# filodb/FiloDB

Hardware: NVIDIA H100
Metric: samples/s scanned+aggregated (rate over 10M series); % HBM roofline (higher is better)
Workload: dtype f64

## Files before the change

### filodb_b200/csrc/capi.cu

```cuda
#include "../../include/filo_b200.h"
#include "kernels.h"
#include "host_util.h"
#include "scan_tile_layout.h"
#include "scan_wp_layout.h"
#include <cub/cub.cuh>
#include <algorithm>
#include <atomic>
#include <chrono>
#include <cmath>
#include <cstdio>
#include <cstdlib>
#include <cstring>
#include <mutex>
#include <string>
#include <thread>
#include <vector>

using namespace filo;

struct filo_ctx {
  int device = 0;
  filo_cfg cfg{};
  cudaStream_t stream = nullptr;
  int sm_count = 132;
// ... 538 lines not shown
                                    int32_t ts_col, int32_t val_col, const int32_t* group_ids, int32_t n_groups,
                                    int32_t schema_flags, filo_table** out) {
  try { return filo_load_series_impl(ctx, n_series, n_chunks, addrs, ts_col, val_col, group_ids, n_groups, schema_flags, out); }
  catch (const std::bad_alloc&) { return fail(ctx, FILO_ERR_OOM, "filo_load_series: host allocation failed"); }
  catch (const std::exception& e) { return fail(ctx, FILO_ERR_INVALID_ARG, std::string("filo_load_series: ") + e.what()); }
}

extern "C" int32_t filo_table_set_groups(filo_ctx* ctx, filo_table* t, const int32_t* group_ids, int32_t n_groups) {
  if (!ctx || !t) return fail(ctx, FILO_ERR_INVALID_ARG, "null");
  CUDA_TRY(ctx, cudaSetDevice(ctx->device));
  if (group_ids && ctx->cfg.group_by_cardinality_limit > 0 && n_groups > ctx->cfg.group_by_cardinality_limit)
    return fail(ctx, FILO_ERR_QUERY_LIMIT, "Query exceeded group-by cardinality limit");
  int32_t* d_gid = nullptr;
  if (group_ids && t->n_series > 0) {
    for (int64_t i = 0; i < t->n_series; ++i) if (group_ids[i] < 0 || group_ids[i] >= n_groups) return fail(ctx, FILO_ERR_INVALID_ARG, "group id out of range");
    CUDA_TRY(ctx, cudaMalloc(&d_gid, (size_t)t->n_series * 4));
    CUDA_TRY(ctx, cudaMemcpy(d_gid, group_ids, (size_t)t->n_series * 4, cudaMemcpyHostToDevice));
  }
  int32_t rc = build_groups(ctx, t, d_gid, group_ids ? n_groups : 1);
  cudaFree(d_gid);
  return rc;
}

extern "C" int64_t filo_table_read_record(filo_ctx* ctx, const filo_table* t, int64_t series, uint8_t* out, int64_t cap) {
  if (!ctx || !t || series < 0 || series >= t->n_series) return fail(ctx, FILO_ERR_INVALID_ARG, "bad series");
  cudaSetDevice(ctx->device);
  int64_t off[2];
  if (cudaMemcpy(off, t->d_rec_off + series, 16, cudaMemcpyDeviceToHost) != cudaSuccess) return fail(ctx, FILO_ERR_CUDA, "read rec_off");
  int64_t n = off[1] - off[0];
  if (n > cap) return -n;
  if (cudaMemcpy(out, t->d_arena + off[0], (size_t)n, cudaMemcpyDeviceToHost) != cudaSuccess) return fail(ctx, FILO_ERR_CUDA, "read record");
  return n;
}

namespace {
__device__ __forceinline__ uint32_t rec_used_vectors(const uint8_t* r) {
  const RecordHeader h = *reinterpret_cast<const RecordHeader*>(r);
  const uint32_t v0 = (uint32_t)sizeof(RecordHeader) + 32u * h.n_chunks;
  if (h.n_chunks == 0) return 0;
  const ChunkEntry& e = reinterpret_cast<const ChunkEntry*>(r + sizeof(RecordHeader))[h.n_chunks - 1];
  const uint32_t vt = *reinterpret_cast<const uint32_t*>(r + e.val_off) + 4u;
  return align_up(e.val_off + vt, 8) - v0;
}
__global__ void append_size_kernel(const uint8_t* __restrict__ ar_o, const int64_t* __restrict__ off_o, const uint8_t* __restrict__ ar_d, const int64_t* __restrict__ off_d,
                                   int64_t n, int64_t* __restrict__ sz) {
  const int64_t i = (int64_t)blockIdx.x * blockDim.x + threadIdx.x;
  if (i < n) {
    const uint8_t* ro = ar_o + off_o[i]; const uint8_t* rd = ar_d + off_d[i];
    const uint32_t nn = reinterpret_cast<const RecordHeader*>(ro)->n_chunks + reinterpret_cast<const RecordHeader*>(rd)->n_chunks;
    sz[i] = (int64_t)align_up((uint32_t)sizeof(RecordHeader) + 32u * nn + rec_used_vectors(ro) + rec_used_vectors(rd), 16);
  }
  if (i == n) sz[i] = 0;
}
__global__ void __launch_bounds__(256) append_merge_kernel(const uint8_t* __restrict__ ar_o, const int64_t* __restrict__ off_o, const uint8_t* __restrict__ ar_d,
                                                           const int64_t* __restrict__ off_d, const int64_t* __restrict__ off_n, int64_t n,
                                                           uint8_t* __restrict__ ar_n, unsigned int* __restrict__ stats) {
  const int lane = threadIdx.x & 31;
  const int64_t i = ((int64_t)blockIdx.x * blockDim.x + threadIdx.x) >> 5;
  if (i >= n) return;
  const uint8_t* ro = ar_o + off_o[i]; const uint8_t* rd = ar_d + off_d[i]; uint8_t* rn = ar_n + off_n[i];
  const RecordHeader ho = *reinterpret_cast<const RecordHeader*>(ro), hd = *reinterpret_cast<const RecordHeader*>(rd);
  const uint32_t no = ho.n_chunks, nd = hd.n_chunks, nn = no + nd;
  const uint32_t vo0 = (uint32_t)sizeof(RecordHeader) + 32u * no, vd0 = (uint32_t)sizeof(RecordHeader) + 32u * nd, vn0 = (uint32_t)sizeof(RecordHeader) + 32u * nn;
  const uint32_t Lo = rec_used_vectors(ro), Ld = rec_used_vectors(rd);
  const uint32_t rec_bytes = align_up(vn0 + Lo + Ld, 16);
  if (lane == 0) {
    RecordHeader hn; hn.rec_bytes = rec_bytes; hn.n_chunks = nn; hn.n_rows = ho.n_rows + hd.n_rows;
    hn.flags = ((ho.flags & hd.flags) & REC_ALL_TS_CONST) | ((ho.flags | hd.flags) & ~REC_ALL_TS_CONST);
    *reinterpret_cast<RecordHeader*>(rn) = hn;
    atomicMax(&stats[0], hn.rec_bytes); atomicMax(&stats[1], hn.n_rows); atomicMax(&stats[2], nn);
    if (no && nd) {
      const ChunkEntry& lo = reinterpret_cast<const ChunkEntry*>(ro + sizeof(RecordHeader))[no - 1];
      const ChunkEntry& fd = reinterpret_cast<const ChunkEntry*>(rd + sizeof(RecordHeader))[0];
      if (fd.start_time < lo.start_time || fd.end_time < lo.end_time) atomicAdd(&stats[3], 1u);
    }
    if ((vn0 + Lo + Ld) & 8u) *reinterpret_cast<uint64_t*>(rn + vn0 + Lo + Ld) = 0ull;
  }
  for (uint32_t c = lane; c < nn; c += 32) {
    ChunkEntry e;
    if (c < no) { e = reinterpret_cast<const ChunkEntry*>(ro + sizeof(RecordHeader))[c]; e.ts_off += 32u * nd; e.val_off += 32u * nd; }
    else { e = reinterpret_cast<const ChunkEntry*>(rd + sizeof(RecordHeader))[c - no]; e.ts_off += 32u * no + Lo; e.val_off += 32u * no + Lo; e.row_base += ho.n_rows; }
    reinterpret_cast<ChunkEntry*>(rn + sizeof(RecordHeader))[c] = e;
  }
  const uint64_t* so = reinterpret_cast<const uint64_t*>(ro + vo0); uint64_t* dn = reinterpret_cast<uint64_t*>(rn + vn0);
  for (uint32_t q = lane; q < Lo / 8; q += 32) dn[q] = so[q];
  const uint64_t* sd = reinterpret_cast<const uint64_t*>(rd + vd0); dn = reinterpret_cast<uint64_t*>(rn + vn0 + Lo);
  for (uint32_t q = lane; q < Ld / 8; q += 32) dn[q] = sd[q];
}
}

static int32_t filo_table_append_impl(filo_ctx* ctx, filo_table* t, const int32_t* n_chunks, const uint64_t* chunk_info_addrs, int32_t ts_col, int32_t val_col) {
  if (!ctx || !t || !n_chunks || !chunk_info_addrs) return fail(ctx, FILO_ERR_INVALID_ARG, "filo_table_append: null argument");
  if (t->hist) return fail(ctx, FILO_ERR_UNSUPPORTED, "filo_table_append: histogram tables are rebuilt with filo_load_series");
  const int64_t S = t->n_series;
  filo_table* d = nullptr;
  { const int32_t rc = filo_load_series(ctx, S, n_chunks, chunk_info_addrs, ts_col, val_col, nullptr, 0, t->schema_flags, &d); if (rc != FILO_OK) return rc; }
  struct FreeT { filo_ctx* c; filo_table* t; ~FreeT() { filo_table_free(c, t); } } guard{ctx, d};
  if (d->hist) return fail(ctx, FILO_ERR_UNSUPPORTED, "filo_table_append: histogram vectors");
  CUDA_TRY(ctx, cudaSetDevice(ctx->device));
  cudaStream_t s = ctx->stream;
  int64_t *d_sz = nullptr, *d_off = nullptr; unsigned int* d_stats = nullptr; void* tmp = nullptr; uint8_t* d_arena = nullptr;
  struct FreeD { std::vector<void*> p; ~FreeD() { for (void* x : p) cudaFree(x); } } tmps;
  CUDA_TRY(ctx, cudaMalloc(&d_sz, (size_t)(S + 1) * 8)); tmps.p.push_back(d_sz);
  CUDA_TRY(ctx, cudaMalloc(&d_off, (size_t)(S + 1) * 8));
  CUDA_TRY(ctx, cudaMalloc(&d_stats, 16)); tmps.p.push_back(d_stats);
  CUDA_TRY(ctx, cudaMemsetAsync(d_stats, 0, 16, s));
  append_size_kernel<<<(unsigned)((S + 1 + 255) / 256), 256, 0, s>>>(t->d_arena, t->d_rec_off, d->d_arena, d->d_rec_off, S, d_sz);
  size_t tmp_bytes = 0;
  cub::DeviceScan::ExclusiveSum(nullptr, tmp_bytes, d_sz, d_off, (int)(S + 1), s);
  if (cudaMalloc(&tmp, tmp_bytes + 16) != cudaSuccess) { cudaFree(d_off); return fail(ctx, FILO_ERR_OOM, "filo_table_append: scan storage"); }
  tmps.p.push_back(tmp);
  if (cub::DeviceScan::ExclusiveSum(tmp, tmp_bytes, d_sz, d_off, (int)(S + 1), s) != cudaSuccess) { cudaFree(d_off); return fail(ctx, FILO_ERR_CUDA, "filo_table_append: scan"); }
  int64_t arena_bytes = 0;
  if (cudaMemcpyAsync(&arena_bytes, d_off + S, 8, cudaMemcpyDeviceToHost, s) != cudaSuccess || cudaStreamSynchronize(s) != cudaSuccess) { cudaFree(d_off); return fail(ctx, FILO_ERR_CUDA, "filo_table_append: sizes"); }
  if (cudaMalloc(&d_arena, (size_t)arena_bytes + 64) != cudaSuccess) { cudaFree(d_off); return fail(ctx, FILO_ERR_OOM, "filo_table_append: the new arena does not fit beside the old one"); }
  cudaMemsetAsync(d_arena + arena_bytes, 0, 64, s);
  if (S > 0) append_merge_kernel<<<(unsigned)((S * 32 + 255) / 256), 256, 0, s>>>(t->d_arena, t->d_rec_off, d->d_arena, d->d_rec_off, d_off, S, d_arena, d_stats);
  unsigned int st[4] = {0, 0, 0, 0};
  cudaError_t e = cudaGetLastError();
  if (e == cudaSuccess) e = cudaMemcpyAsync(st, d_stats, 16, cudaMemcpyDeviceToHost, s);
  if (e == cudaSuccess) e = cudaStreamSynchronize(s);
  if (e != cudaSuccess) { cudaFree(d_off); cudaFree(d_arena); return fail(ctx, FILO_ERR_CUDA, std::string("filo_table_append: ") + cudaGetErrorString(e)); }
  if (st[3]) { cudaFree(d_off); cudaFree(d_arena); return fail(ctx, FILO_ERR_UNSUPPORTED, "filo_table_append: new chunks must follow the resident ones in time (unsupported on the device path)"); }
  cudaFree(t->d_arena); cudaFree(t->d_rec_off);
  t->d_arena = d_arena; t->d_rec_off = d_off;
  t->n_chunks += d->n_chunks; t->n_samples += d->n_samples; t->algorithmic_bytes += d->algorithmic_bytes;
  t->arena_bytes = arena_bytes + (S + 1) * 8;
  t->max_rec_bytes = st[0]; t->max_rows = (int32_t)st[1]; t->max_chunks = (int32_t)st[2];
  t->any_nonconst_ts = t->any_nonconst_ts || (d->n_chunks > 0 && d->any_nonconst_ts); t->any_drop = t->any_drop || d->any_drop;
  return FILO_OK;
}
extern "C" int32_t filo_table_append(filo_ctx* ctx, filo_table* t, const int32_t* n_chunks, const uint64_t* chunk_info_addrs, int32_t ts_col, int32_t val_col) {
  try { return filo_table_append_impl(ctx, t, n_chunks, chunk_info_addrs, ts_col, val_col); }
  catch (const std::bad_alloc&) { return fail(ctx, FILO_ERR_OOM, "filo_table_append: host allocation failed"); }
  catch (const std::exception& e) { return fail(ctx, FILO_ERR_INVALID_ARG, std::string("filo_table_append: ") + e.what()); }
}

extern "C" int64_t filo_table_read_arena(filo_ctx* ctx, const filo_table* t, int64_t first, int64_t n, uint8_t* out, int64_t cap,
                                         int64_t* rec_off_out) {
  if (!ctx || !t || first < 0 || n < 0 || first + n > t->n_series || !rec_off_out) return fail(ctx, FILO_ERR_INVALID_ARG, "bad range");
  cudaSetDevice(ctx->device);
  if (cudaMemcpy(rec_off_out, t->d_rec_off + first, (size_t)(n + 1) * 8, cudaMemcpyDeviceToHost) != cudaSuccess)
    return fail(ctx, FILO_ERR_CUDA, "read rec_off");
  const int64_t base = rec_off_out[0], bytes = rec_off_out[n] - base;
  for (int64_t i = 0; i <= n; ++i) rec_off_out[i] -= base;
  if (bytes > cap || !out) return -bytes;
  if (bytes > 0 && cudaMemcpy(out, t->d_arena + base, (size_t)bytes, cudaMemcpyDeviceToHost) != cudaSuccess)
    return fail(ctx, FILO_ERR_CUDA, "read arena");
  return bytes;
}

namespace {
struct Temp {
  cudaStream_t s; std::vector<void*> ptrs;
  explicit Temp(cudaStream_t st) : s(st) {}
  ~Temp() { for (void* p : ptrs) cudaFreeAsync(p, s); }
  cudaError_t alloc(void** p, size_t bytes) { cudaError_t e = cudaMallocAsync(p, bytes ? bytes : 16, s); if (e == cudaSuccess) ptrs.push_back(*p); return e; }
};
}

namespace {
struct AsyncSink { int herr[4]; unsigned long long hc[2]; int64_t launches; };
}
static int32_t query_device_impl(filo_ctx* ctx, const filo_table* t, int32_t fn, int64_t start, int64_t step, int64_t end, int64_t window,
                                 int32_t agg, int32_t k, int32_t flags, void* d_out_values, void* d_out_aux, void* cuda_stream,
                                 filo_stats* stats, AsyncSink* sink);
extern "C" int32_t filo_query_device(filo_ctx* ctx, const filo_table* t, int32_t fn, int64_t start, int64_t step, int64_t end, int64_t window,
                                     int32_t agg, int32_t k, int32_t flags, void* d_out_values, void* d_out_aux, void* cuda_stream,
                                     filo_stats* stats) {
  return query_device_impl(ctx, t, fn, start, step, end, window, agg, k, flags, d_out_values, d_out_aux, cuda_stream, stats, nullptr);
}
namespace {
struct EventPair {
  cudaEvent_t e0 = nullptr, e1 = nullptr;
  ~EventPair() { if (e0) cudaEventDestroy(e0); if (e1) cudaEventDestroy(e1); }
};
}
static int32_t report_device_error(filo_ctx* ctx, const int herr[4], int64_t series_base);
static int32_t poll_async_errors(filo_ctx* ctx, bool wait) {
  std::lock_guard<std::mutex> g(ctx->errslot_mu);
  int32_t rc = FILO_OK;
  for (auto& sl : ctx->errslots) {
    if (!sl.pending) continue;
    cudaError_t e = wait ? cudaEventSynchronize(sl.ev) : cudaEventQuery(sl.ev);
    if (e == cudaErrorNotReady) { cudaGetLastError(); continue; }
    sl.pending = false;
    if (e != cudaSuccess) { if (rc == FILO_OK) rc = fail(ctx, FILO_ERR_CUDA, std::string("asynchronous query: ") + cudaGetErrorString(e)); continue; }
    if (sl.h[0] && rc == FILO_OK) rc = report_device_error(ctx, sl.h, 0);
  }
  return rc;
}
static int32_t push_async_error(filo_ctx* ctx, const int* d_err, cudaStream_t s) {
  std::lock_guard<std::mutex> g(ctx->errslot_mu);
  filo_ctx::ErrSlot& sl = ctx->errslots[ctx->errslot_next];
  ctx->errslot_next = (ctx->errslot_next + 1) % 16;
  if (!sl.h) { CUDA_TRY(ctx, cudaMallocHost((void**)&sl.h, 16)); CUDA_TRY(ctx, cudaEventCreateWithFlags(&sl.ev, cudaEventDisableTiming)); }
  if (sl.pending) {
    CUDA_TRY(ctx, cudaEventSynchronize(sl.ev)); sl.pending = false;
    if (sl.h[0]) return report_device_error(ctx, sl.h, 0);
  }
  CUDA_TRY(ctx, cudaMemcpyAsync(sl.h, d_err, 16, cudaMemcpyDeviceToHost, s));
  CUDA_TRY(ctx, cudaEventRecord(sl.ev, s));
  sl.pending = true;
  return FILO_OK;
}
extern "C" int32_t filo_ctx_check(filo_ctx* ctx) {
  if (!ctx) return fail(nullptr, FILO_ERR_INVALID_ARG, "ctx is null");
  return poll_async_errors(ctx, true);
}
static int32_t report_device_error(filo_ctx* ctx, const int herr[4], int64_t series_base) {
  if (herr[0] == 5)
    return fail(ctx, FILO_ERR_UNSUPPORTED, "histogram series with more chunks / sections / rows in range than the device path holds, at series " +
                std::to_string(series_base + ((int64_t)herr[1] | ((int64_t)herr[2] << 31))));
  const char* what = herr[0] == 4 ? "series needs more decode scratch than the table statistics promised" : "CorruptVector on device";
  return fail(ctx, FILO_ERR_CORRUPT_VECTOR, std::string(what) + " (code " + std::to_string(herr[0]) + ") at series " +
              std::to_string(series_base + ((int64_t)herr[1] | ((int64_t)herr[2] << 31))));
}
static int32_t query_device_impl(filo_ctx* ctx, const filo_table* t, int32_t fn, int64_t start, int64_t step, int64_t end, int64_t window,
                                 int32_t agg, int32_t k, int32_t flags, void* d_out_values, void* d_out_aux, void* cuda_stream,
                                 filo_stats* stats, AsyncSink* sink) {
  if (!ctx || !t || !d_out_values) return fail(ctx, FILO_ERR_INVALID_ARG, "filo_query: null argument");
  if (fn < FILO_FN_LAST || fn > FILO_FN_PRESENT_OVER_TIME) return fail(ctx, FILO_ERR_INVALID_ARG, "unknown range function");
  if (t->hist) return fail(ctx, FILO_ERR_UNSUPPORTED, "histogram table: use filo_query_hist");
  const bool long_values = (t->schema_flags & FILO_SCHEMA_LONG_VALUES) != 0;
  if (long_values && !fn_long_column_ok(fn)) return fail(ctx, FILO_ERR_UNSUPPORTED, "no chunked range function for this function on a Long column");
  if (fn == FILO_FN_HOLT_WINTERS) {
    if (!(ctx->fn_args[0] >= 0 && ctx->fn_args[0] <= 1)) return fail(ctx, FILO_ERR_INVALID_ARG, "Sf should be in between 0 and 1");
    if (!(ctx->fn_args[1] >= 0 && ctx->fn_args[1] <= 1)) return fail(ctx, FILO_ERR_INVALID_ARG, "tf should be in between 0 and 1");
  }
  if (agg < FILO_AGG_NONE || agg > FILO_AGG_GROUP) return fail(ctx, FILO_ERR_INVALID_ARG, "unknown aggregation operator");
  if (start > end) return fail(ctx, FILO_ERR_INVALID_ARG, "start should be <= end");
  if (!(start == end || step > 0)) return fail(ctx, FILO_ERR_INVALID_ARG, "step should be > 0 for range query");
  if (start < end && step < ctx->cfg.min_step_ms) return fail(ctx, FILO_ERR_BAD_QUERY, "step should be at least min-step");
  const int64_t adjustedStep = step > 0 ? step : step + 1;
  const bool isLast = (fn == FILO_FN_LAST || fn == FILO_FN_TIMESTAMP);
  if (window <= 0) { if (isLast) window = 5 * 60 * 1000 + 1; else return fail(ctx, FILO_ERR_INVALID_ARG, "Need positive window lengths to apply range function"); }
  if ((agg == FILO_AGG_TOPK || agg == FILO_AGG_BOTTOMK) && (k <= 0 || k > FILO_MAX_TOPK)) return fail(ctx, FILO_ERR_INVALID_ARG, "topk/bottomk k must be in [1, 32]");
  if ((agg == FILO_AGG_TOPK || agg == FILO_AGG_BOTTOMK || agg == FILO_AGG_AVG) && !d_out_aux && !(agg == FILO_AGG_AVG && !(flags & FILO_Q_PARTIAL)))
    return fail(ctx, FILO_ERR_INVALID_ARG, "out_aux required");
  if ((flags & FILO_Q_PARTIAL) && agg != FILO_AGG_NONE && agg != FILO_AGG_TOPK && agg != FILO_AGG_BOTTOMK && !d_out_aux)
    return fail(ctx, FILO_ERR_INVALID_ARG, "partial aggregates need out_aux (counts)");
  CUDA_TRY(ctx, cudaSetDevice(ctx->device));
  { const int32_t prc = poll_async_errors(ctx, false); if (prc != FILO_OK) return prc; }
  cudaStream_t s = cuda_stream ? (cudaStream_t)cuda_stream : ctx->stream;
  QueryParams q{};
  q.start = start; q.step = adjustedStep; q.end = end; q.window = window; q.T = filo_num_windows(start, adjustedStep, end);
  q.fn = fn; q.cumulative = (t->schema_flags & FILO_SCHEMA_CUMULATIVE) ? 1 : 0; q.inclusive = ctx->cfg.inclusive_range ? 1 : 0;
  q.long_values = long_values ? 1 : 0; q.p0 = ctx->fn_args[0]; q.p1 = ctx->fn_args[1];
  const bool need_corr = (fn == FILO_FN_RATE || fn == FILO_FN_INCREASE) && q.cumulative;
  const bool fused = (agg != FILO_AGG_NONE && agg != FILO_AGG_TOPK && agg != FILO_AGG_BOTTOMK);
  const bool moments = agg_moments(agg);
  const int scan_op = moments ? AGG_SUM : agg == FILO_AGG_GROUP ? AGG_COUNT : agg;

  Temp tmp(s);
  int* d_err = nullptr; unsigned long long* d_counters = nullptr;
  CUDA_TRY(ctx, tmp.alloc((void**)&d_err, 16)); CUDA_TRY(ctx, tmp.alloc((void**)&d_counters, 16));
  CUDA_TRY(ctx, cudaMemsetAsync(d_err, 0, 16, s)); CUDA_TRY(ctx, cudaMemsetAsync(d_counters, 0, 16, s));
  EventPair evp;
  if (stats) { CUDA_TRY(ctx, cudaEventCreate(&evp.e0)); CUDA_TRY(ctx, cudaEventCreate(&evp.e1)); }
  cudaEvent_t& e0 = evp.e0; cudaEvent_t& e1 = evp.e1;

  const uint32_t acc_bytes = fused ? align_up((uint32_t)q.T * (moments ? 20u : 12u), 128) : 0;
  const bool need_corr2 = need_corr && t->any_drop;
  uint32_t scratch2 = align_up((uint32_t)t->max_chunks * (uint32_t)CHUNK_DESC_BYTES, 16) +
                      ((uint32_t)t->max_rows + (uint32_t)t->max_chunks * 8u) * 8u * (1u + (t->any_nonconst_ts ? 1u : 0u) + (need_corr2 ? 1u : 0u));
  scratch2 = align_up(scratch2 + 16, 128);
  const uint32_t rec_cap = align_up(t->max_rec_bytes + 16, 128);
  const size_t per_warp2 = v2_smem_per_warp(rec_cap, scratch2, acc_bytes);
  const char* force_env = std::getenv("FILO_KERNEL");
  const std::string force = force_env ? force_env : "";
  const size_t smem_cap = std::min<size_t>(ctx->max_smem_optin, 227 * 1024);
  const bool use_v2 = force != "v1" && t->max_rec_bytes > 0 && per_warp2 * FAST_WARPS + 1024 <= smem_cap;
  const int64_t work = fused ? t->n_items : t->n_series;
  int64_t launches = 0;
  uint8_t* gscratch = nullptr;
  ScanLaunch L{t->d_arena, t->d_rec_off, t->n_series, q, nullptr, 0, 0, d_counters, d_err, 1, s};
  uint32_t rec_cap_used = 0;
  if (use_v2) {
    const size_t cta_smem = per_warp2 * FAST_WARPS + 1024;
    const int ctas_per_sm = (int)std::max<size_t>(1, std::min<size_t>(64 / FAST_WARPS, (size_t)(228 * 1024) / cta_smem));
    L.grid = (int)std::max<int64_t>(1, std::min<int64_t>((work + FAST_WARPS - 1) / FAST_WARPS, (int64_t)ctx->sm_count * ctas_per_sm));
    L.scratch_bytes = scratch2; L.use_smem = 1; rec_cap_used = rec_cap;
  } else {
    uint32_t scratch = align_up((uint32_t)t->max_chunks * (uint32_t)CHUNK_DESC_BYTES, 16) + (uint32_t)t->max_rows * 8u * (need_corr ? 3u : 2u);
    scratch = align_up(scratch + 16, 16);
    const size_t cta_smem = (size_t)(scratch + acc_bytes) * SCAN_WARPS;
    const int use_smem = cta_smem <= std::min<size_t>(ctx->max_smem_optin, 200 * 1024);
    int ctas_per_sm = 16;
    if (use_smem) ctas_per_sm = (int)std::max<size_t>(1, std::min<size_t>(16, (size_t)(220 * 1024) / std::max<size_t>(cta_smem + 1024, 1)));
    L.grid = (int)std::max<int64_t>(1, std::min<int64_t>((work + SCAN_WARPS - 1) / SCAN_WARPS, (int64_t)ctx->sm_count * ctas_per_sm));
    if (!use_smem) CUDA_TRY(ctx, tmp.alloc((void**)&gscratch, (size_t)L.grid * SCAN_WARPS * (scratch + acc_bytes)));
    L.gscratch = gscratch; L.scratch_bytes = scratch; L.use_smem = use_smem;
  }
  const int fn_cls = fn_class_of(fn, q.cumulative, q.long_values);
  const uint64_t wrows = (uint64_t)(q.window / q.step) + 1;
  TileSmem TL{};
  bool use_tile = false;
  if (use_v2 && force != "v2" && fn_cls == CLASS_SUM && t->n_series > 0) {
    TL = tile_layout(t->max_rec_bytes, (uint32_t)t->max_rows, (uint32_t)q.T, (uint32_t)std::min<uint64_t>(2 * wrows, 1u << 20) + 16);
    if (((size_t)TL.total + 1024) * 2 > (size_t)228 * 1024) TL = tile_layout(t->max_rec_bytes, (uint32_t)t->max_rows, (uint32_t)q.T, 16);
    use_tile = (size_t)TL.total + 1024 <= smem_cap;
  }
  WpSmem WL{};
  bool use_wp = false;
  if (use_tile && force != "v3" && wrows <= 4096 && t->max_chunks > 0) {
    const bool alias = wp_max_items((uint32_t)t->max_chunks, (uint32_t)q.T, (uint32_t)wrows) <= 64;
    WL = wp_layout(t->max_rec_bytes, (uint32_t)t->max_rows, (uint32_t)t->max_chunks, (uint32_t)q.T, (uint32_t)wrows, alias);
    WL.warps = (uint32_t)std::min<size_t>(smem_cap / WL.per_warp, alias ? WP_MAX_WARPS_ALIAS : WP_MAX_WARPS);
    const WpSmem WL2 = wp_layout(t->max_rec_bytes, (uint32_t)t->max_rows, (uint32_t)t->max_chunks, (uint32_t)q.T, (uint32_t)wrows, alias, true);
    if (smem_cap / WL2.per_warp >= (size_t)WP_MAX_WARPS) { WL = WL2; WL.warps = WP_MAX_WARPS; }
    use_wp = WL.warps >= 4;
  }
  WpCtrSmem WC{};
  bool use_wp_ctr = false;
  if (use_v2 && force != "v2" && force != "v3" && fn_cls == CLASS_COUNTER && t->n_series > 0 && t->max_chunks > 0 &&
      (!fused || q.T <= TILE_AGG_ACC * TILE_THREADS) && wp_ctr_tile_footprint_ok(t->max_rec_bytes, (uint32_t)t->max_rows, (uint32_t)q.T, smem_cap)) {
    WC = wp_ctr_layout(t->max_rec_bytes, (uint32_t)t->max_rows, (uint32_t)t->max_chunks, (uint32_t)q.T, fused, t->any_nonconst_ts, moments);
    const size_t w = std::min<size_t>((smem_cap - sizeof(TileCtrTab) * (TILE_CTR_TABMAX + 1) - 64) / WC.per_warp, WC.tsr != 0 ? 16 : WP_CTR_MAX_WARPS);
    WC.warps = (uint32_t)w; WC.tab = (uint32_t)(WC.per_warp * w);
    use_wp_ctr = w >= 4;
  }
  auto run_per_series = [&](double* outp) -> int32_t {
    if (use_tile || use_wp_ctr) {
      int64_t* d_list = nullptr; unsigned long long* d_cnt = nullptr;
      CUDA_TRY(ctx, tmp.alloc((void**)&d_list, (size_t)t->n_series * 8));
      CUDA_TRY(ctx, tmp.alloc((void**)&d_cnt, 16));
      CUDA_TRY(ctx, cudaMemsetAsync(d_cnt, 0, 16, s));
      ScanLaunch LT = L;
      static const bool dbg = std::getenv("FILO_DEBUG_SYNC") != nullptr;
      if (use_wp) {
        LT.grid = (int)std::max<int64_t>(1, std::min<int64_t>((t->n_series + WL.warps - 1) / WL.warps, (int64_t)ctx->sm_count));
        CUDA_TRY(ctx, launch_scan_wp(LT, outp, WL, d_list, d_cnt));
      } else if (use_wp_ctr) {
        LT.grid = (int)std::max<int64_t>(1, std::min<int64_t>((t->n_series + WC.warps - 1) / WC.warps, (int64_t)ctx->sm_count));
        CUDA_TRY(ctx, launch_scan_wp_ctr(LT, outp, WC, d_list, d_cnt));
      } else {
        const int ctas_per_sm = ((size_t)TL.total + 1024) * 2 <= (size_t)228 * 1024 ? 2 : 1;
        const int64_t n_tiles = (t->n_series + TILE_NS - 1) / TILE_NS;
        LT.grid = (int)std::max<int64_t>(1, std::min<int64_t>(n_tiles, (int64_t)ctx->sm_count * ctas_per_sm));
        if (dbg) { fprintf(stderr, "[filo] tile kernel fn=%d T=%d grid=%d smem=%u pitch=%u\n", fn, q.T, LT.grid, TL.total, TL.vals_pitch); fflush(stderr); }
        CUDA_TRY(ctx, launch_scan_tile(LT, outp, TL, d_list, d_cnt));
      }
      if (dbg) { CUDA_TRY(ctx, cudaStreamSynchronize(s)); fprintf(stderr, "[filo] tile kernel done\n"); fflush(stderr); }
      ScanLaunch LF = L; LF.list = d_list; LF.list_count = d_cnt;
      CUDA_TRY(ctx, launch_scan_series_v2(LF, outp, rec_cap_used));
      if (dbg) { CUDA_TRY(ctx, cudaStreamSynchronize(s)); fprintf(stderr, "[filo] fallback kernel done\n"); fflush(stderr); }
      launches += 2;
    } else {
      CUDA_TRY(ctx, use_v2 ? launch_scan_series_v2(L, outp, rec_cap_used) : launch_scan_series(L, outp));
      launches += 1;
    }
    return FILO_OK;
  };
  if (stats) CUDA_TRY(ctx, cudaEventRecord(e0, s));
  if (agg == FILO_AGG_NONE) {
    { int32_t rc = run_per_series((double*)d_out_values); if (rc) return rc; }
  } else if (!fused) {
    double* per = nullptr;
    CUDA_TRY(ctx, tmp.alloc((void**)&per, (size_t)t->n_series * q.T * 8));
    { int32_t rc = run_per_series(per); if (rc) return rc; }
    CUDA_TRY(ctx, launch_topk(per, t->grouped ? t->d_order : nullptr, t->d_group_start, t->n_groups, q.T, k, agg == FILO_AGG_BOTTOMK,
                              (double*)d_out_values, (int64_t*)d_out_aux, s));
    launches += 1;
  } else {
    double* pval = nullptr; uint32_t* pcnt = nullptr;
    CUDA_TRY(ctx, tmp.alloc((void**)&pval, (size_t)t->n_items * q.T * 8 * (moments ? 2 : 1)));
    CUDA_TRY(ctx, tmp.alloc((void**)&pcnt, (size_t)t->n_items * q.T * 4));
    const int32_t* order = t->grouped ? t->d_order : nullptr;
    if ((use_tile && q.T <= TILE_AGG_ACC * TILE_THREADS) || use_wp_ctr) {
      int64_t* d_list = nullptr; unsigned long long* d_cnt = nullptr;
      CUDA_TRY(ctx, tmp.alloc((void**)&d_list, (size_t)t->n_items * 8));
      CUDA_TRY(ctx, tmp.alloc((void**)&d_cnt, 16));
      CUDA_TRY(ctx, cudaMemsetAsync(d_cnt, 0, 16, s));
      ScanLaunch LT = L;
      if (use_wp_ctr) {
        LT.grid = (int)std::max<int64_t>(1, std::min<int64_t>((t->n_items + WC.warps - 1) / WC.warps, (int64_t)ctx->sm_count));
        CUDA_TRY(ctx, launch_scan_wp_ctr_agg(LT, WC, order, t->d_item_begin, t->n_items, scan_op, pval, pcnt, d_list, d_cnt, moments));
      } else {
        const int ctas_per_sm = ((size_t)TL.total + 1024) * 2 <= (size_t)228 * 1024 ? 2 : 1;
        LT.grid = (int)std::max<int64_t>(1, std::min<int64_t>(t->n_items, (int64_t)ctx->sm_count * ctas_per_sm));
        CUDA_TRY(ctx, launch_scan_tile_agg(LT, TL, order, t->d_item_begin, t->n_items, scan_op, pval, pcnt, d_list, d_cnt, moments));
      }
      ScanLaunch LF = L; LF.list = d_list; LF.list_count = d_cnt;
      CUDA_TRY(ctx, launch_scan_agg_v2(LF, order, t->d_item_begin, t->n_items, scan_op, pval, pcnt, acc_bytes, rec_cap_used, moments));
      launches += 1;
    } else {
      CUDA_TRY(ctx, use_v2 ? launch_scan_agg_v2(L, order, t->d_item_begin, t->n_items, scan_op, pval, pcnt, acc_bytes, rec_cap_used, moments)
                           : launch_scan_agg(L, order, t->d_item_begin, t->n_items, moments ? agg : scan_op, pval, pcnt, acc_bytes));
    }
    CUDA_TRY(ctx, launch_merge_partials(pval, pcnt, t->d_gis, t->n_groups, q.T, agg, (flags & FILO_Q_PARTIAL) ? 1 : 0,
                                        (double*)d_out_values, (int64_t*)d_out_aux, s));
    launches += 2;
  }
  if (stats) {
    CUDA_TRY(ctx, cudaEventRecord(e1, s));
    int herr[4]; unsigned long long hc[2];
    CUDA_TRY(ctx, cudaMemcpyAsync(herr, d_err, 16, cudaMemcpyDeviceToHost, s));
    CUDA_TRY(ctx, cudaMemcpyAsync(hc, d_counters, 16, cudaMemcpyDeviceToHost, s));
    CUDA_TRY(ctx, cudaStreamSynchronize(s));
    float ms = 0; cudaEventElapsedTime(&ms, e0, e1);
    stats->kernel_ns = (int64_t)((double)ms * 1e6); stats->samples_scanned = (int64_t)hc[0]; stats->bytes_scanned = (int64_t)hc[1];
    stats->kernel_launches = launches; stats->h2d_bytes = 0; stats->d2h_bytes = 0;
    if (herr[0]) return report_device_error(ctx, herr, 0);
  }
  if (!stats && !sink) { const int32_t rc = push_async_error(ctx, d_err, s); if (rc != FILO_OK) return rc; }
  if (sink) {
    sink->launches = launches;
    CUDA_TRY(ctx, cudaMemcpyAsync(sink->herr, d_err, 16, cudaMemcpyDeviceToHost, s));
    CUDA_TRY(ctx, cudaMemcpyAsync(sink->hc, d_counters, 16, cudaMemcpyDeviceToHost, s));
  }
  return FILO_OK;
}

static int32_t filo_query_impl(filo_ctx* ctx, const filo_table* t, int32_t fn, int64_t start, int64_t step, int64_t end, int64_t window,
                              int32_t agg, int32_t k, int32_t flags, double* out_values, int64_t* out_aux, filo_stats* stats) {
  if (!ctx || !t || !out_values) return fail(ctx, FILO_ERR_INVALID_ARG, "filo_query: null argument");
  if (start > end) return fail(ctx, FILO_ERR_INVALID_ARG, "start should be <= end");
  CUDA_TRY(ctx, cudaSetDevice(ctx->device));
  const int64_t adjustedStep = step > 0 ? step : step + 1;
  const int T = filo_num_windows(start, adjustedStep, end);
  size_t nvals, naux = 0;
  if (agg == FILO_AGG_NONE) nvals = (size_t)t->n_series * T;
  else if (agg == FILO_AGG_TOPK || agg == FILO_AGG_BOTTOMK) { if (k <= 0 || k > FILO_MAX_TOPK) return fail(ctx, FILO_ERR_INVALID_ARG, "topk/bottomk k must be in [1, 32]"); nvals = naux = (size_t)t->n_groups * T * k; }
  else { naux = (size_t)t->n_groups * T; nvals = naux * ((flags & FILO_Q_PARTIAL) && agg_moments(agg) ? 2 : 1); }
  cudaStream_t s = ctx->stream;
  double* d_vals = nullptr; int64_t* d_aux = nullptr;
  CUDA_TRY(ctx, cudaMallocAsync((void**)&d_vals, std::max<size_t>(nvals, 1) * 8, s));
  if (naux) CUDA_TRY(ctx, cudaMallocAsync((void**)&d_aux, naux * 8, s));
  filo_stats st{};
  int32_t rc = filo_query_device(ctx, t, fn, start, step, end, window, agg, k, flags, d_vals, d_aux, s, &st);
  if (rc == FILO_OK) {
    cudaError_t e = cudaMemcpyAsync(out_values, d_vals, nvals * 8, cudaMemcpyDeviceToHost, s);
    if (e == cudaSuccess && naux && out_aux) e = cudaMemcpyAsync(out_aux, d_aux, naux * 8, cudaMemcpyDeviceToHost, s);
    if (e == cudaSuccess) e = cudaStreamSynchronize(s);
    if (e != cudaSuccess) rc = fail(ctx, FILO_ERR_CUDA, std::string("result copy: ") + cudaGetErrorString(e));
    st.d2h_bytes = (int64_t)(nvals * 8 + ((naux && out_aux) ? naux * 8 : 0));
  }
  cudaFreeAsync(d_vals, s); if (d_aux) cudaFreeAsync(d_aux, s);
  if (stats) *stats = st;
  return rc;
}
extern "C" int32_t filo_query(filo_ctx* ctx, const filo_table* t, int32_t fn, int64_t start, int64_t step, int64_t end, int64_t window,
                              int32_t agg, int32_t k, int32_t flags, double* out_values, int64_t* out_aux, filo_stats* stats) {
  try { return filo_query_impl(ctx, t, fn, start, step, end, window, agg, k, flags, out_values, out_aux, stats); }
  catch (const std::bad_alloc&) { return fail(ctx, FILO_ERR_OOM, "filo_query: host allocation failed"); }
  catch (const std::exception& e) { return fail(ctx, FILO_ERR_INVALID_ARG, std::string("filo_query: ") + e.what()); }
}



namespace {
__global__ void ratio_kernel(double* __restrict__ num, const double* __restrict__ den, int64_t n) {
  for (int64_t i = (int64_t)blockIdx.x * blockDim.x + threadIdx.x; i < n; i += (int64_t)gridDim.x * blockDim.x) num[i] = num[i] / den[i];
}
}
static int32_t filo_query_avg_sum_count_impl(filo_ctx* ctx, const filo_table* t_sum, const filo_table* t_count, int64_t start, int64_t step, int64_t end,
                                             int64_t window, double* out_values, filo_stats* stats) {
  if (!ctx || !t_sum || !t_count || !out_values) return fail(ctx, FILO_ERR_INVALID_ARG, "filo_query_avg_sum_count: null argument");
  if (start > end) return fail(ctx, FILO_ERR_INVALID_ARG, "start should be <= end");
  if (t_sum->hist || t_count->hist) return fail(ctx, FILO_ERR_INVALID_ARG, "filo_query_avg_sum_count: scalar columns only");
  if (t_sum->n_series != t_count->n_series) return fail(ctx, FILO_ERR_INVALID_ARG, "filo_query_avg_sum_count: the two tables hold different numbers of series");
  if (t_count->schema_flags & FILO_SCHEMA_LONG_VALUES) return fail(ctx, FILO_ERR_UNSUPPORTED, "filo_query_avg_sum_count: the count column is read as a DoubleVector (AggrOverTimeFunctions.scala:851,890)");
  CUDA_TRY(ctx, cudaSetDevice(ctx->device));
  const int64_t adjustedStep = step > 0 ? step : step + 1;
  const int T = filo_num_windows(start, adjustedStep, end);
  const size_t n = (size_t)t_sum->n_series * (size_t)T;
  cudaStream_t s = ctx->stream;
  Temp tmp(s);
  double *d_num = nullptr, *d_den = nullptr;
  CUDA_TRY(ctx, tmp.alloc((void**)&d_num, n * 8));
  CUDA_TRY(ctx, tmp.alloc((void**)&d_den, n * 8));
  const bool long_sum = (t_sum->schema_flags & FILO_SCHEMA_LONG_VALUES) != 0;
  filo_stats a{}, b{};
  int32_t rc = filo_query_device(ctx, t_sum, FILO_FN_SUM_OVER_TIME, start, step, end, window, FILO_AGG_NONE, 0, 0, d_num, nullptr, s, &a);
  if (rc == FILO_OK) rc = filo_query_device(ctx, t_count, long_sum ? FILO_FN_COUNT_OVER_TIME : FILO_FN_SUM_OVER_TIME, start, step, end, window, FILO_AGG_NONE, 0, 0, d_den, nullptr, s, &b);
  if (rc != FILO_OK) return rc;
  if (n) {
    ratio_kernel<<<(unsigned)std::min<size_t>((n + 255) / 256, (size_t)ctx->sm_count * 16), 256, 0, s>>>(d_num, d_den, (int64_t)n);
    CUDA_TRY(ctx, cudaGetLastError());
    CUDA_TRY(ctx, cudaMemcpyAsync(out_values, d_num, n * 8, cudaMemcpyDeviceToHost, s));
  }
  CUDA_TRY(ctx, cudaStreamSynchronize(s));
  if (stats) {
    *stats = a;
    stats->bytes_scanned += b.bytes_scanned; stats->samples_scanned += b.samples_scanned; stats->kernel_ns += b.kernel_ns;
    stats->kernel_launches += b.kernel_launches + 1; stats->d2h_bytes = (int64_t)(n * 8);
  }
  return FILO_OK;
}
extern "C" int32_t filo_query_avg_sum_count(filo_ctx* ctx, const filo_table* t_sum, const filo_table* t_count, int64_t start, int64_t step, int64_t end,
                                            int64_t window, double* out_values, filo_stats* stats) {
  try { return filo_query_avg_sum_count_impl(ctx, t_sum, t_count, start, step, end, window, out_values, stats); }
  catch (const std::bad_alloc&) { return fail(ctx, FILO_ERR_OOM, "filo_query_avg_sum_count: host allocation failed"); }
  catch (const std::exception& e) { return fail(ctx, FILO_ERR_INVALID_ARG, std::string("filo_query_avg_sum_count: ") + e.what()); }
}

namespace {

__device__ __forceinline__ void copy_bytes_warp(uint8_t* dst, const uint8_t* src, int n, int lane) {
  const uintptr_t a = reinterpret_cast<uintptr_t>(src);
  if ((a & 3) == 0) {
    const int nw = n >> 2;
    const uint32_t* s4 = reinterpret_cast<const uint32_t*>(src); uint32_t* d4 = reinterpret_cast<uint32_t*>(dst);
    for (int i = lane; i < nw; i += 32) d4[i] = s4[i];
    for (int i = (nw << 2) + lane; i < n; i += 32) dst[i] = src[i];
  } else {
    for (int i = lane; i < n; i += 32) dst[i] = src[i];
  }
}
__global__ void __launch_bounds__(256) gather_records_kernel(const GatherSeries* __restrict__ gs, const GatherChunk* __restrict__ gc,
                                                             const int64_t* __restrict__ rec_off, int64_t n, uint8_t* __restrict__ arena, int64_t rebase) {
  const int lane = threadIdx.x & 31;
  const int64_t w = ((int64_t)blockIdx.x * blockDim.x + threadIdx.x) >> 5, nw = ((int64_t)gridDim.x * blockDim.x) >> 5;
  for (int64_t i = w; i < n; i += nw) {
    const GatherSeries S = gs[i];
    uint8_t* rec = arena + rec_off[i];
    if (lane == 0) { RecordHeader h{S.rec_bytes, S.n_chunks, S.n_rows, S.flags}; *reinterpret_cast<RecordHeader*>(rec) = h; }
    uint32_t off = sizeof(RecordHeader) + S.n_chunks * (uint32_t)sizeof(ChunkEntry), row_base = 0;
    for (uint32_t c = 0; c < S.n_chunks; ++c) {
      const GatherChunk G = gc[S.first_chunk + c];
      const uint32_t ts_off = off, ts_pad = align_up((uint32_t)G.ts_bytes, 8), val_off = off + ts_pad, val_pad = align_up((uint32_t)G.val_bytes, 8);
      if (lane == 0) {
        ChunkEntry ce; ce.start_time = G.start_time; ce.end_time = G.end_time; ce.num_rows = G.num_rows; ce.ts_off = ts_off; ce.val_off = val_off; ce.row_base = row_base;
        reinterpret_cast<ChunkEntry*>(rec + sizeof(RecordHeader))[c] = ce;
      }
      copy_bytes_warp(rec + ts_off, reinterpret_cast<const uint8_t*>(G.ts_src + (uint64_t)rebase), G.ts_bytes, lane);
      copy_bytes_warp(rec + val_off, reinterpret_cast<const uint8_t*>(G.val_src + (uint64_t)rebase), G.val_bytes, lane);
      if (lane < (int)(ts_pad - G.ts_bytes)) rec[ts_off + G.ts_bytes + lane] = 0;
      if (lane < (int)(val_pad - G.val_bytes)) rec[val_off + G.val_bytes + lane] = 0;
      __syncwarp();
      if (lane == 0 && G.drop_patch) { if (G.drop_patch == 1) rec[val_off + 7] |= 0x80; else rec[val_off + 7] &= 0x7f; }
      off = val_off + val_pad; row_base += (uint32_t)G.val_len;
    }
    for (uint32_t k = off + lane; k < S.rec_bytes; k += 32) rec[k] = 0;
  }
}
}

extern "C" int32_t filo_host_register(filo_ctx* ctx, const void* base, int64_t bytes) {
  if (!ctx || !base || bytes <= 0) return fail(ctx, FILO_ERR_INVALID_ARG, "filo_host_register: bad arguments");
  CUDA_TRY(ctx, cudaSetDevice(ctx->device));
  CUDA_TRY(ctx, cudaHostRegister(const_cast<void*>(base), (size_t)bytes, cudaHostRegisterMapped | cudaHostRegisterPortable));
  std::lock_guard<std::mutex> g(ctx->scan_mu);
  ctx->ranges.push_back({(uintptr_t)base, (size_t)bytes});
  return FILO_OK;
}
extern "C" int32_t filo_host_unregister(filo_ctx* ctx, const void* base) {
  if (!ctx || !base) return fail(ctx, FILO_ERR_INVALID_ARG, "filo_host_unregister: bad arguments");
  std::lock_guard<std::mutex> g(ctx->scan_mu);
  for (size_t i = 0; i < ctx->ranges.size(); ++i) if (ctx->ranges[i].base == (uintptr_t)base) {
    for (auto& sl : ctx->scan) if (sl.stream) cudaStreamSynchronize(sl.stream);
    CUDA_TRY(ctx, cudaHostUnregister(const_cast<void*>(base)));
    ctx->ranges.erase(ctx->ranges.begin() + (long)i);
    return FILO_OK;
  }
  return fail(ctx, FILO_ERR_INVALID_ARG, "filo_host_unregister: range not registered");
}

namespace {
template <class T> int32_t grow_pinned(filo_ctx* ctx, T*& p, size_t& cap, size_t need) {
  if (need <= cap) return FILO_OK;
  cudaFreeHost(p); p = nullptr; cap = 0;
  CUDA_TRY(ctx, cudaHostAlloc((void**)&p, need, cudaHostAllocDefault));
  cap = need; return FILO_OK;
}
template <class T> int32_t grow_device(filo_ctx* ctx, T*& p, size_t& cap, size_t need) {
  if (need <= cap) return FILO_OK;
  cudaFree(p); p = nullptr; cap = 0;
  CUDA_TRY(ctx, cudaMalloc((void**)&p, need));
  cap = need; return FILO_OK;
}
}

static int32_t filo_scan_series_impl(filo_ctx* ctx, int64_t n_series, const int32_t* n_chunks, const uint64_t* addrs,
                                    int32_t ts_col, int32_t val_col, int32_t schema_flags,
                                    int32_t fn, int64_t start, int64_t step, int64_t end, int64_t window,
                                    double* out_values, filo_stats* stats) {
  if (!ctx || n_series < 0 || (n_series > 0 && (!n_chunks || !addrs || !out_values)) || ts_col < 0 || val_col < 0)
    return fail(ctx, FILO_ERR_INVALID_ARG, "filo_scan_series: bad arguments");
  if (start > end) return fail(ctx, FILO_ERR_INVALID_ARG, "start should be <= end");
  CUDA_TRY(ctx, cudaSetDevice(ctx->device));
  std::lock_guard<std::mutex> one(ctx->scan_mu);
  const int64_t adjustedStep = step > 0 ? step : step + 1;
  const int T = filo_num_windows(start, adjustedStep, end);
  static const bool timing = std::getenv("FILO_DEBUG_TIMING") != nullptr;
  auto now = [] { return std::chrono::steady_clock::now(); };
  auto ms_since = [](std::chrono::steady_clock::time_point a) { return std::chrono::duration<double, std::milli>(std::chrono::steady_clock::now() - a).count(); };
  const auto t_begin = now();
  double t_fill = 0, t_retire = 0, t_enq = 0;
  std::vector<SeriesPlan> plan;
  std::vector<int64_t> chunk_base;
  int64_t chunks_before = 0;
  LoadIn in{n_series, n_chunks, addrs, nullptr, ts_col, val_col};
  auto env_int = [](const char* name, long dflt, long lo, long hi) { const char* e = std::getenv(name); if (!e || !*e) return dflt; const long v = std::atol(e); return v < lo ? lo : v > hi ? hi : v; };
  const int64_t PLAN_CHUNK = env_int("FILO_SCAN_PLAN_CHUNK", 65536, 1024, 1 << 24);
  std::vector<GatherChunk> gc_walk;
  const size_t SLAB = (size_t)env_int("FILO_SCAN_SLAB_MB", 192, 1, 4096) << 20;
  const int64_t max_rows_out = std::max<int64_t>(1, (int64_t)(((size_t)env_int("FILO_SCAN_OUT_MB", 256, 1, 4096) << 20) / ((size_t)std::max(T, 1) * 8)));
  const char* trace_path = std::getenv("FILO_SCAN_TRACE");
  struct TraceRow { int64_t nb; size_t bytes; double host_ms; cudaEvent_t ev[4]; };
  std::vector<TraceRow> trace; cudaEvent_t trace_t0 = nullptr;
  struct Batch { int64_t s0, s1; size_t bytes; int64_t chunks; };
  std::vector<filo_ctx::HostRange> ranges = ctx->ranges;
  auto in_ranges = [&](const uint8_t* p, size_t n) { for (auto& r : ranges) if ((uintptr_t)p >= r.base && (uintptr_t)p + n <= r.base + r.bytes) return true; return false; };
  const int NSLOT = (int)env_int("FILO_SCAN_SLOTS", 6, 2, filo_ctx::MAX_SCAN_SLOTS);
  for (int i = 0; i < NSLOT; ++i) {
    filo_ctx::ScanSlot& sl = ctx->scan[i];
    if (!sl.stream) { CUDA_TRY(ctx, cudaStreamCreateWithFlags(&sl.stream, cudaStreamNonBlocking)); CUDA_TRY(ctx, cudaEventCreateWithFlags(&sl.done, cudaEventDisableTiming)); }
    if (!sl.h_sink) CUDA_TRY(ctx, cudaHostAlloc(&sl.h_sink, sizeof(AsyncSink), cudaHostAllocDefault));
  }
  double t_plan = 0;
  int64_t alg_total = 0; size_t n_batches = 0;
  filo_stats acc{};
  struct InFlight { int64_t s0 = -1; } fl[filo_ctx::MAX_SCAN_SLOTS];
  int32_t rc = FILO_OK;
  auto retire = [&](int i) -> int32_t {
    filo_ctx::ScanSlot& sl = ctx->scan[i];
    if (fl[i].s0 < 0) return FILO_OK;
    CUDA_TRY(ctx, cudaEventSynchronize(sl.done));
    const AsyncSink* k = reinterpret_cast<const AsyncSink*>(sl.h_sink);
    acc.samples_scanned += (int64_t)k->hc[0]; acc.bytes_scanned += (int64_t)k->hc[1]; acc.kernel_launches += k->launches;
    const int64_t base = fl[i].s0; fl[i].s0 = -1;
    if (k->herr[0]) return report_device_error(ctx, k->herr, base);
    return FILO_OK;
  };
  for (int64_t c0 = 0; c0 < n_series && rc == FILO_OK; c0 += PLAN_CHUNK) {
    const int64_t c1 = std::min<int64_t>(n_series, c0 + PLAN_CHUNK);
    const auto t_p0 = now();
    PlanTotals tot; int64_t err_series = -1;
    plan.resize((size_t)(c1 - c0)); chunk_base.resize((size_t)(c1 - c0) + 1);
    chunk_base[0] = chunks_before;
    for (int64_t i = c0; i < c1; ++i) {
      if (n_chunks[i] < 0) { rc = fail(ctx, FILO_ERR_INVALID_ARG, "negative n_chunks"); break; }
// ... 285 lines not shown
```

### filodb_b200/csrc/kernels.h

```cpp
#pragma once
#include <cuda_runtime.h>
#include <stdint.h>
#include "filo_record.h"

namespace filo {

constexpr int SCAN_WARPS = 4;
constexpr int FAST_WARPS = 4;
constexpr int FAST_MIN_CTAS = 4;
constexpr int CHUNK_DESC_BYTES = 144;
constexpr int FILO_MAX_TOPK = 32;
enum { AGG_NONE = 0, AGG_SUM = 1, AGG_AVG = 2, AGG_MIN = 3, AGG_MAX = 4, AGG_COUNT = 5, AGG_TOPK = 6, AGG_BOTTOMK = 7,
       AGG_STDDEV = 8, AGG_STDVAR = 9, AGG_GROUP = 10 };
__host__ __device__ inline bool agg_moments(int agg_op) { return agg_op == AGG_STDDEV || agg_op == AGG_STDVAR; }
template <bool ON, typename T> struct MomOnly { T v; };
template <typename T> struct MomOnly<false, T> {};

struct QueryParams;

}
#include "scan_params.h"
#include "scan_tile_layout.h"
namespace filo {

struct ScanLaunch {
  const uint8_t* arena; const int64_t* rec_off; int64_t n_series;
  QueryParams q;
  uint8_t* gscratch; uint32_t scratch_bytes; int use_smem;
  unsigned long long* d_counters; int* d_err;
  int grid; cudaStream_t stream;
  const int64_t* list = nullptr; const unsigned long long* list_count = nullptr;
};

cudaError_t launch_scan_series(const ScanLaunch& L, double* out);
cudaError_t launch_scan_agg(const ScanLaunch& L, const int32_t* order, const int64_t* item_begin, int64_t n_items, int agg_op,
                            double* pval, uint32_t* pcnt, uint32_t acc_bytes);
cudaError_t launch_scan_series_v2(const ScanLaunch& L, double* out, uint32_t rec_cap);
cudaError_t launch_scan_agg_v2(const ScanLaunch& L, const int32_t* order, const int64_t* item_begin, int64_t n_items, int agg_op,
                               double* pval, uint32_t* pcnt, uint32_t acc_bytes, uint32_t rec_cap, bool moments = false);
size_t v2_smem_per_warp(uint32_t rec_cap, uint32_t scratch_bytes, uint32_t acc_bytes);
cudaError_t launch_scan_tile(const ScanLaunch& L, double* out, const TileSmem& T, int64_t* fallback_list, unsigned long long* fallback_count);
cudaError_t launch_scan_tile_agg(const ScanLaunch& L, const TileSmem& T, const int32_t* order, const int64_t* item_begin, int64_t n_items, int agg_op,
                                 double* pval, uint32_t* pcnt, int64_t* fallback_list, unsigned long long* fallback_count, bool moments = false);
cudaError_t launch_merge_partials(const double* pval, const uint32_t* pcnt, const int64_t* gis, int n_groups, int T, int agg_op,
                                  int partial_out, double* out_val, int64_t* out_cnt, cudaStream_t s);
cudaError_t launch_present(int agg_op, int64_t n, const double* vals, const int64_t* cnts, double* out, cudaStream_t s);
cudaError_t launch_topk(const double* per_series, const int32_t* order, const int64_t* group_start, int n_groups, int T, int k, int bottom,
                        double* out_val, int64_t* out_id, cudaStream_t s);
struct WpSmem;
cudaError_t launch_scan_wp(const ScanLaunch& L, double* out, const WpSmem& W, int64_t* fallback_list, unsigned long long* fallback_count);
struct WpCtrSmem;
cudaError_t launch_scan_wp_ctr(const ScanLaunch& L, double* out, const WpCtrSmem& W, int64_t* fallback_list, unsigned long long* fallback_count);
cudaError_t launch_scan_wp_ctr_agg(const ScanLaunch& L, const WpCtrSmem& W, const int32_t* order, const int64_t* item_begin, int64_t n_items, int agg_op,
                                   double* pval, uint32_t* pcnt, int64_t* fallback_list, unsigned long long* fallback_count, bool moments = false);
size_t hist_smem_bytes(int max_rows, int nb, int T, bool agg, uint32_t max_rec);
cudaError_t launch_hist_scan(const ScanLaunch& L, int nb, int max_rows, uint32_t max_rec, const int32_t* order, const int64_t* item_begin, int64_t n_items, int agg,
                             double* out, double* pval, uint8_t* pany, const double* tops = nullptr, double qtl = 0.0, int exp_buckets = 0, double* out_q = nullptr);
cudaError_t launch_hist_merge(const double* pval, const uint8_t* pany, const int64_t* gis, int n_groups, int T, int nb, int exp_buckets, const double* tops, double q,
                              double* out_values, double* out_q, cudaStream_t s);
size_t hist2_smem_bytes(int max_rows, int nb, uint32_t max_rec);
cudaError_t launch_hist_scan2(const ScanLaunch& L, int nb, int max_rows, uint32_t max_rec, const int32_t* order, const int64_t* item_begin, int64_t n_items,
                              double* pval, uint8_t* pany);
int64_t hist2_series_items(int64_t n_series);
cudaError_t launch_hist_scan2_series(const ScanLaunch& L, int nb, int max_rows, uint32_t max_rec, double* out_values, double* out_q, double* scratch,
                                     const double* tops, double qtl, int exp_buckets);
cudaError_t launch_hist_merge2(const double* pval, const uint8_t* pany, const int64_t* gis, int n_groups, int T, int nb, int exp_buckets, const double* tops, double q,
                               double* out_values, double* out_q, cudaStream_t s);
cudaError_t launch_hist_merge_parts(const double* parts, int n_parts, int64_t n_cells, int nb, int exp_buckets, const double* tops, double q,
                                    double* out_values, double* out_q, cudaStream_t s);
cudaError_t launch_iota(int32_t* a, int64_t n, cudaStream_t s);
cudaError_t launch_group_bounds(const int32_t* sorted_keys, int64_t n, int n_groups, int64_t* group_start, cudaStream_t s);
cudaError_t launch_group_item_count(const int64_t* group_start, int n_groups, int seg, int64_t* cnt, cudaStream_t s);
cudaError_t launch_fill_items(const int64_t* group_start, const int64_t* gis, int n_groups, int seg, int64_t n_items, int64_t n_series,
                              int64_t* item_begin, cudaStream_t s);

}
```

### filodb_b200/csrc/scan_kernels.cu

```cuda
#include <cuda_runtime.h>
#include <stdint.h>
#define FILO_DEV_ERR_TS_WIRE 1
#define FILO_DEV_ERR_VAL_WIRE 2
#define FILO_DEV_ERR_EMPTY 3
#define FILO_DEV_ERR_SCRATCH 4
#include "scan_device.cuh"
#include "kernels.h"
#include "scan_fast.cuh"
#include "scan_tile.cuh"
#include "scan_wp.cuh"
#include "scan_wp_ctr.cuh"

namespace filo {

__device__ __forceinline__ void report_error(int* d_err, int code, int64_t series) {
  if (atomicCAS(&d_err[0], 0, code) == 0) { d_err[1] = (int)(series & 0x7fffffff); d_err[2] = (int)(series >> 31); }
}

__device__ __forceinline__ int resolve_series(const uint8_t* rec, const QueryParams& q, uint8_t* scratch, uint32_t scratch_bytes,
                                              bool need_corrected, int lane, int& err, int64_t& rows_scanned, int64_t& bytes_scanned) {
  const RecordHeader* h = reinterpret_cast<const RecordHeader*>(rec);
  const ChunkEntry* E = reinterpret_cast<const ChunkEntry*>(rec + sizeof(RecordHeader));
  const int nch = (int)h->n_chunks;
  const int64_t t1 = q.start - q.window, t2 = q.end;
// ... 63 lines not shown
  double* acc2 = acc + q.T;
  uint32_t* cnt = reinterpret_cast<uint32_t*>(base + (size_t)q.T * (mom ? 16 : 8));
  uint8_t* scratch = base + acc_bytes;
  const int fn = q.fn;
  const bool need_corrected = ((fn == FN_RATE || fn == FN_INCREASE) && q.cumulative);
  const double ident = agg_op == AGG_MIN ? __longlong_as_double(0x7ff0000000000000LL)
                     : agg_op == AGG_MAX ? __longlong_as_double(0xfff0000000000000LL) : 0.0;
  int64_t rows = 0, bytes = 0;
  for (int64_t it = gw; it < n_items; it += nw) {
    for (int k = lane; k < q.T; k += 32) { acc[k] = ident; cnt[k] = 0; if (mom) acc2[k] = 0.0; }
    const int64_t b = item_begin[it], e = item_begin[it + 1];
    for (int64_t pos = b; pos < e; ++pos) {
      const int64_t i = order ? order[pos] : pos;
      const uint8_t* rec = arena + rec_off[i];
      int err;
      const int n = resolve_series(rec, q, scratch, scratch_bytes, need_corrected, lane, err, rows, bytes);
      if (err) { if (lane == 0) report_error(d_err, err, i); continue; }
      const ChunkDesc* D = reinterpret_cast<const ChunkDesc*>(scratch);
      for (int k = lane; k < q.T; k += 32) {
        const double v = eval_window(D, 0, n, q, k);
        if (v == v) {
          double a = acc[k];
          if (agg_op == AGG_MIN) a = a < v ? a : v;
          else if (agg_op == AGG_MAX) a = a > v ? a : v;
          else if (agg_op == AGG_COUNT) a = a;
          else a += v;
          acc[k] = a; cnt[k] += 1;
          if (mom) acc2[k] += v * v;
        }
      }
      __syncwarp();
    }
    double* pv = pval + (size_t)it * q.T; uint32_t* pc = pcnt + (size_t)it * q.T;
    for (int k = lane; k < q.T; k += 32) { pv[k] = acc[k]; pc[k] = cnt[k]; }
    if (mom) { double* pv2 = pval + (size_t)(n_items + it) * q.T; for (int k = lane; k < q.T; k += 32) pv2[k] = acc2[k]; }
    __syncwarp();
  }
  if (lane == 0 && (rows | bytes)) { atomicAdd(&d_counters[0], (unsigned long long)rows); atomicAdd(&d_counters[1], (unsigned long long)bytes); }
}

__device__ __forceinline__ double present_cell(int agg_op, double s, double s2, int64_t c) {
  const double NaNv = __longlong_as_double(0x7ff8000000000000LL);
  if (c == 0) return NaNv;
  if (agg_op == AGG_AVG) return s / (double)c;
  if (agg_op == AGG_COUNT) return (double)c;
  if (agg_op == AGG_GROUP) return 1.0;
  if (agg_moments(agg_op)) {
    const double m = s / (double)c;
    const double var = s2 / (double)c - m * m;
    if (agg_op == AGG_STDVAR) return var;
    if (var < 0.0) return var == -__longlong_as_double(0x7ff0000000000000LL) ? __longlong_as_double(0x7ff0000000000000LL) : NaNv;
    return var == 0.0 ? 0.0 : sqrt(var);
  }
  return s;
}

enum { MERGE_PLAIN = 0, MERGE_MOMENTS = 1, MERGE_GROUP = 2 };
template <int EXT = MERGE_PLAIN>
__global__ void __launch_bounds__(256)
merge_partials_kernel(const double* __restrict__ pval, const uint32_t* __restrict__ pcnt, const int64_t* __restrict__ gis,
                      int n_groups, int T, int agg_op, int partial_out, double* __restrict__ out_val, int64_t* __restrict__ out_cnt) {
  __shared__ double sv[8][33]; __shared__ unsigned long long sc[8][33];
  const int kk = threadIdx.x & 31, j = threadIdx.x >> 5;
  const int ktiles = (T + 31) / 32;
  const int g = blockIdx.x / ktiles, k = (blockIdx.x % ktiles) * 32 + kk;
  if (g >= n_groups) return;
  const double ident = agg_op == AGG_MIN ? __longlong_as_double(0x7ff0000000000000LL)
                     : agg_op == AGG_MAX ? __longlong_as_double(0xfff0000000000000LL) : 0.0;
  double a = ident; unsigned long long c = 0;
  constexpr bool MOM = EXT == MERGE_MOMENTS;
  MomOnly<MOM, double> a2;
  if constexpr (MOM) a2.v = 0.0;
  if (k < T) {
    for (int64_t it = gis[g] + j; it < gis[g + 1]; it += 8) {
      const double v = pval[(size_t)it * T + k]; const uint32_t n = pcnt[(size_t)it * T + k];
      if (n) {
        if (agg_op == AGG_MIN) a = a < v ? a : v; else if (agg_op == AGG_MAX) a = a > v ? a : v; else a += v;
        if constexpr (MOM) a2.v += pval[(size_t)(gis[n_groups] + it) * T + k];
        c += n;
      }
    }
  }
  sv[j][kk] = a; sc[j][kk] = c;
  if constexpr (MOM) { __shared__ double sv2[8][33]; sv2[j][kk] = a2.v; __syncthreads(); if (j == 0 && k < T) for (int jj = 1; jj < 8; ++jj) if (sc[jj][kk]) a2.v += sv2[jj][kk]; }
  __syncthreads();
  if (j == 0 && k < T) {
    for (int jj = 1; jj < 8; ++jj) {
      const double v = sv[jj][kk]; const unsigned long long n = sc[jj][kk];
      if (n) { if (agg_op == AGG_MIN) a = a < v ? a : v; else if (agg_op == AGG_MAX) a = a > v ? a : v; else a += v; c += n; }
    }
    const size_t o = (size_t)g * T + k;
    if constexpr (EXT != MERGE_PLAIN) {
      double s2 = 0.0;
      if constexpr (MOM) s2 = a2.v;
      if (partial_out) { out_val[o] = a; if constexpr (MOM) out_val[(size_t)n_groups * T + o] = s2; if (out_cnt) out_cnt[o] = (int64_t)c; }
      else { out_val[o] = present_cell(agg_op, a, s2, (int64_t)c); if (out_cnt) out_cnt[o] = (int64_t)c; }
    } else if (partial_out) { out_val[o] = a; if (out_cnt) out_cnt[o] = (int64_t)c; }
    else {
      const double NaNv = __longlong_as_double(0x7ff8000000000000LL);
      double r;
      if (c == 0) r = NaNv;
      else if (agg_op == AGG_AVG) r = a / (double)c;
      else if (agg_op == AGG_COUNT) r = (double)c;
      else r = a;
      out_val[o] = r; if (out_cnt) out_cnt[o] = (int64_t)c;
    }
  }
}

__global__ void present_kernel(int agg_op, int64_t n, const double* __restrict__ vals, const int64_t* __restrict__ cnts, double* __restrict__ out) {
  const int64_t i = (int64_t)blockIdx.x * blockDim.x + threadIdx.x;
  if (i >= n) return;
  out[i] = present_cell(agg_op, vals[i], agg_moments(agg_op) ? vals[n + i] : 0.0, cnts[i]);
}

__global__ void topk_kernel(const double* __restrict__ per_series, const int32_t* __restrict__ order, const int64_t* __restrict__ group_start,
                            int n_groups, int T, int kk, int bottom, double* __restrict__ out_val, int64_t* __restrict__ out_id) {
  const int64_t tid = (int64_t)blockIdx.x * blockDim.x + threadIdx.x;
  if (tid >= (int64_t)n_groups * T) return;
  const int g = (int)(tid / T), t = (int)(tid % T);
  double bv[FILO_MAX_TOPK]; int64_t bi[FILO_MAX_TOPK]; int n = 0;
  for (int64_t pos = group_start[g]; pos < group_start[g + 1]; ++pos) {
    const int64_t s = order ? order[pos] : pos;
    const double v = per_series[(size_t)s * T + t];
    if (v != v) continue;
    int p = n;
    while (p > 0 && (bottom ? (v < bv[p - 1]) : (v > bv[p - 1]))) --p;
    if (p >= kk) continue;
    const int last = n < kk ? n : kk - 1;
    for (int m = last; m > p; --m) { bv[m] = bv[m - 1]; bi[m] = bi[m - 1]; }
    bv[p] = v; bi[p] = s; if (n < kk) ++n;
  }
  double* ov = out_val + (size_t)tid * kk; int64_t* oi = out_id + (size_t)tid * kk;
  for (int m = 0; m < kk; ++m) {
    if (m < n) { ov[m] = bv[n - 1 - m]; oi[m] = bi[n - 1 - m]; }
    else { ov[m] = bottom ? 1.7976931348623157e308 : -1.7976931348623157e308; oi[m] = -1; }
  }
}

__global__ void iota_kernel(int32_t* a, int64_t n) { int64_t i = (int64_t)blockIdx.x * blockDim.x + threadIdx.x; if (i < n) a[i] = (int32_t)i; }
__global__ void group_bounds_kernel(const int32_t* __restrict__ sorted_keys, int64_t n, int n_groups, int64_t* __restrict__ group_start) {
  const int g = blockIdx.x * blockDim.x + threadIdx.x;
  if (g > n_groups) return;
  int64_t lo = 0, hi = n;
  while (lo < hi) { int64_t m = (lo + hi) >> 1; if (sorted_keys[m] < g) lo = m + 1; else hi = m; }
  group_start[g] = lo;
}
__global__ void group_item_count_kernel(const int64_t* __restrict__ group_start, int n_groups, int seg, int64_t* __restrict__ cnt) {
  const int g = blockIdx.x * blockDim.x + threadIdx.x;
  if (g < n_groups) { int64_t n = group_start[g + 1] - group_start[g]; cnt[g] = (n + seg - 1) / seg; }
}
__global__ void fill_items_kernel(const int64_t* __restrict__ group_start, const int64_t* __restrict__ gis, int n_groups, int seg,
                                  int64_t n_items, int64_t n_series, int64_t* __restrict__ item_begin) {
  const int g = blockIdx.x * blockDim.x + threadIdx.x;
  if (g < n_groups) {
    const int64_t b = group_start[g], e = group_start[g + 1];
    int64_t it = gis[g];
    for (int64_t p = b; p < e; p += seg) item_begin[it++] = p;
  }
  if (g == 0) item_begin[n_items] = n_series;
}

struct WarpStage {
  uint64_t* bar; uint8_t* buf; uint32_t cap; uint32_t parity; bool staged;
  const uint8_t* arena; const int64_t* rec_off;
  __device__ __forceinline__ void issue(int64_t series, int lane) {
    const int64_t o = rec_off[series];
    const uint32_t bytes = (uint32_t)(rec_off[series + 1] - o);
    staged = cap != 0 && bytes <= cap;
    if (staged && lane == 0) { mbar_expect_tx(bar, bytes); tma_load_1d(buf, arena + o, bytes, bar); }
  }
  __device__ __forceinline__ const uint8_t* acquire(int64_t series) {
    if (!staged) return arena + rec_off[series];
    mbar_wait(bar, parity); parity ^= 1;
    return buf;
  }
};

template <int CLS>
__global__ void __launch_bounds__(FAST_WARPS * 32, FAST_MIN_CTAS)
scan_series_kernel_v2(const uint8_t* __restrict__ arena, const int64_t* __restrict__ rec_off, int64_t n_series,
                      QueryParams q, double* __restrict__ out, uint32_t rec_cap, uint32_t scratch_bytes,
                      unsigned long long* d_counters, int* d_err,
                      const int64_t* __restrict__ list, const unsigned long long* __restrict__ list_count) {
  if (list) n_series = (int64_t)*list_count;
  extern __shared__ __align__(128) uint8_t smem[];
  const int warp = threadIdx.x >> 5, lane = threadIdx.x & 31;
  const int64_t gw = (int64_t)blockIdx.x * FAST_WARPS + warp, nw = (int64_t)gridDim.x * FAST_WARPS;
  const uint32_t per_warp = WARP_HDR_BYTES + rec_cap + STAGE_BYTES + scratch_bytes;
  uint8_t* base = smem + (size_t)warp * per_warp;
  WarpStage st{reinterpret_cast<uint64_t*>(base), base + WARP_HDR_BYTES, rec_cap, 0, false, arena, rec_off};
  double* stage = reinterpret_cast<double*>(base + WARP_HDR_BYTES + rec_cap);
  uint8_t* scratch = base + WARP_HDR_BYTES + rec_cap + STAGE_BYTES;
  if (lane == 0) { mbar_init(st.bar, 1); mbar_fence_init(); }
  __syncwarp();
  int64_t rows = 0, bytes = 0;
  int64_t ii = gw;
  if (ii < n_series) st.issue(list ? list[ii] : ii, lane);
  for (; ii < n_series; ii += nw) {
    const int64_t i = list ? list[ii] : ii;
    const uint8_t* rec = st.acquire(i);
    double* o = out + (size_t)i * q.T;
    int err;
    const int64_t inext_i = ii + nw;
    const bool has_next = inext_i < n_series;
    const int64_t inext = has_next ? (list ? list[inext_i] : inext_i) : 0;
    process_series<CLS>(rec, q, scratch, scratch_bytes, stage, lane, err, rows, bytes,
                   [&](int k, double v, bool valid) { if (valid) o[k] = v; },
                   [&]() { if (has_next) st.issue(inext, lane); });
    if (err) {
      if (lane == 0) report_error(d_err, err, i);
      __syncwarp();
      if (has_next) st.issue(inext, lane);
    }
    __syncwarp();
  }
  if (lane == 0 && (rows | bytes)) { atomicAdd(&d_counters[0], (unsigned long long)rows); atomicAdd(&d_counters[1], (unsigned long long)bytes); }
}

template <int CLS, bool MOM = false>
__global__ void __launch_bounds__(FAST_WARPS * 32, FAST_MIN_CTAS)
scan_agg_kernel_v2(const uint8_t* __restrict__ arena, const int64_t* __restrict__ rec_off, const int32_t* __restrict__ order,
                   const int64_t* __restrict__ item_begin, int64_t n_items,
                   QueryParams q, int agg_op, double* __restrict__ pval, uint32_t* __restrict__ pcnt,
                   uint32_t rec_cap, uint32_t scratch_bytes, uint32_t acc_bytes,
                   unsigned long long* d_counters, int* d_err,
                   const int64_t* __restrict__ list, const unsigned long long* __restrict__ list_count) {
  MomOnly<MOM, double*> pval2;
  if constexpr (MOM) pval2.v = pval + (size_t)n_items * q.T;
  if (list) n_items = (int64_t)*list_count;
  extern __shared__ __align__(128) uint8_t smem[];
  const int warp = threadIdx.x >> 5, lane = threadIdx.x & 31;
  const int64_t gw = (int64_t)blockIdx.x * FAST_WARPS + warp, nw = (int64_t)gridDim.x * FAST_WARPS;
  const uint32_t per_warp = WARP_HDR_BYTES + rec_cap + STAGE_BYTES + acc_bytes + scratch_bytes;
  uint8_t* base = smem + (size_t)warp * per_warp;
  WarpStage st{reinterpret_cast<uint64_t*>(base), base + WARP_HDR_BYTES, rec_cap, 0, false, arena, rec_off};
  double* stage = reinterpret_cast<double*>(base + WARP_HDR_BYTES + rec_cap);
  double* acc = reinterpret_cast<double*>(base + WARP_HDR_BYTES + rec_cap + STAGE_BYTES);
  MomOnly<MOM, double*> acc2;
  if constexpr (MOM) acc2.v = acc + q.T;
  uint32_t* cnt = reinterpret_cast<uint32_t*>(base + WARP_HDR_BYTES + rec_cap + STAGE_BYTES + (size_t)q.T * (MOM ? 16 : 8));
  uint8_t* scratch = base + WARP_HDR_BYTES + rec_cap + STAGE_BYTES + acc_bytes;
  if (lane == 0) { mbar_init(st.bar, 1); mbar_fence_init(); }
  __syncwarp();
  const double ident = agg_op == AGG_MIN ? __longlong_as_double(0x7ff0000000000000LL)
                     : agg_op == AGG_MAX ? __longlong_as_double(0xfff0000000000000LL) : 0.0;
  int64_t rows = 0, bytes = 0;
  int64_t it = gw;
  int64_t pos = 0, pend = 0;
  auto real_item = [&](int64_t x) -> int64_t { return list ? list[x] : x; };
  auto advance_item = [&]() { while (it < n_items) { const int64_t ri = real_item(it); pos = item_begin[ri]; pend = item_begin[ri + 1]; if (pos < pend) return true; it += nw; } return false; };
  bool have = advance_item();
  if (have) st.issue(order ? order[pos] : pos, lane);
  while (have) {
    for (int k = lane; k < q.T; k += 32) { acc[k] = ident; cnt[k] = 0; if constexpr (MOM) acc2.v[k] = 0.0; }
    __syncwarp();
    const int64_t my_item = real_item(it);
    while (true) {
      const int64_t i = order ? order[pos] : pos;
      int64_t npos = pos + 1, nit = it, npend = pend; bool nhave = true;
      if (npos >= pend) { nit = it + nw; nhave = false; while (nit < n_items) { const int64_t ri = real_item(nit); npos = item_begin[ri]; npend = item_begin[ri + 1]; if (npos < npend) { nhave = true; break; } nit += nw; } }
      const int64_t inext = nhave ? (order ? order[npos] : npos) : -1;
      const uint8_t* rec = st.acquire(i);
      int err;
      process_series<CLS>(rec, q, scratch, scratch_bytes, stage, lane, err, rows, bytes,
                     [&](int k, double v, bool valid) {
                       if (valid && v == v) {
                         double a = acc[k];
                         if (agg_op == AGG_MIN) a = a < v ? a : v;
                         else if (agg_op == AGG_MAX) a = a > v ? a : v;
                         else if (agg_op != AGG_COUNT) a += v;
                         acc[k] = a; cnt[k] += 1;
                         if constexpr (MOM) acc2.v[k] += v * v;
                       }
                     },
                     [&]() { if (inext >= 0) st.issue(inext, lane); });
      if (err) {
        if (lane == 0) report_error(d_err, err, i);
        __syncwarp();
        if (inext >= 0) st.issue(inext, lane);
      }
      __syncwarp();
      const bool same_item = nhave && nit == it;
      pos = npos; pend = npend; it = nit; have = nhave;
      if (!same_item) break;
    }
    double* pv = pval + (size_t)my_item * q.T; uint32_t* pc = pcnt + (size_t)my_item * q.T;
    for (int k = lane; k < q.T; k += 32) { pv[k] = acc[k]; pc[k] = cnt[k]; }
    if constexpr (MOM) { double* pv2 = pval2.v + (size_t)my_item * q.T; for (int k = lane; k < q.T; k += 32) pv2[k] = acc2.v[k]; }
    __syncwarp();
  }
  if (lane == 0 && (rows | bytes)) { atomicAdd(&d_counters[0], (unsigned long long)rows); atomicAdd(&d_counters[1], (unsigned long long)bytes); }
}

#ifndef FILO_CUSIM
#ifdef FILO_TILE_PROF
extern "C" int filo_debug_tile_prof(unsigned long long* out16, int reset) {
  cudaError_t e = cudaMemcpyFromSymbol(out16, g_tile_prof, sizeof(unsigned long long) * 16);
  if (e == cudaSuccess && reset) { unsigned long long z[16] = {}; e = cudaMemcpyToSymbol(g_tile_prof, z, sizeof z); }
  return (int)e;
}
#endif
#ifdef FILO_WP_PROF
extern "C" int filo_debug_wp_prof(unsigned long long* out16, int reset) {
  cudaError_t e = cudaMemcpyFromSymbol(out16, g_wp_prof, sizeof(unsigned long long) * 16);
  if (e == cudaSuccess && reset) { unsigned long long z[16] = {}; e = cudaMemcpyToSymbol(g_wp_prof, z, sizeof z); }
  return (int)e;
}
#endif
template <int CLS>
static cudaError_t launch_series_v2_cls(const ScanLaunch& L, double* out, uint32_t rec_cap, size_t smem) {
  cudaError_t e = cudaFuncSetAttribute(scan_series_kernel_v2<CLS>, cudaFuncAttributeMaxDynamicSharedMemorySize, (int)smem);
  if (e != cudaSuccess) return e;
  scan_series_kernel_v2<CLS><<<L.grid, FAST_WARPS * 32, smem, L.stream>>>(L.arena, L.rec_off, L.n_series, L.q, out, rec_cap, L.scratch_bytes,
                                                                           L.d_counters, L.d_err, L.list, L.list_count);
  return cudaGetLastError();
}
cudaError_t launch_scan_series_v2(const ScanLaunch& L, double* out, uint32_t rec_cap) {
  const size_t smem = (size_t)(WARP_HDR_BYTES + rec_cap + STAGE_BYTES + L.scratch_bytes) * FAST_WARPS;
  switch (fn_class_of(L.q.fn, L.q.cumulative, L.q.long_values)) {
    case CLASS_SUM: return launch_series_v2_cls<CLASS_SUM>(L, out, rec_cap, smem);
    case CLASS_MINMAX: return launch_series_v2_cls<CLASS_MINMAX>(L, out, rec_cap, smem);
    case CLASS_COUNTER: return launch_series_v2_cls<CLASS_COUNTER>(L, out, rec_cap, smem);
    default: return launch_series_v2_cls<CLASS_POINT>(L, out, rec_cap, smem);
  }
}
template <int CLS, bool MOM>
static cudaError_t launch_agg_v2_cls(const ScanLaunch& L, const int32_t* order, const int64_t* item_begin, int64_t n_items, int agg_op,
                                     double* pval, uint32_t* pcnt, uint32_t acc_bytes, uint32_t rec_cap, size_t smem) {
  cudaError_t e = cudaFuncSetAttribute(scan_agg_kernel_v2<CLS, MOM>, cudaFuncAttributeMaxDynamicSharedMemorySize, (int)smem);
  if (e != cudaSuccess) return e;
  scan_agg_kernel_v2<CLS, MOM><<<L.grid, FAST_WARPS * 32, smem, L.stream>>>(L.arena, L.rec_off, order, item_begin, n_items, L.q, agg_op, pval, pcnt,
                                                                             rec_cap, L.scratch_bytes, acc_bytes, L.d_counters, L.d_err, L.list, L.list_count);
  return cudaGetLastError();
}
template <bool MOM>
static cudaError_t launch_agg_v2_any(const ScanLaunch& L, const int32_t* order, const int64_t* item_begin, int64_t n_items, int agg_op,
                                     double* pval, uint32_t* pcnt, uint32_t acc_bytes, uint32_t rec_cap, size_t smem) {
  switch (fn_class_of(L.q.fn, L.q.cumulative, L.q.long_values)) {
    case CLASS_SUM: return launch_agg_v2_cls<CLASS_SUM, MOM>(L, order, item_begin, n_items, agg_op, pval, pcnt, acc_bytes, rec_cap, smem);
    case CLASS_MINMAX: return launch_agg_v2_cls<CLASS_MINMAX, MOM>(L, order, item_begin, n_items, agg_op, pval, pcnt, acc_bytes, rec_cap, smem);
    case CLASS_COUNTER: return launch_agg_v2_cls<CLASS_COUNTER, MOM>(L, order, item_begin, n_items, agg_op, pval, pcnt, acc_bytes, rec_cap, smem);
    default: return launch_agg_v2_cls<CLASS_POINT, MOM>(L, order, item_begin, n_items, agg_op, pval, pcnt, acc_bytes, rec_cap, smem);
  }
}
cudaError_t launch_scan_agg_v2(const ScanLaunch& L, const int32_t* order, const int64_t* item_begin, int64_t n_items, int agg_op,
                               double* pval, uint32_t* pcnt, uint32_t acc_bytes, uint32_t rec_cap, bool moments) {
  const size_t smem = (size_t)(WARP_HDR_BYTES + rec_cap + STAGE_BYTES + acc_bytes + L.scratch_bytes) * FAST_WARPS;
  return moments ? launch_agg_v2_any<true>(L, order, item_begin, n_items, agg_op, pval, pcnt, acc_bytes, rec_cap, smem)
                 : launch_agg_v2_any<false>(L, order, item_begin, n_items, agg_op, pval, pcnt, acc_bytes, rec_cap, smem);
}
struct TileAggArgs { const int32_t* order; const int64_t* item_begin; int64_t n_items; int agg_op; double* pval; uint32_t* pcnt; };
template <int FN, bool AGG, bool MOM>
static cudaError_t launch_tile_fn(const ScanLaunch& L, double* out, const TileSmem& T, int64_t* fallback_list, unsigned long long* fallback_count,
                                  const TileAggArgs& A) {
  cudaError_t e = cudaFuncSetAttribute(scan_tile_kernel<FN, AGG, MOM>, cudaFuncAttributeMaxDynamicSharedMemorySize, (int)T.total);
  if (e != cudaSuccess) return e;
  scan_tile_kernel<FN, AGG, MOM><<<L.grid, TILE_LAUNCH_THREADS, T.total, L.stream>>>(L.arena, L.rec_off, L.n_series, L.q, out, T, fallback_list, fallback_count,
      L.d_counters, L.d_err, A.order, A.item_begin, A.n_items, A.agg_op, A.pval, A.pcnt);
  return cudaGetLastError();
}
template <bool AGG, bool MOM = false>
static cudaError_t launch_tile_any(const ScanLaunch& L, double* out, const TileSmem& T, int64_t* fallback_list, unsigned long long* fallback_count,
                                   const TileAggArgs& A) {
  switch (L.q.fn) {
    case FN_RATE: return launch_tile_fn<FN_RATE, AGG, MOM>(L, out, T, fallback_list, fallback_count, A);
    case FN_AVG: return launch_tile_fn<FN_AVG, AGG, MOM>(L, out, T, fallback_list, fallback_count, A);
    case FN_COUNT: return launch_tile_fn<FN_COUNT, AGG, MOM>(L, out, T, fallback_list, fallback_count, A);
    default: return launch_tile_fn<FN_SUM, AGG, MOM>(L, out, T, fallback_list, fallback_count, A);
  }
}
cudaError_t launch_scan_tile(const ScanLaunch& L, double* out, const TileSmem& T, int64_t* fallback_list, unsigned long long* fallback_count) {
  return launch_tile_any<false>(L, out, T, fallback_list, fallback_count, TileAggArgs{nullptr, nullptr, 0, 0, nullptr, nullptr});
}
cudaError_t launch_scan_tile_agg(const ScanLaunch& L, const TileSmem& T, const int32_t* order, const int64_t* item_begin, int64_t n_items, int agg_op,
                                 double* pval, uint32_t* pcnt, int64_t* fallback_list, unsigned long long* fallback_count, bool moments) {
  const TileAggArgs A{order, item_begin, n_items, agg_op, pval, pcnt};
  return moments ? launch_tile_any<true, true>(L, nullptr, T, fallback_list, fallback_count, A)
                 : launch_tile_any<true>(L, nullptr, T, fallback_list, fallback_count, A);
}
template <int FN, int NW>
static cudaError_t launch_wp_nw(const ScanLaunch& L, double* out, const WpSmem& W, int64_t* fallback_list, unsigned long long* fallback_count) {
  const size_t smem = (size_t)W.per_warp * W.warps;
  cudaError_t e = cudaFuncSetAttribute(scan_wp_sum_kernel<FN, NW>, cudaFuncAttributeMaxDynamicSharedMemorySize, (int)smem);
  if (e != cudaSuccess) return e;
  scan_wp_sum_kernel<FN, NW><<<L.grid, W.warps * 32, smem, L.stream>>>(L.arena, L.rec_off, L.n_series, L.q, out, W, fallback_list, fallback_count, L.d_counters, L.d_err);
  return cudaGetLastError();
}
template <int FN>
static cudaError_t launch_wp_fn(const ScanLaunch& L, double* out, const WpSmem& W, int64_t* fallback_list, unsigned long long* fallback_count) {
  if (W.warps <= (uint32_t)WP_MAX_WARPS) return launch_wp_nw<FN, WP_MAX_WARPS>(L, out, W, fallback_list, fallback_count);
  return launch_wp_nw<FN, WP_MAX_WARPS_ALIAS>(L, out, W, fallback_list, fallback_count);
}
cudaError_t launch_scan_wp(const ScanLaunch& L, double* out, const WpSmem& W, int64_t* fallback_list, unsigned long long* fallback_count) {
  switch (L.q.fn) {
    case FN_RATE: return launch_wp_fn<FN_RATE>(L, out, W, fallback_list, fallback_count);
    case FN_AVG: return launch_wp_fn<FN_AVG>(L, out, W, fallback_list, fallback_count);
    case FN_COUNT: return launch_wp_fn<FN_COUNT>(L, out, W, fallback_list, fallback_count);
    default: return launch_wp_fn<FN_SUM>(L, out, W, fallback_list, fallback_count);
  }
}
template <int FN, bool AGG, int NW, bool IRR, bool MOM>
static cudaError_t launch_wp_ctr_nw(const ScanLaunch& L, double* out, const WpCtrSmem& W, int64_t* fallback_list, unsigned long long* fallback_count,
                                    const TileAggArgs& A) {
  const size_t smem = (size_t)W.per_warp * W.warps + sizeof(TileCtrTab) * (TILE_CTR_TABMAX + 1);
  cudaError_t e = cudaFuncSetAttribute(scan_wp_ctr_kernel<FN, AGG, NW, IRR, MOM>, cudaFuncAttributeMaxDynamicSharedMemorySize, (int)smem);
  if (e != cudaSuccess) return e;
  scan_wp_ctr_kernel<FN, AGG, NW, IRR, MOM><<<L.grid, W.warps * 32, smem, L.stream>>>(L.arena, L.rec_off, L.n_series, L.q, out, W, fallback_list, fallback_count,
      L.d_counters, L.d_err, A.order, A.item_begin, A.n_items, A.agg_op, A.pval, A.pcnt);
  return cudaGetLastError();
}
template <int FN, bool AGG, bool MOM>
static cudaError_t launch_wp_ctr_fn(const ScanLaunch& L, double* out, const WpCtrSmem& W, int64_t* fallback_list, unsigned long long* fallback_count, const TileAggArgs& A) {
  if (W.tsr != 0) return launch_wp_ctr_nw<FN, AGG, 16, true, MOM>(L, out, W, fallback_list, fallback_count, A);
  if (W.warps <= 16) return launch_wp_ctr_nw<FN, AGG, 16, false, MOM>(L, out, W, fallback_list, fallback_count, A);
  return launch_wp_ctr_nw<FN, AGG, WP_CTR_MAX_WARPS, false, MOM>(L, out, W, fallback_list, fallback_count, A);
}
template <bool AGG, bool MOM = false>
static cudaError_t launch_wp_ctr_any(const ScanLaunch& L, double* out, const WpCtrSmem& W, int64_t* fallback_list, unsigned long long* fallback_count, const TileAggArgs& A) {
  switch (L.q.fn) {
    case FN_RATE: return launch_wp_ctr_fn<FN_RATE, AGG, MOM>(L, out, W, fallback_list, fallback_count, A);
    case FN_INCREASE: return launch_wp_ctr_fn<FN_INCREASE, AGG, MOM>(L, out, W, fallback_list, fallback_count, A);
    default: return launch_wp_ctr_fn<FN_DELTA, AGG, MOM>(L, out, W, fallback_list, fallback_count, A);
  }
}
cudaError_t launch_scan_wp_ctr(const ScanLaunch& L, double* out, const WpCtrSmem& W, int64_t* fallback_list, unsigned long long* fallback_count) {
  return launch_wp_ctr_any<false>(L, out, W, fallback_list, fallback_count, TileAggArgs{nullptr, nullptr, 0, 0, nullptr, nullptr});
}
cudaError_t launch_scan_wp_ctr_agg(const ScanLaunch& L, const WpCtrSmem& W, const int32_t* order, const int64_t* item_begin, int64_t n_items, int agg_op,
                                   double* pval, uint32_t* pcnt, int64_t* fallback_list, unsigned long long* fallback_count, bool moments) {
  const TileAggArgs A{order, item_begin, n_items, agg_op, pval, pcnt};
  return moments ? launch_wp_ctr_any<true, true>(L, nullptr, W, fallback_list, fallback_count, A)
                 : launch_wp_ctr_any<true>(L, nullptr, W, fallback_list, fallback_count, A);
}
size_t v2_smem_per_warp(uint32_t rec_cap, uint32_t scratch_bytes, uint32_t acc_bytes) { return WARP_HDR_BYTES + (size_t)rec_cap + STAGE_BYTES + acc_bytes + scratch_bytes; }
cudaError_t launch_scan_series(const ScanLaunch& L, double* out) {
  size_t smem = L.use_smem ? (size_t)L.scratch_bytes * SCAN_WARPS : 0;
  if (smem > 48 * 1024) {
    cudaError_t e = cudaFuncSetAttribute(scan_series_kernel, cudaFuncAttributeMaxDynamicSharedMemorySize, (int)smem);
    if (e != cudaSuccess) return e;
  }
  scan_series_kernel<<<L.grid, SCAN_WARPS * 32, smem, L.stream>>>(L.arena, L.rec_off, L.n_series, L.q, out,
      L.gscratch, L.scratch_bytes, L.use_smem, L.d_counters, L.d_err);
  return cudaGetLastError();
}
cudaError_t launch_scan_agg(const ScanLaunch& L, const int32_t* order, const int64_t* item_begin, int64_t n_items, int agg_op,
                            double* pval, uint32_t* pcnt, uint32_t acc_bytes) {
  size_t smem = L.use_smem ? (size_t)(L.scratch_bytes + acc_bytes) * SCAN_WARPS : 0;
  if (smem > 48 * 1024) {
    cudaError_t e = cudaFuncSetAttribute(scan_agg_kernel, cudaFuncAttributeMaxDynamicSharedMemorySize, (int)smem);
    if (e != cudaSuccess) return e;
  }
  scan_agg_kernel<<<L.grid, SCAN_WARPS * 32, smem, L.stream>>>(L.arena, L.rec_off, order, item_begin, n_items, L.q, agg_op,
      pval, pcnt, L.gscratch, L.scratch_bytes, acc_bytes, L.use_smem, L.d_counters, L.d_err);
  return cudaGetLastError();
}
cudaError_t launch_merge_partials(const double* pval, const uint32_t* pcnt, const int64_t* gis, int n_groups, int T, int agg_op,
                                  int partial_out, double* out_val, int64_t* out_cnt, cudaStream_t s) {
  const int ktiles = (T + 31) / 32;
  if (agg_moments(agg_op)) merge_partials_kernel<MERGE_MOMENTS><<<n_groups * ktiles, 256, 0, s>>>(pval, pcnt, gis, n_groups, T, agg_op, partial_out, out_val, out_cnt);
  else if (agg_op == AGG_GROUP) merge_partials_kernel<MERGE_GROUP><<<n_groups * ktiles, 256, 0, s>>>(pval, pcnt, gis, n_groups, T, agg_op, partial_out, out_val, out_cnt);
  else merge_partials_kernel<<<n_groups * ktiles, 256, 0, s>>>(pval, pcnt, gis, n_groups, T, agg_op, partial_out, out_val, out_cnt);
  return cudaGetLastError();
}
cudaError_t launch_present(int agg_op, int64_t n, const double* vals, const int64_t* cnts, double* out, cudaStream_t s) {
  present_kernel<<<(unsigned)((n + 255) / 256), 256, 0, s>>>(agg_op, n, vals, cnts, out);
  return cudaGetLastError();
}
cudaError_t launch_topk(const double* per_series, const int32_t* order, const int64_t* group_start, int n_groups, int T, int k, int bottom,
                        double* out_val, int64_t* out_id, cudaStream_t s) {
  const int64_t n = (int64_t)n_groups * T;
  topk_kernel<<<(unsigned)((n + 127) / 128), 128, 0, s>>>(per_series, order, group_start, n_groups, T, k, bottom, out_val, out_id);
  return cudaGetLastError();
}
cudaError_t launch_iota(int32_t* a, int64_t n, cudaStream_t s) {
  iota_kernel<<<(unsigned)((n + 255) / 256), 256, 0, s>>>(a, n); return cudaGetLastError();
}
cudaError_t launch_group_bounds(const int32_t* sorted_keys, int64_t n, int n_groups, int64_t* group_start, cudaStream_t s) {
  group_bounds_kernel<<<(n_groups + 1 + 127) / 128, 128, 0, s>>>(sorted_keys, n, n_groups, group_start); return cudaGetLastError();
}
cudaError_t launch_group_item_count(const int64_t* group_start, int n_groups, int seg, int64_t* cnt, cudaStream_t s) {
  group_item_count_kernel<<<(n_groups + 127) / 128, 128, 0, s>>>(group_start, n_groups, seg, cnt); return cudaGetLastError();
}
cudaError_t launch_fill_items(const int64_t* group_start, const int64_t* gis, int n_groups, int seg, int64_t n_items, int64_t n_series,
                              int64_t* item_begin, cudaStream_t s) {
  fill_items_kernel<<<(n_groups + 127) / 128, 128, 0, s>>>(group_start, gis, n_groups, seg, n_items, n_series, item_begin);
  return cudaGetLastError();
}

#endif

}
```

### filodb_b200/csrc/scan_wp.cuh

```cuda
#pragma once
#include "scan_tile.cuh"
#include "scan_wp_layout.h"

namespace filo {

#ifdef FILO_CUSIM
__device__ __forceinline__ uint32_t wp_soff(const void* p) { return (uint32_t)(reinterpret_cast<const uint8_t*>(p) - smem); }
__device__ __forceinline__ uint32_t wp_lds32(uint32_t off) { uint32_t v; std::memcpy(&v, smem + off, 4); return v; }
#else
__device__ __forceinline__ uint32_t wp_soff(const void* p) { return smem_u32(p); }
__device__ __forceinline__ uint32_t wp_lds32(uint32_t off) { uint32_t v; asm volatile("ld.shared.u32 %0, [%1];" : "=r"(v) : "r"(off)); return v; }
#endif

#if defined(FILO_WP_PROF) && !defined(FILO_CUSIM)
__device__ unsigned long long g_wp_prof[16];
#define WPROF_DECL uint32_t wpp_t0 = (uint32_t)clock(), wpp_acc[14] = {0, 0, 0, 0, 0, 0, 0, 0, 0, 0, 0, 0, 0, 0};
#define WPROF(i) { const uint32_t wpp_t1 = (uint32_t)clock(); wpp_acc[i] += wpp_t1 - wpp_t0; wpp_t0 = wpp_t1; }
#define WPROF_COUNT(i) { ++wpp_acc[i]; }
#define WPROF_FLUSH if (lane == 0) { for (int wpp_i = 0; wpp_i < 14; ++wpp_i) atomicAdd(&g_wp_prof[wpp_i], (unsigned long long)wpp_acc[wpp_i]); atomicAdd(&g_wp_prof[15], 1ull); }
#else
#define WPROF_DECL
#define WPROF(i)
#define WPROF_COUNT(i)
#define WPROF_FLUSH
#endif

__device__ __forceinline__ int wp_vidx(int p) { return p + (p >> 3); }
__device__ __forceinline__ double nan0(double x) { return x != x ? 0.0 : x; }
#ifdef FILO_CUSIM
__device__ __forceinline__ void wp_store_result(double* g, double v) { *g = v; }
#else
__device__ __forceinline__ void wp_store_result(double* g, double v) { __stcs(g, v); }
#endif

template <int FN>
__device__ __forceinline__ double wp_finish(double cs, int nn, double div, double rcp, double scale, int nfull, double rcpn, bool raw) {
  if (FN == FN_RATE) { const double q0 = __dmul_rn(cs, rcp); const double r = __fma_rn(-q0, div, cs); return __dmul_rn(__fma_rn(r, rcp, q0), scale); }
  if (FN == FN_COUNT) return (double)nn;
  if (FN == FN_AVG) {
    if (raw) return cs;
    if (nn == nfull) { const double q0 = __dmul_rn(cs, rcpn); const double r = __fma_rn(-q0, (double)nfull, cs); return __fma_rn(r, rcpn, q0); }
    return cs / (double)nn;
  }
  return cs;
}

template <int U>
__device__ __forceinline__ void wp_block_tail(const double* __restrict__ pa, const double* __restrict__ pb, double a[WP_R], double b[WP_R]) {
#pragma unroll
  for (int t = 0; t < 8; ++t) {
    const double va = pa[t], vb = pb[t];
#pragma unroll
    for (int w = 0; w < 8; ++w) if (w >= t - U) { a[w] += va; b[w] += vb; }
  }
#pragma unroll
  for (int t = 0; t < U; ++t) {
    const double va = pa[9 + t], vb = pb[9 + t];
#pragma unroll
    for (int w = 0; w < 8; ++w) if (w >= 8 + t - U) { a[w] += va; b[w] += vb; }
  }
}

__device__ __forceinline__ void wp_block_pair(const double* __restrict__ pa, const double* __restrict__ pb, int Wr, double a[WP_R], double b[WP_R]) {
#pragma unroll
  for (int t = 0; t < 8; ++t) {
    const double va = pa[t], vb = pb[t];
#pragma unroll
    for (int w = 0; w < t; ++w) { a[w] += va; b[w] += vb; }
    a[t] = va; b[t] = vb;
  }
  const int q = Wr >> 3;
  pa += 9; pb += 9;
  for (int m = 1; m < q; ++m, pa += 9, pb += 9) {
#pragma unroll
    for (int t = 0; t < 8; ++t) {
      const double va = pa[t], vb = pb[t];
#pragma unroll
      for (int w = 0; w < 8; ++w) { a[w] += va; b[w] += vb; }
    }
  }
  switch (Wr & 7) {
    case 0: wp_block_tail<0>(pa, pb, a, b); break;
    case 1: wp_block_tail<1>(pa, pb, a, b); break;
    case 2: wp_block_tail<2>(pa, pb, a, b); break;
    case 3: wp_block_tail<3>(pa, pb, a, b); break;
    case 4: wp_block_tail<4>(pa, pb, a, b); break;
    case 5: wp_block_tail<5>(pa, pb, a, b); break;
    case 6: wp_block_tail<6>(pa, pb, a, b); break;
    default: wp_block_tail<7>(pa, pb, a, b); break;
  }
}

struct WpParsed {
  bool regular, have, any_raw; bool irr;
  int tslope; uint32_t toff;
  int n, cLo;
  int64_t init, end_time; int nrows, num_rows, vbytes, ng, vwire, dropped, tlen, grp_base, ngroups; uint32_t voff, w12;
};
template <bool STRICT, bool IRR = false>
__device__ __forceinline__ WpParsed wp_parse(const uint8_t* R, const QueryParams& q, bool staged, int lane) {
  const unsigned FULL = 0xffffffffu;
  WpParsed P;
  bool regular = staged;
  int n = 0, cLo = 0;
  if (staged) {
    const RecordHeader* h = reinterpret_cast<const RecordHeader*>(R);
    const ChunkEntry* Eall = reinterpret_cast<const ChunkEntry*>(R + sizeof(RecordHeader));
    const int nch = (int)h->n_chunks;
    regular = nch <= 32 && (IRR || (h->flags & REC_ALL_TS_CONST) != 0);
    const int64_t t1 = q.start - q.window, t2 = q.end;
    bool below = false, within = false;
    if (regular && lane < nch) { below = Eall[lane].end_time < t1; within = !below && Eall[lane].start_time <= t2; }
    const unsigned mb = __ballot_sync(FULL, below), mw = __ballot_sync(FULL, within);
    cLo = __ffs((int)~mb) - 1; if (cLo < 0) cLo = 32;
    const unsigned rest = cLo < 32 ? (mw >> cLo) : 0u;
    n = __ffs((int)~rest) - 1; if (n < 0) n = 32;
    if (n > WP_MAXC) regular = false;
  }
  const int c = lane;
  bool have = regular && c < n;
  int64_t init = 0, end_time = 0; int nrows = 0, num_rows = 0, vbytes = 0, ng = 0, vwire = 0, dropped = 0, tlen = 0; uint32_t voff = 0, w12 = 0;
  bool okc = true, irrc = false; int slope = 0; uint32_t toff = 0;
  if (have) {
    const ChunkEntry& e = reinterpret_cast<const ChunkEntry*>(R + sizeof(RecordHeader))[cLo + c];
    const uint8_t* tv = R + e.ts_off; const uint8_t* vv = R + e.val_off;
    const uint32_t vw4 = ld32(vv + 4);
    vwire = (int)(vw4 & 0xffff); dropped = (int)((vw4 >> 31) & 1);
    toff = e.ts_off;
    const int twire = (int)(ld32(tv + 4) & 0xffff);
    if (!IRR || twire == WIRE_DDV_CONST) { tlen = (int)ld32(tv + 8); init = (int64_t)ld64_a4(tv + 12); slope = (int)ld32(tv + 20); if (IRR && twire != WIRE_DDV_CONST) okc = false; }
    else if (twire == WIRE_DDV) {
      init = (int64_t)ld64(tv + 8); slope = (int)ld32(tv + 16); tlen = int_length(tv + 20); irrc = true;
      const int nb = (int)((ld32(tv + 24) >> 16) & 0x7f);
      if (!(nb == 2 || nb == 4 || nb == 8 || nb == 16 || nb == 32)) okc = false;
    } else okc = false;
    if (IRR && (int64_t)slope != q.step) irrc = true;
    end_time = e.end_time; num_rows = e.num_rows; voff = e.val_off;
    vbytes = (int)ld32(tv) + 4 + (int)ld32(vv) + 4;
    int vlen = 0;
    if (vwire == WIRE_XOR) { vlen = (int)ld32(vv + XOR_OFF_N); w12 = ld32(vv + XOR_OFF_NGROUPS); ng = (int)(w12 & 0xffff); if (ng != (vlen + 6) / 8) okc = false; }
    else if (vwire == WIRE_RAW64) vlen = ((int)ld32(vv) - 4) / 8;
    else okc = false;
    if ((!IRR && (int64_t)slope != q.step) || slope <= 0 || tlen <= 0 || vlen <= 0 || num_rows <= 0) okc = false;
    nrows = num_rows < tlen ? num_rows : tlen;
    if (vlen != nrows) okc = false;
    if (STRICT && end_time < init + (int64_t)(nrows - 1) * q.step) okc = false;
  }
  {
    const int64_t endp = __shfl_up_sync(FULL, end_time, 1);
    if (STRICT && have && c > 0 && !(endp < init)) okc = false;
    if (!__all_sync(FULL, okc)) regular = false;
  }
  have = have && regular;
  if (!have) { ng = 0; nrows = 0; }
  int grp_base = ng;
  { const int a0 = __shfl_sync(FULL, ng, 0), a1 = __shfl_sync(FULL, ng, 1), a2 = __shfl_sync(FULL, ng, 2), a3 = __shfl_sync(FULL, ng, 3);
    grp_base = (c > 0 ? a0 : 0) + (c > 1 ? a1 : 0) + (c > 2 ? a2 : 0);
    if (a0 + a1 + a2 + a3 > WP_MAXG) regular = false; }
  P.ngroups = __shfl_sync(FULL, grp_base + ng, WP_MAXC - 1);
  P.any_raw = __any_sync(FULL, have && vwire == WIRE_RAW64);
  P.irr = IRR && __any_sync(FULL, have && irrc); P.tslope = slope; P.toff = toff;
  P.regular = regular; P.have = have && regular; P.n = n; P.cLo = cLo; P.init = init; P.end_time = end_time; P.nrows = nrows; P.num_rows = num_rows;
  P.vbytes = vbytes; P.ng = ng; P.vwire = vwire; P.dropped = dropped; P.tlen = tlen; P.grp_base = grp_base; P.voff = voff; P.w12 = w12;
  return P;
}

struct WpNoop { __device__ __forceinline__ void operator()() const {} };
template <bool DROPS, typename RDone = WpNoop>
__device__ __forceinline__ uint32_t wp_decode(const uint8_t* R, double* V, const WpChunk* CD, uint64_t* xtab, const int dd_dst[2], const int dd_inf[2],
                                              int n, bool any_raw, int lane, TileDrops* DR, RDone r_done = RDone()) {
  uint32_t okbits = 0xffffffffu;
  uint64_t d[2][8];
#pragma unroll
  for (int jj = 0; jj < 2; ++jj) {
    const bool active = dd_inf[jj] & 1;
    const WpChunk& ch = CD[(dd_inf[jj] >> 1) & 3];
    const uint8_t* gp = R;
    if (active) gp = R + ch.grp_off + reinterpret_cast<const uint16_t*>(R + ch.tab_off)[dd_inf[jj] >> 8];
    const uint32_t mask = active ? gp[0] : 0u;
    const uint32_t hdr = gp[1];
    const uint32_t numBits = ((hdr >> 4) + 1) * 4;
    const uint32_t tz = (hdr & 0x0f) * 4;
    const uint64_t fm = (~0ull >> (64 - numBits)) << tz;
    uint32_t xb = (wp_soff(gp + 2) << 3) - tz;
    uint64_t x = 0;
#pragma unroll
    for (int i = 0; i < 8; ++i) {
      const bool on = (mask >> i) & 1u;
      const uint32_t wa = (xb >> 3) & ~3u;
      const uint32_t w0 = wp_lds32(wa), w1 = wp_lds32(wa + 4), w2 = wp_lds32(wa + 8);
      const uint32_t lo = __funnelshift_r(w0, w1, xb), hi = __funnelshift_r(w1, w2, xb);
      const uint64_t f = on ? fm : 0ull;
      x ^= (((uint64_t)hi << 32) | lo) & f;
      xb += on ? numBits : 0u;
      d[jj][i] = x;
    }
  }
  if (!any_raw) r_done();
  uint64_t i0x = d[0][7], i1x = d[1][7];
#pragma unroll
  for (int o = 1; o < 32; o <<= 1) {
    const uint64_t y0 = shfl_up_u64(i0x, o), y1 = shfl_up_u64(i1x, o);
    if (lane >= o) { i0x ^= y0; i1x ^= y1; }
  }
  const uint64_t tot0 = shfl_u64(i0x, 31);
  const uint64_t ex0 = i0x ^ d[0][7], ex1 = i1x ^ d[1][7] ^ tot0;
  xtab[lane] = ex0; xtab[32 + lane] = ex1;
  __syncwarp();
#pragma unroll
  for (int jj = 0; jj < 2; ++jj) {
    const bool active = dd_inf[jj] & 1;
    const int ci = (dd_inf[jj] >> 1) & 3;
    const WpChunk& ch = CD[ci];
    const uint64_t pre = ch.first ^ (jj ? ex1 : ex0) ^ xtab[active ? ch.grp_base : 0];
    uint64_t* dst = reinterpret_cast<uint64_t*>(V) + dd_dst[jj];
    const int t = (dd_inf[jj] >> 3) & 7;
    if (active) {
#pragma unroll
      for (int i = 0; i < 8; ++i) {
        const uint64_t b = d[jj][i] ^ pre;
        dst[i + ((t + i) >> 3)] = b;
        const uint32_t h = (uint32_t)(b >> 32);
        okbits &= h ^ (h << 1);
      }
      if ((dd_inf[jj] >> 8) == 0) { dst[t == 0 ? -2 : -1] = ch.first; const uint32_t h = (uint32_t)(ch.first >> 32); okbits &= h ^ (h << 1); }
      if (DROPS && ch.dropped) {
        const int g = dd_inf[jj] >> 8;
        const int nleft = ch.nrows - 1 - g * 8;
        double prevv = nan0(__longlong_as_double((long long)pre));
        TileDrops& D = DR[ci];
#pragma unroll
        for (int i = 0; i < 8; ++i) {
          const double cur = nan0(__longlong_as_double((long long)(d[jj][i] ^ pre)));
          if (i < nleft && cur < prevv) {
            const int at = atomicAdd(&D.n, 1);
            if (at < TILE_MAXDROP) { D.pos[at] = 1 + g * 8 + i; D.amt[at] = prevv; }
          }
          prevv = cur;
        }
      }
    }
  }
  for (int ci = 0; any_raw && ci < n; ++ci) {
    const WpChunk& ch = CD[ci];
    if (ch.wire != WIRE_RAW64) continue;
    const uint64_t* src = reinterpret_cast<const uint64_t*>(R + ch.val_off + 8);
    const bool drp = DROPS && ch.dropped;
    for (int r = lane; r < ch.nrows; r += 32) {
      const uint64_t b = src[r];
      reinterpret_cast<uint64_t*>(V)[wp_vidx(ch.rowpos + r)] = b;
      const uint32_t h = (uint32_t)(b >> 32);
      okbits &= h ^ (h << 1);
      if (drp && r > 0) {
        const double cur = nan0(__longlong_as_double((long long)b)), prevv = nan0(__longlong_as_double((long long)src[r - 1]));
        if (cur < prevv) { TileDrops& D = DR[ci]; const int at = atomicAdd(&D.n, 1); if (at < TILE_MAXDROP) { D.pos[at] = r; D.amt[at] = prevv; } }
      }
    }
  }
  if (any_raw) r_done();
  return okbits;
}

constexpr uint32_t WP_FINAL = 0, WP_RAWFIN = 1, WP_JUNC = 2, WP_GAP = 3;
__device__ __forceinline__ int wp_chunk_of(const WpChunk* CD, int n, int k) {
  int ci = -1;
  for (int c = 0; c < n; ++c) if (CD[c].nblk > 0 && k >= CD[c].kT0) ci = c;
  return ci;
}
__device__ __forceinline__ uint32_t wp_class(const WpChunk* CD, int n, int k, uint32_t& jslot) {
  const int ci = wp_chunk_of(CD, n, k);
  jslot = 0;
  if (ci < 0 || k > CD[ci].kT1) return WP_GAP;
  const WpChunk& ch = CD[ci];
  const int i = k - ch.kT0;
  if (i < ch.jzb * WP_R) { jslot = (uint32_t)(ch.joff + i) | (i < ch.hs ? 128u : 0u); return WP_JUNC; }
  return i >= ch.tb * WP_R ? WP_RAWFIN : WP_FINAL;
}
__device__ __forceinline__ int wp_rows_in(const WpChunk& x, int k, int Wr) {
  int lo = x.s0 + k; if (lo < 0) lo = 0; int hi = x.s0 + k + Wr; if (hi > x.nrows - 1) hi = x.nrows - 1;
  return hi - lo + 1;
}

__device__ __forceinline__ void wp_item(const WpChunk* CD, const WpSmem& L, int it, int items, int psi, int& pp, int& op, int& inf) {
  const bool active = it < items;
  int ci = 0;
  if (CD[1].nblk > 0 && it >= CD[1].blk0) ci = 1;
  if (CD[2].nblk > 0 && it >= CD[2].blk0) ci = 2;
  if (CD[3].nblk > 0 && it >= CD[3].blk0) ci = 3;
  const WpChunk& ch = CD[ci];
  const int b = active ? it - ch.blk0 : 0;
  const int k0 = ch.kT0 + WP_R * b;
  pp = ch.vidx0 + 9 * b;
  const bool tojz = b < ch.jzb;
  const bool raw = tojz || b >= ch.tb;
  op = tojz ? (int)WP_OFF_J + 8 * (ch.joff + WP_R * b) : (int)L.out + 8 * (k0 + ((k0 + psi) >> 3));
  int jEnd = !active ? -1 : tojz ? WP_R - 1 : ch.kT1 - k0;
  if (jEnd > WP_R - 1) jEnd = WP_R - 1;
  const int ot = tojz ? 0 : (k0 + psi) & 7;
  inf = (jEnd + 1) | ((raw ? 1 : 0) << 4) | (ot << 5) | (ci << 8) | (k0 << 10);
}

template <int FN, int NW>
__global__ void __launch_bounds__(NW * 32, 1)
scan_wp_sum_kernel(const uint8_t* __restrict__ arena, const int64_t* __restrict__ rec_off, int64_t n_series, QueryParams q,
                   double* __restrict__ out, WpSmem L, int64_t* __restrict__ fallback_list, unsigned long long* __restrict__ fallback_count,
                   unsigned long long* d_counters, int* d_err) {
  extern __shared__ __align__(128) uint8_t smem[];
  const unsigned FULL = 0xffffffffu;
  const int lane = threadIdx.x & 31, warp = threadIdx.x >> 5;
  uint8_t* wb = smem + (size_t)warp * L.per_warp;
  uint64_t* bar = reinterpret_cast<uint64_t*>(wb);
  WpChunk* CD = reinterpret_cast<WpChunk*>(wb + WP_OFF_DESC);
  uint64_t* xtab = reinterpret_cast<uint64_t*>(wb + WP_OFF_J);
  double* J = reinterpret_cast<double*>(wb + WP_OFF_J);
  const bool two = L.rec2 != 0;
  uint8_t* R = wb + WP_OFF_REC;
  double* V = reinterpret_cast<double*>(wb + L.vals);
  double* O = reinterpret_cast<double*>(wb + L.out);
  const int64_t nwarps = (int64_t)gridDim.x * (blockDim.x >> 5);
  int64_t s = (int64_t)blockIdx.x * (blockDim.x >> 5) + warp;
  if (lane == 0) { mbar_init(bar, 1); if (two) mbar_init(bar + 1, 1); mbar_fence_init(); }
  __syncwarp();

  int64_t winDur = q.inclusive ? q.window : q.window - 1; if (winDur < 0) winDur = 0;
  const double fdiv = (double)(q.inclusive ? winDur : winDur + 1), frcp = 1.0 / fdiv;
  const int64_t S0 = q.start - winDur, E0 = q.start;
  const int64_t lastEnd = q.start + (int64_t)(q.T - 1) * q.step;
  StepDiv sd; sd.init(q.step);
  const double NaNv = __longlong_as_double(0x7ff8000000000000LL);

  int64_t m_init = 0, m_end = 0; int m_nrows = -1, m_n = -1, m_wire = -1; bool m_ok = false;
  int dd_dst[2] = {0, 0}, dd_inf[2] = {0, 0}, wi_pp[2] = {0, 0}, wi_op[2] = {0, 0}, wi_inf[2] = {0, 0};
  int gz[3] = {-1, -1, -1}; bool gz_all = true;
  int p_Wr = 0, p_items = 0, p_nfull = 0, p_psi = 0; double p_rcpn = 0.0; bool p_oal = false;
  uint32_t p_cls = 0; uint64_t p_jx = 0;
  int64_t rows_scanned = 0, bytes_scanned = 0;
  uint32_t parity = 0;

  auto issue = [&](int64_t off, uint32_t sz) {
    uint64_t* b = bar + (R == wb + WP_OFF_REC ? 0 : 1);
    mbar_expect_tx(b, sz);
    tma_load_1d(R, arena + off, sz, b);
  };
  uint32_t cur_sz = 0, nb_sz = 0;
  int64_t cur_off = 0;
  if (s < n_series) { cur_off = rec_off[s]; cur_sz = (uint32_t)(rec_off[s + 1] - cur_off); }
  if (s < n_series && cur_sz <= L.rec_cap && lane == 0) issue(cur_off, cur_sz);
  if (two && s + nwarps < n_series) {
    const int64_t o1 = rec_off[s + nwarps]; nb_sz = (uint32_t)(rec_off[s + nwarps + 1] - o1);
    R = wb + L.rec2;
    if (nb_sz <= L.rec_cap && lane == 0) issue(o1, nb_sz);
    R = wb + WP_OFF_REC;
  }
  uint32_t stage = 0;
  WPROF_DECL

  for (; s < n_series; s += nwarps) {
    const int64_t sn = s + (two ? 2 : 1) * nwarps;
    int64_t nxt_off = 0; uint32_t nxt_end = 0;
    if (sn < n_series) { nxt_off = rec_off[sn]; nxt_end = (uint32_t)rec_off[sn + 1]; }
    const bool staged = cur_sz <= L.rec_cap;
    WPROF_COUNT(10)
    WPROF(9)
    if (staged) { mbar_wait(bar + stage, (parity >> stage) & 1u); parity ^= 1u << stage; }
    WPROF(0)
    const WpParsed P = wp_parse<true>(R, q, staged, lane);
    const uint32_t nxt_sz = nxt_end - (uint32_t)nxt_off;
    WPROF(1)
    bool regular = P.regular;
    const bool have = P.have; const int n = P.n, c = lane;
    const int64_t init = P.init, end_time = P.end_time;
    const int nrows = P.nrows, num_rows = P.num_rows, vbytes = P.vbytes, ng = P.ng, vwire = P.vwire, grp_base = P.grp_base, ngroups = P.ngroups;
    const uint32_t voff = P.voff, w12 = P.w12; const bool any_raw = P.any_raw;
    const bool samec = !(c < n) || (init == m_init && nrows == m_nrows && end_time == m_end && vwire == m_wire);
    const bool same_all = __all_sync(FULL, samec);
    const bool same = m_ok && n == m_n && same_all;
    if (regular && !same) {
      WPROF_COUNT(11)
      m_init = init; m_end = end_time; m_nrows = nrows; m_n = n; m_wire = vwire; m_ok = false;
      int64_t s0 = 0, e0 = 0;
      if (have) { s0 = sd.ceil_div(S0 - init); e0 = sd.floor_div(E0 - init); }
      const int Wr = (int)(e0 - s0);
      int64_t kT0 = -e0; if (kT0 < 0) kT0 = 0;
      int64_t kT1 = (int64_t)(nrows - 1) - s0; if (kT1 > q.T - 1) kT1 = q.T - 1;
      const bool touch = have && kT0 <= kT1;
      if (!touch) { kT0 = 0x3fffffff; kT1 = -1; }
      const int Wr0 = __shfl_sync(FULL, Wr, 0);
      bool okp = !have || Wr == Wr0;
      if (Wr0 < 8 || (uint32_t)Wr0 + 1 > L.jcap) okp = false;
      const unsigned tm = __ballot_sync(FULL, touch) & 0xfu;
      if (tm != 0) { const unsigned lowbit = tm & (0u - tm); const unsigned filled = tm + lowbit; if ((filled & (filled - 1)) != 0) okp = false; }
      const int64_t kT1p = __shfl_up_sync(FULL, kT1, 1), kT1pp = __shfl_up_sync(FULL, kT1, 2), kT0n = __shfl_down_sync(FULL, kT0, 1);
      const bool prev_t = c > 0 && ((tm >> (c - 1)) & 1u), next_t = c + 1 < WP_MAXC && ((tm >> (c + 1)) & 1u);
      if (touch && c >= 2 && ((tm >> (c - 2)) & 1u) && !(kT1pp < kT0)) okp = false;
      int64_t ownLo = kT0, ownHi = kT1;
      if (touch && prev_t && kT1p + 1 > ownLo) ownLo = kT1p + 1;
      if (touch && next_t && kT0n - 1 < ownHi) ownHi = kT0n - 1;
      const int hs = touch ? (int)(ownLo - kT0) : 0;
      const int nblk = touch ? (int)((kT1 - kT0 + WP_R) / WP_R) : 0;
      const int jzb = (hs + WP_R - 1) / WP_R;
      const int tb = (touch && ownHi < kT1) ? (int)((ownHi + 1 - kT0) / WP_R) : nblk;
      if (touch && jzb > tb) okp = false;
      int blk0, items, joff, jtot;
      { const int a0 = __shfl_sync(FULL, nblk, 0), a1 = __shfl_sync(FULL, nblk, 1), a2 = __shfl_sync(FULL, nblk, 2), a3 = __shfl_sync(FULL, nblk, 3);
        blk0 = (c > 0 ? a0 : 0) + (c > 1 ? a1 : 0) + (c > 2 ? a2 : 0); items = a0 + a1 + a2 + a3; }
      { const int z = jzb * WP_R;
        const int a0 = __shfl_sync(FULL, z, 0), a1 = __shfl_sync(FULL, z, 1), a2 = __shfl_sync(FULL, z, 2), a3 = __shfl_sync(FULL, z, 3);
        joff = (c > 0 ? a0 : 0) + (c > 1 ? a1 : 0) + (c > 2 ? a2 : 0); jtot = a0 + a1 + a2 + a3; }
      if ((uint32_t)jtot > L.jcap) okp = false;
      if (L.alias && items > 64) okp = false;
      const int fr = touch ? (int)(s0 + kT0) : 0;
      int rowpos = 0;
      {
        int base = 0;
#pragma unroll
        for (int cc = 0; cc < WP_MAXC; ++cc) {
          int x;
          if (cc == 0) { x = fr < 0 ? -fr : ((8 - (fr & 7)) & 7); }
          else { x = base + ((-(base + fr)) & 7); }
          if (c == cc) rowpos = x;
          const int nb = __shfl_sync(FULL, x + nrows + Wr0, cc);
          base = nb;
        }
      }
      const int pend = __shfl_sync(FULL, rowpos + nrows, n > 0 ? n - 1 : 0) + Wr0 + 8;
      if ((uint32_t)(pend + (pend >> 3) + 2) > L.vcap) okp = false;
      if (!__all_sync(FULL, okp)) regular = false;
      if (regular) {
        if (c < WP_MAXC) {
          WpChunk& d = CD[c];
          d.kT0 = (int)kT0; d.kT1 = (int)kT1; d.ownLo = (int)ownLo; d.ownHi = (int)ownHi; d.blk0 = blk0; d.nblk = nblk;
          d.vidx0 = wp_vidx(rowpos + fr); d.rowpos = rowpos; d.nrows = nrows; d.s0 = (int)s0; d.e0 = (int)e0; d.joff = joff; d.hs = hs; d.jzb = jzb; d.tb = tb;
        }
        { const int first_t = tm ? __ffs((int)tm) - 1 : 0;
          p_psi = (-(int)__shfl_sync(FULL, (int)(touch ? kT0 : 0), first_t)) & 7;
          p_oal = __all_sync(FULL, !touch || (((int)kT0 + p_psi) & 7) == 0); }
        p_Wr = Wr0; p_items = items; p_nfull = Wr0 + 1; p_rcpn = 1.0 / (double)(Wr0 + 1);
        __syncwarp();
        {
          int tot = 0;
          gz[0] = gz[1] = gz[2] = -1;
          for (int g = 0; g <= n; ++g) {
            const int g0 = g == 0 ? 0 : CD[g - 1].rowpos + CD[g - 1].nrows;
            const int g1 = g == n ? pend : CD[g].rowpos;
#pragma unroll
            for (int u = 0; u < 3; ++u) { const int i = u * 32 + lane - tot; if (i >= 0 && i < g1 - g0) gz[u] = wp_vidx(g0 + i); }
            tot += g1 - g0;
          }
          gz_all = tot <= 96;
        }
        {
          uint32_t cls = 0; uint64_t jx = 0; int nj = 0;
#pragma unroll 1
          for (int m = 0; m < 16 && lane + 32 * m < q.T; ++m) {
            uint32_t js;
            const uint32_t code = wp_class(CD, n, lane + 32 * m, js);
            cls |= code << (2 * m);
            if (code == WP_JUNC) { jx |= (uint64_t)js << (8 * nj); ++nj; }
          }
          p_cls = cls; p_jx = jx;
        }
        {
          const int gb1 = __shfl_sync(FULL, have ? grp_base : 0x7fffffff, 1), gb2 = __shfl_sync(FULL, have ? grp_base : 0x7fffffff, 2),
                    gb3 = __shfl_sync(FULL, have ? grp_base : 0x7fffffff, 3);
#pragma unroll
          for (int jj = 0; jj < 2; ++jj) {
            const int slot = jj * 32 + lane;
            const bool active = slot < ngroups;
            const int ci = active ? (slot >= gb1 ? 1 : 0) + (slot >= gb2 ? 1 : 0) + (slot >= gb3 ? 1 : 0) : 0;
            const int gbc = ci == 0 ? 0 : ci == 1 ? gb1 : ci == 2 ? gb2 : gb3;
            const int g = active ? slot - gbc : 0;
            const int pq = CD[ci].rowpos + 1 + g * 8;
            dd_dst[jj] = wp_vidx(pq);
            dd_inf[jj] = (active ? 1 : 0) | (ci << 1) | ((pq & 7) << 3) | (g << 8);
          }
#pragma unroll
          for (int X = 0; X < 2; ++X) wp_item(CD, L, X * 32 + lane, items, p_psi, wi_pp[X], wi_op[X], wi_inf[X]);
        }
        m_ok = true;
      }
    }
    WPROF(2)
    if (!regular) {
      WPROF_COUNT(12)
      if (lane == 0) { const unsigned long long slot = atomicAdd(fallback_count, 1ull); fallback_list[slot] = s; }
      __syncwarp();
      if (sn < n_series && nxt_sz <= L.rec_cap && lane == 0) issue(nxt_off, nxt_sz);
      if (two) { cur_sz = nb_sz; nb_sz = nxt_sz; stage ^= 1u; R = wb + (stage ? L.rec2 : WP_OFF_REC); } else cur_sz = nxt_sz;
      continue;
    }
    if (c < WP_MAXC) {
      WpChunk& d = CD[c];
      d.grp_base = have ? grp_base : 0x7fffffff; d.ng = ng; d.wire = vwire; d.val_off = voff; d.dropped = P.dropped;
      if (have && vwire == WIRE_XOR) { const uint32_t po = w12 >> 16; d.first = ld64(R + voff + po); d.grp_off = voff + po + 8; d.tab_off = voff + XOR_OFF_GROUPTAB; }
      else { d.first = have ? ld64(R + voff + 8) : 0ull; d.grp_off = 0; d.tab_off = 0; }
    }
    int cnt_rows = 0, cnt_bytes = 0;
    { const int64_t endp = __shfl_up_sync(FULL, end_time, 1);
      if (have && !(c > 0 && !(endp < lastEnd))) { cnt_rows = num_rows; cnt_bytes = vbytes; } }
#pragma unroll
    for (int o = 1; o < WP_MAXC; o <<= 1) { cnt_rows += __shfl_xor_sync(FULL, cnt_rows, o); cnt_bytes += __shfl_xor_sync(FULL, cnt_bytes, o); }
    __syncwarp();
    WPROF(3)
    auto rec_done = [&]() {
      __syncwarp();
      if (sn < n_series && nxt_sz <= L.rec_cap && lane == 0) issue(nxt_off, nxt_sz);
    };
    const uint32_t okbits = wp_decode<false>(R, V, CD, xtab, dd_dst, dd_inf, n, any_raw, lane, nullptr, rec_done);
    const bool vals_ok = __all_sync(FULL, (okbits >> 30) & 1u);
    __syncwarp();
    if (two) { cur_sz = nb_sz; nb_sz = nxt_sz; stage ^= 1u; R = wb + (stage ? L.rec2 : WP_OFF_REC); } else cur_sz = nxt_sz;
    WPROF(4)
    if (gz_all) {
#pragma unroll
      for (int u = 0; u < 3; ++u) if (gz[u] >= 0) V[gz[u]] = 0.0;
    } else {
      const int pend = CD[n - 1].rowpos + CD[n - 1].nrows + p_Wr + 8;
      for (int g = 0; g <= n; ++g) {
        const int g0 = g == 0 ? 0 : CD[g - 1].rowpos + CD[g - 1].nrows;
        const int g1 = g == n ? pend : CD[g].rowpos;
        for (int pz = g0 + lane; pz < g1; pz += 32) V[wp_vidx(pz)] = 0.0;
      }
    }
    WPROF(5)
    if (!vals_ok) {
      WPROF_COUNT(13)
      if (lane == 0) { const unsigned long long slot = atomicAdd(fallback_count, 1ull); fallback_list[slot] = s; }
      __syncwarp();
      continue;
    }
    if (lane == 0) { rows_scanned += cnt_rows; bytes_scanned += cnt_bytes; }
    __syncwarp();
    const int psi = p_psi;
    auto oidx = [&](int k) -> int { return k + ((k + psi) >> 3); };
    {
      const int Wr = p_Wr;
      for (int it0 = 0; it0 < p_items; it0 += 64) {
        int ipp[2], iop[2], iinf[2];
#pragma unroll
        for (int X = 0; X < 2; ++X) {
          if (it0 == 0) { ipp[X] = wi_pp[X]; iop[X] = wi_op[X]; iinf[X] = wi_inf[X]; }
          else wp_item(CD, L, it0 + X * 32 + lane, p_items, psi, ipp[X], iop[X], iinf[X]);
        }
        const double* pp[2]; double* op[2]; int jEnd[2], ot[2]; bool rawm[2];
#pragma unroll
        for (int X = 0; X < 2; ++X) {
          pp[X] = V + ipp[X]; op[X] = reinterpret_cast<double*>(wb + iop[X]);
          jEnd[X] = (iinf[X] & 15) - 1; rawm[X] = (iinf[X] >> 4) & 1; ot[X] = (iinf[X] >> 5) & 7;
        }
        double a[WP_R], bb[WP_R];
        wp_block_pair(pp[0], pp[1], Wr, a, bb);
        __syncwarp();
#pragma unroll
        for (int X = 0; X < 2; ++X) {
          const double dv = rawm[X] ? 1.0 : fdiv, rc = rawm[X] ? 1.0 : frcp, sc = rawm[X] ? 1.0 : 1000.0;
#pragma unroll
          for (int j = 0; j < WP_R; ++j) {
            const double raw = X ? bb[j] : a[j];
            int nn = 1;
            if (FN == FN_AVG || FN == FN_COUNT) {
              const WpChunk& ch = CD[(iinf[X] >> 8) & 3];
              int lo = ch.s0 + (iinf[X] >> 10) + j; const int hi0 = lo + Wr; if (lo < 0) lo = 0;
              const int hi = hi0 > ch.nrows - 1 ? ch.nrows - 1 : hi0;
              nn = hi - lo + 1;
            }
            const double fin = wp_finish<FN>(raw, nn, dv, rc, sc, p_nfull, p_rcpn, rawm[X]);
            if (X) bb[j] = fin; else a[j] = fin;
          }
        }
        if (p_oal) {
#pragma unroll
          for (int j = 0; j < WP_R; ++j) { if (j <= jEnd[0]) op[0][j] = a[j]; if (j <= jEnd[1]) op[1][j] = bb[j]; }
        } else {
#pragma unroll
          for (int j = 0; j < WP_R; ++j) {
            if (j <= jEnd[0]) op[0][j + ((ot[0] + j) >> 3)] = a[j];
            if (j <= jEnd[1]) op[1][j + ((ot[1] + j) >> 3)] = bb[j];
          }
        }
      }
      __syncwarp();
      WPROF(6)
      double* gp = out + (size_t)s * q.T + lane;
      const double* sp = O + oidx(lane);
      auto fin = [&](double o, uint32_t code, uint32_t js, int k) -> double {
        double v = o;
        if (code == WP_JUNC) { const double jv = J[js & 127u]; v = (js & 128u) ? o + jv : jv; }
        double r;
        if (FN == FN_COUNT) r = v;
        else {
          int nn = 1;
          if (FN == FN_AVG && (code == WP_RAWFIN || code == WP_JUNC)) {
            const int ci = wp_chunk_of(CD, n, k);
            nn = wp_rows_in(CD[ci], k, Wr);
            if (code == WP_JUNC && (js & 128u)) nn += wp_rows_in(CD[ci - 1], k, Wr);
          }
          r = wp_finish<FN>(v, nn, fdiv, frcp, 1000.0, p_nfull, p_rcpn, false);
        }
        return code == WP_FINAL ? o : code == WP_GAP ? NaNv : r;
      };
      uint32_t cls = p_cls; uint64_t jx = p_jx;
      auto fin_m = [&](double o, int k) -> double {
        const uint32_t code = cls & 3u, js = (uint32_t)jx & 0xffu;
        cls >>= 2;
        if (code == WP_JUNC) jx >>= 8;
        return fin(o, code, js, k);
      };
      int k = lane, iters = (q.T - lane + 31) >> 5;
      int rest = iters > 16 ? iters - 16 : 0;
      if (rest) iters = 16;
      for (; iters >= 4; iters -= 4, gp += 128, sp += 144, k += 128) {
        const double v0 = sp[0], v1 = sp[36], v2 = sp[72], v3 = sp[108];
        const double r0 = fin_m(v0, k), r1 = fin_m(v1, k + 32), r2 = fin_m(v2, k + 64), r3 = fin_m(v3, k + 96);
        wp_store_result(gp, r0); wp_store_result(gp + 32, r1); wp_store_result(gp + 64, r2); wp_store_result(gp + 96, r3);
      }
      for (; iters > 0; --iters, gp += 32, sp += 36, k += 32) wp_store_result(gp, fin_m(*sp, k));
      for (; rest > 0; --rest, gp += 32, sp += 36, k += 32) {
        uint32_t js;
        const uint32_t code = wp_class(CD, n, k, js);
        wp_store_result(gp, fin(*sp, code, js, k));
      }
    }
    __syncwarp();
    WPROF(7)
  }
  WPROF(9)
  WPROF_FLUSH
  if (lane == 0) {
    if (rows_scanned | bytes_scanned) { atomicAdd(&d_counters[0], (unsigned long long)rows_scanned); atomicAdd(&d_counters[1], (unsigned long long)bytes_scanned); }
  }
}

}
```

### filodb_b200/csrc/scan_wp_layout.h

```cpp
#pragma once
#include <stdint.h>
#include "filo_record.h"
#include "scan_params.h"
#include "scan_tile_layout.h"
namespace filo {
constexpr int WP_MAXC = 4;
constexpr int WP_MAXG = 64;
constexpr int WP_R = 8;
constexpr int WP_MAX_WARPS = 16;
constexpr int WP_MAX_WARPS_ALIAS = 20;

struct WpChunk {
  uint64_t first;
  int32_t kT0, kT1;
  int32_t ownLo, ownHi;
  int32_t blk0, nblk;
  int32_t vidx0;
  int32_t rowpos;
  int32_t nrows, s0, e0;
  int32_t grp_base, ng, wire;
  uint32_t grp_off, tab_off, val_off;
  int32_t joff, hs;
  int32_t jzb, tb;
  int32_t dropped;
};
static_assert(sizeof(WpChunk) == 96, "WpChunk");

constexpr uint32_t WP_OFF_DESC = 16, WP_OFF_J = WP_OFF_DESC + WP_MAXC * 96, WP_J_DOUBLES = 128, WP_OFF_REC = WP_OFF_J + WP_J_DOUBLES * 8;
struct WpSmem {
  uint32_t desc, jbuf, rec, vals, out, per_warp;
  uint32_t rec_cap, vcap , jcap , ocap ;
  uint32_t warps;
  uint32_t alias;
  uint32_t rec2;
};
FILO_HD inline WpSmem wp_layout(uint32_t max_rec_bytes, uint32_t max_rows, uint32_t max_chunks, uint32_t T, uint32_t wrows, bool alias, bool two_rec = false) {
  WpSmem L;
  if (max_chunks > (uint32_t)WP_MAXC) max_chunks = WP_MAXC;
  L.rec_cap = align_up(max_rec_bytes + 16, 16);
  const uint32_t P = max_rows + (max_chunks + 1) * (wrows + 7) + 16;
  L.vcap = align_up(P + P / 8 + 2, 2);
  L.jcap = WP_J_DOUBLES;
  (void)wrows;
  L.ocap = align_up(T + T / 8 + 4, 2);
  if (alias && L.vcap < L.ocap) L.vcap = L.ocap;
  static_assert(sizeof(WpChunk) == 96, "WP_OFF_J");
  uint32_t o = WP_OFF_REC;
  L.desc = WP_OFF_DESC; L.jbuf = WP_OFF_J;
  L.rec = o; o += L.rec_cap;
  L.rec2 = 0;
  if (two_rec) { L.rec2 = o; o += L.rec_cap; }
  L.vals = o; o += L.vcap * 8;
  if (alias) L.out = L.vals; else { L.out = o; o += L.ocap * 8; }
  L.per_warp = align_up(o, 16);
  L.warps = 0;
  L.alias = alias ? 1u : 0u;
  return L;
}
FILO_HD inline uint32_t wp_max_items(uint32_t max_chunks, uint32_t T, uint32_t wrows) {
  if (max_chunks > (uint32_t)WP_MAXC) max_chunks = WP_MAXC;
  if (max_chunks == 0) max_chunks = 1;
  return (T + (max_chunks - 1) * (wrows - 1) + 7 * max_chunks) / 8;
}

constexpr int WP_CTR_MAX_WARPS = 20;
struct TileCtr {
  double dTS, thr, half, endpart, sI, ratio0, skipC;
  int32_t dropped, pad;
};
constexpr int TILE_MAXDROP = 8;
constexpr int TILE_CTR_TABMAX = 64;
struct TileCtrTab { double sI, thr, half, rcpSI; };
struct TileDrops {
  int32_t n, pos[TILE_MAXDROP], pad[3];
  double amt[TILE_MAXDROP];
};
struct WpCtrChunk {
  int64_t init, end_time;
  int32_t nrows, s0, e0, rowpos;
  int32_t kA, kB;
  int32_t kA2, kB2;
  TileCtr kc;
};
static_assert(sizeof(WpCtrChunk) == 112, "WpCtrChunk");

struct WpCtrSmem {
  uint32_t vals, kc, acc, nbad, per_warp, tab ;
  uint32_t rec_cap, vcap , warps, agg;
  uint32_t tsr;
};
constexpr uint32_t WP_OFF_DROPS = WP_OFF_J + 64 * 8;
static_assert(WP_OFF_DROPS + WP_MAXC * sizeof(TileDrops) <= WP_OFF_REC, "drops fit in front of the record");
FILO_HD inline WpCtrSmem wp_ctr_layout(uint32_t max_rec_bytes, uint32_t max_rows, uint32_t max_chunks, uint32_t T, bool agg, bool irr = false,
                                       bool moments = false) {
  WpCtrSmem L;
  if (max_chunks > (uint32_t)WP_MAXC) max_chunks = WP_MAXC;
  L.rec_cap = align_up(max_rec_bytes + 16, 16);
  const uint32_t P = max_rows + 8 * max_chunks + 8;
  L.vcap = align_up(P + P / 8 + 2, 2);
  uint32_t o = WP_OFF_REC + L.rec_cap;
  L.vals = o; o += L.vcap * 8;
  L.kc = o; o += (uint32_t)(WP_MAXC * sizeof(WpCtrChunk));
  L.tsr = 0;
  if (irr) { L.tsr = o; o += align_up(P * 4, 16); }
  L.acc = o; L.nbad = o;
  if (agg) { o += T * 8; L.nbad = o; o += align_up(T * 2, 16); }
  if (agg && moments) o += T * 8;
  L.per_warp = align_up(o, 16);
  L.tab = 0; L.warps = 0; L.agg = agg ? 1u : 0u;
  return L;
}
FILO_HD inline bool wp_ctr_tile_footprint_ok(uint32_t max_rec_bytes, uint32_t max_rows, uint32_t T, uint64_t cap) {
  const uint32_t ctr = 2 * align_up(TILE_NS * TILE_MAXC * (uint32_t)sizeof(TileCtr), 128) + align_up(TILE_NS * TILE_MAXC * (uint32_t)sizeof(TileDrops), 128) +
                       align_up((TILE_CTR_TABMAX + 1) * (uint32_t)sizeof(TileCtrTab), 128);
  return (uint64_t)(tile_layout(max_rec_bytes, max_rows, T, 0).total + ctr) + 1024 <= cap;
}

}
```

### scratch/wp_prof.py

```python
import ctypes as C
import os
import sys

import numpy as np

HERE = os.path.dirname(os.path.abspath(__file__))
sys.path.insert(0, os.path.dirname(HERE))
import filodb_b200.capi as capi
capi.LIB_PATH = os.environ.get("FILO_LIB_PATH") or os.path.join(HERE, "libfilo_b200_wp_prof.so")
import bench

workload = sys.argv[1] if len(sys.argv) > 1 else "c2"
series = sys.argv[2] if len(sys.argv) > 2 else "5000000"
L = capi.lib()
L.filo_debug_wp_prof.argtypes = [C.c_void_p, C.c_int]
out = np.zeros(16, np.uint64)
sys.argv = ["bench.py", "--workload", workload, "--series", series, "--steps", "4", "--warmup", "2", "--no-e2e", "--no-cpu", "--no-extra", "--no-c5"]
L.filo_debug_wp_prof(out.ctypes.data, 1)
bench.main()
L.filo_debug_wp_prof(out.ctypes.data, 0)
names = ["wait: record (mbarrier)", "parse", "memo check (+ window plan on a miss)", "per-series descriptors, scan counters", "decode",
         "zero rows", "window blocks", "finish and store (earlier: fix-up, gaps)", None, "loop head, declined series"]
ns = float(out[10])
tot = float(out[:10].sum())
print("scan_wp_sum_kernel: %d warps, %d series taken up, %d memo misses, %d declined by the plan, %d declined by the values"
      % (int(out[15]), int(ns), int(out[11]), int(out[12]), int(out[13])))
print("  %-40s %10s %7s" % ("phase", "cyc/series", "share"))
for i, n in enumerate(names):
    if n is None:
        if out[i] == 0:
            continue
        n = "result row (earlier builds)"
    print("  %-40s %10.1f %6.1f %%" % (n, float(out[i]) / ns, 100.0 * float(out[i]) / tot))
print("  %-40s %10.1f" % ("total", tot / ns))
```

Baseline: 151.8 billion.

## Add producer/consumer batched warp-per-series scan kernel with staged record buffers

Adds a new scan kernel in which one producer warp per CTA copies batches of series records into double-buffered shared memory and pre-parses chunk headers into entry tables. Fifteen consumer warps wait on mbarriers, then plan, decode and window-aggregate from those entries. The host now prefers this path when the shared-memory layout fits. The goal is to overlap record loading and parsing with decode and aggregation and to move per-series header parsing off the consumer warps. In exchange it spends a whole warp on production, adds barrier synchronisation, and uses more shared memory per CTA.

Result: faster. 160.2 billion (median of 6 runs) (+5.5%).

```diff
diff --git a/filodb_b200/csrc/capi.cu b/filodb_b200/csrc/capi.cu
--- a/filodb_b200/csrc/capi.cu
+++ b/filodb_b200/csrc/capi.cu
@@ -864,13 +864,18 @@
     use_tile = (size_t)TL.total + 1024 <= smem_cap;
   }
   WpSmem WL{};
-  bool use_wp = false;
+  WpBatchSmem WB{};
+  bool use_wp = false, use_wp_batch = false;
   if (use_tile && force != "v3" && wrows <= 4096 && t->max_chunks > 0) {
     const bool alias = wp_max_items((uint32_t)t->max_chunks, (uint32_t)q.T, (uint32_t)wrows) <= 64;
     WL = wp_layout(t->max_rec_bytes, (uint32_t)t->max_rows, (uint32_t)t->max_chunks, (uint32_t)q.T, (uint32_t)wrows, alias);
     WL.warps = (uint32_t)std::min<size_t>(smem_cap / WL.per_warp, alias ? WP_MAX_WARPS_ALIAS : WP_MAX_WARPS);
     const WpSmem WL2 = wp_layout(t->max_rec_bytes, (uint32_t)t->max_rows, (uint32_t)t->max_chunks, (uint32_t)q.T, (uint32_t)wrows, alias, true);
-    if (smem_cap / WL2.per_warp >= (size_t)WP_MAX_WARPS) { WL = WL2; WL.warps = WP_MAX_WARPS; }
+    if (smem_cap / WL2.per_warp >= (size_t)WP_MAX_WARPS) {
+      WL = WL2; WL.warps = WP_MAX_WARPS;
+      WB = wp_batch_layout(t->max_rec_bytes, (uint32_t)t->max_rows, (uint32_t)t->max_chunks, (uint32_t)q.T, (uint32_t)wrows, alias);
+      use_wp_batch = WB.total <= smem_cap;
+    }
     use_wp = WL.warps >= 4;
   }
   WpCtrSmem WC{};
@@ -890,7 +895,10 @@
       CUDA_TRY(ctx, cudaMemsetAsync(d_cnt, 0, 16, s));
       ScanLaunch LT = L;
       static const bool dbg = std::getenv("FILO_DEBUG_SYNC") != nullptr;
-      if (use_wp) {
+      if (use_wp_batch) {
+        LT.grid = (int)std::max<int64_t>(1, std::min<int64_t>((t->n_series + WB.B - 1) / WB.B, (int64_t)ctx->sm_count));
+        CUDA_TRY(ctx, launch_scan_wp_batch(LT, outp, WB, d_list, d_cnt));
+      } else if (use_wp) {
         LT.grid = (int)std::max<int64_t>(1, std::min<int64_t>((t->n_series + WL.warps - 1) / WL.warps, (int64_t)ctx->sm_count));
         CUDA_TRY(ctx, launch_scan_wp(LT, outp, WL, d_list, d_cnt));
       } else if (use_wp_ctr) {
diff --git a/filodb_b200/csrc/kernels.h b/filodb_b200/csrc/kernels.h
--- a/filodb_b200/csrc/kernels.h
+++ b/filodb_b200/csrc/kernels.h
@@ -49,6 +49,8 @@
                         double* out_val, int64_t* out_id, cudaStream_t s);
 struct WpSmem;
 cudaError_t launch_scan_wp(const ScanLaunch& L, double* out, const WpSmem& W, int64_t* fallback_list, unsigned long long* fallback_count);
+struct WpBatchSmem;
+cudaError_t launch_scan_wp_batch(const ScanLaunch& L, double* out, const WpBatchSmem& W, int64_t* fallback_list, unsigned long long* fallback_count);
 struct WpCtrSmem;
 cudaError_t launch_scan_wp_ctr(const ScanLaunch& L, double* out, const WpCtrSmem& W, int64_t* fallback_list, unsigned long long* fallback_count);
 cudaError_t launch_scan_wp_ctr_agg(const ScanLaunch& L, const WpCtrSmem& W, const int32_t* order, const int64_t* item_begin, int64_t n_items, int agg_op,
diff --git a/filodb_b200/csrc/scan_kernels.cu b/filodb_b200/csrc/scan_kernels.cu
--- a/filodb_b200/csrc/scan_kernels.cu
+++ b/filodb_b200/csrc/scan_kernels.cu
@@ -389,9 +389,9 @@
 }
 #endif
 #ifdef FILO_WP_PROF
-extern "C" int filo_debug_wp_prof(unsigned long long* out16, int reset) {
-  cudaError_t e = cudaMemcpyFromSymbol(out16, g_wp_prof, sizeof(unsigned long long) * 16);
-  if (e == cudaSuccess && reset) { unsigned long long z[16] = {}; e = cudaMemcpyToSymbol(g_wp_prof, z, sizeof z); }
+extern "C" int filo_debug_wp_prof(unsigned long long* out32, int reset) {
+  cudaError_t e = cudaMemcpyFromSymbol(out32, g_wp_prof, sizeof(unsigned long long) * 32);
+  if (e == cudaSuccess && reset) { unsigned long long z[32] = {}; e = cudaMemcpyToSymbol(g_wp_prof, z, sizeof z); }
   return (int)e;
 }
 #endif
@@ -487,6 +487,22 @@
     default: return launch_wp_fn<FN_SUM>(L, out, W, fallback_list, fallback_count);
   }
 }
+template <int FN>
+static cudaError_t launch_wp_batch_fn(const ScanLaunch& L, double* out, const WpBatchSmem& W, int64_t* fallback_list, unsigned long long* fallback_count) {
+  cudaError_t e = cudaFuncSetAttribute(scan_wp_batch_kernel<FN, WP_BATCH_WARPS>, cudaFuncAttributeMaxDynamicSharedMemorySize, (int)W.total);
+  if (e != cudaSuccess) return e;
+  scan_wp_batch_kernel<FN, WP_BATCH_WARPS><<<L.grid, WP_BATCH_WARPS * 32, W.total, L.stream>>>(L.arena, L.rec_off, L.n_series, L.q, out, W, fallback_list,
+      fallback_count, L.d_counters, L.d_err);
+  return cudaGetLastError();
+}
+cudaError_t launch_scan_wp_batch(const ScanLaunch& L, double* out, const WpBatchSmem& W, int64_t* fallback_list, unsigned long long* fallback_count) {
+  switch (L.q.fn) {
+    case FN_RATE: return launch_wp_batch_fn<FN_RATE>(L, out, W, fallback_list, fallback_count);
+    case FN_AVG: return launch_wp_batch_fn<FN_AVG>(L, out, W, fallback_list, fallback_count);
+    case FN_COUNT: return launch_wp_batch_fn<FN_COUNT>(L, out, W, fallback_list, fallback_count);
+    default: return launch_wp_batch_fn<FN_SUM>(L, out, W, fallback_list, fallback_count);
+  }
+}
 template <int FN, bool AGG, int NW, bool IRR, bool MOM>
 static cudaError_t launch_wp_ctr_nw(const ScanLaunch& L, double* out, const WpCtrSmem& W, int64_t* fallback_list, unsigned long long* fallback_count,
                                     const TileAggArgs& A) {
diff --git a/filodb_b200/csrc/scan_wp.cuh b/filodb_b200/csrc/scan_wp.cuh
--- a/filodb_b200/csrc/scan_wp.cuh
+++ b/filodb_b200/csrc/scan_wp.cuh
@@ -13,7 +13,7 @@
 #endif
 
 #if defined(FILO_WP_PROF) && !defined(FILO_CUSIM)
-__device__ unsigned long long g_wp_prof[16];
+__device__ unsigned long long g_wp_prof[32];
 #define WPROF_DECL uint32_t wpp_t0 = (uint32_t)clock(), wpp_acc[14] = {0, 0, 0, 0, 0, 0, 0, 0, 0, 0, 0, 0, 0, 0};
 #define WPROF(i) { const uint32_t wpp_t1 = (uint32_t)clock(); wpp_acc[i] += wpp_t1 - wpp_t0; wpp_t0 = wpp_t1; }
 #define WPROF_COUNT(i) { ++wpp_acc[i]; }
@@ -97,6 +97,34 @@
   int n, cLo;
   int64_t init, end_time; int nrows, num_rows, vbytes, ng, vwire, dropped, tlen, grp_base, ngroups; uint32_t voff, w12;
 };
+template <bool STRICT, bool IRR>
+__device__ __forceinline__ void wp_chunk_fields(const uint8_t* R, const ChunkEntry& e, const QueryParams& q, int64_t& init, int64_t& end_time, int& nrows,
+                                                int& num_rows, int& vbytes, int& ng, int& vwire, int& dropped, int& tlen, uint32_t& voff, uint32_t& w12,
+                                                bool& okc, bool& irrc, int& slope, uint32_t& toff) {
+  const uint8_t* tv = R + e.ts_off; const uint8_t* vv = R + e.val_off;
+  const uint32_t vw4 = ld32(vv + 4);
+  vwire = (int)(vw4 & 0xffff); dropped = (int)((vw4 >> 31) & 1);
+  toff = e.ts_off;
+  const int twire = (int)(ld32(tv + 4) & 0xffff);
+  if (!IRR || twire == WIRE_DDV_CONST) { tlen = (int)ld32(tv + 8); init = (int64_t)ld64_a4(tv + 12); slope = (int)ld32(tv + 20); if (IRR && twire != WIRE_DDV_CONST) okc = false; }
+  else if (twire == WIRE_DDV) {
+    init = (int64_t)ld64(tv + 8); slope = (int)ld32(tv + 16); tlen = int_length(tv + 20); irrc = true;
+    const int nb = (int)((ld32(tv + 24) >> 16) & 0x7f);
+    if (!(nb == 2 || nb == 4 || nb == 8 || nb == 16 || nb == 32)) okc = false;
+  } else okc = false;
+  if (IRR && (int64_t)slope != q.step) irrc = true;
+  end_time = e.end_time; num_rows = e.num_rows; voff = e.val_off;
+  vbytes = (int)ld32(tv) + 4 + (int)ld32(vv) + 4;
+  int vlen = 0;
+  if (vwire == WIRE_XOR) { vlen = (int)ld32(vv + XOR_OFF_N); w12 = ld32(vv + XOR_OFF_NGROUPS); ng = (int)(w12 & 0xffff); if (ng != (vlen + 6) / 8) okc = false; }
+  else if (vwire == WIRE_RAW64) vlen = ((int)ld32(vv) - 4) / 8;
+  else okc = false;
+  if ((!IRR && (int64_t)slope != q.step) || slope <= 0 || tlen <= 0 || vlen <= 0 || num_rows <= 0) okc = false;
+  nrows = num_rows < tlen ? num_rows : tlen;
+  if (vlen != nrows) okc = false;
+  if (STRICT && end_time < init + (int64_t)(nrows - 1) * q.step) okc = false;
+}
+
 template <bool STRICT, bool IRR = false>
 __device__ __forceinline__ WpParsed wp_parse(const uint8_t* R, const QueryParams& q, bool staged, int lane) {
   const unsigned FULL = 0xffffffffu;
@@ -121,31 +149,9 @@
   bool have = regular && c < n;
   int64_t init = 0, end_time = 0; int nrows = 0, num_rows = 0, vbytes = 0, ng = 0, vwire = 0, dropped = 0, tlen = 0; uint32_t voff = 0, w12 = 0;
   bool okc = true, irrc = false; int slope = 0; uint32_t toff = 0;
-  if (have) {
-    const ChunkEntry& e = reinterpret_cast<const ChunkEntry*>(R + sizeof(RecordHeader))[cLo + c];
-    const uint8_t* tv = R + e.ts_off; const uint8_t* vv = R + e.val_off;
-    const uint32_t vw4 = ld32(vv + 4);
-    vwire = (int)(vw4 & 0xffff); dropped = (int)((vw4 >> 31) & 1);
-    toff = e.ts_off;
-    const int twire = (int)(ld32(tv + 4) & 0xffff);
-    if (!IRR || twire == WIRE_DDV_CONST) { tlen = (int)ld32(tv + 8); init = (int64_t)ld64_a4(tv + 12); slope = (int)ld32(tv + 20); if (IRR && twire != WIRE_DDV_CONST) okc = false; }
-    else if (twire == WIRE_DDV) {
-      init = (int64_t)ld64(tv + 8); slope = (int)ld32(tv + 16); tlen = int_length(tv + 20); irrc = true;
-      const int nb = (int)((ld32(tv + 24) >> 16) & 0x7f);
-      if (!(nb == 2 || nb == 4 || nb == 8 || nb == 16 || nb == 32)) okc = false;
-    } else okc = false;
-    if (IRR && (int64_t)slope != q.step) irrc = true;
-    end_time = e.end_time; num_rows = e.num_rows; voff = e.val_off;
-    vbytes = (int)ld32(tv) + 4 + (int)ld32(vv) + 4;
-    int vlen = 0;
-    if (vwire == WIRE_XOR) { vlen = (int)ld32(vv + XOR_OFF_N); w12 = ld32(vv + XOR_OFF_NGROUPS); ng = (int)(w12 & 0xffff); if (ng != (vlen + 6) / 8) okc = false; }
-    else if (vwire == WIRE_RAW64) vlen = ((int)ld32(vv) - 4) / 8;
-    else okc = false;
-    if ((!IRR && (int64_t)slope != q.step) || slope <= 0 || tlen <= 0 || vlen <= 0 || num_rows <= 0) okc = false;
-    nrows = num_rows < tlen ? num_rows : tlen;
-    if (vlen != nrows) okc = false;
-    if (STRICT && end_time < init + (int64_t)(nrows - 1) * q.step) okc = false;
-  }
+  if (have)
+    wp_chunk_fields<STRICT, IRR>(R, reinterpret_cast<const ChunkEntry*>(R + sizeof(RecordHeader))[cLo + c], q, init, end_time, nrows, num_rows, vbytes, ng,
+                                 vwire, dropped, tlen, voff, w12, okc, irrc, slope, toff);
   {
     const int64_t endp = __shfl_up_sync(FULL, end_time, 1);
     if (STRICT && have && c > 0 && !(endp < init)) okc = false;
@@ -298,6 +304,263 @@
   if (jEnd > WP_R - 1) jEnd = WP_R - 1;
   const int ot = tojz ? 0 : (k0 + psi) & 7;
   inf = (jEnd + 1) | ((raw ? 1 : 0) << 4) | (ot << 5) | (ci << 8) | (k0 << 10);
+}
+
+struct WpQuery {
+  double fdiv, frcp;
+  int64_t S0, E0, lastEnd;
+  StepDiv sd;
+  __device__ __forceinline__ void init(const QueryParams& q) {
+    int64_t winDur = q.inclusive ? q.window : q.window - 1; if (winDur < 0) winDur = 0;
+    fdiv = (double)(q.inclusive ? winDur : winDur + 1); frcp = 1.0 / fdiv;
+    S0 = q.start - winDur; E0 = q.start;
+    lastEnd = q.start + (int64_t)(q.T - 1) * q.step;
+    sd.init(q.step);
+  }
+};
+struct WpPlan {
+  int64_t m_init = 0, m_end = 0; int m_nrows = -1, m_n = -1, m_wire = -1; bool m_ok = false;
+  int dd_dst[2] = {0, 0}, dd_inf[2] = {0, 0}, wi_pp[2] = {0, 0}, wi_op[2] = {0, 0}, wi_inf[2] = {0, 0};
+  int gz[3] = {-1, -1, -1}; bool gz_all = true;
+  int p_Wr = 0, p_items = 0, p_nfull = 0, p_psi = 0; double p_rcpn = 0.0; bool p_oal = false;
+  uint32_t p_cls = 0; uint64_t p_jx = 0;
+};
+
+__device__ __forceinline__ bool wp_plan_series(WpPlan& M, bool& regular, bool have, int n, int64_t init, int64_t end_time, int nrows, int vwire,
+                                               int grp_base, int ngroups, const QueryParams& q, const WpSmem& L, const WpQuery& Q, WpChunk* CD, int lane) {
+  const unsigned FULL = 0xffffffffu;
+  const int c = lane;
+  const bool samec = !(c < n) || (init == M.m_init && nrows == M.m_nrows && end_time == M.m_end && vwire == M.m_wire);
+  const bool same_all = __all_sync(FULL, samec);
+  const bool same = M.m_ok && n == M.m_n && same_all;
+  const bool miss = regular && !same;
+  if (miss) {
+    M.m_init = init; M.m_end = end_time; M.m_nrows = nrows; M.m_n = n; M.m_wire = vwire; M.m_ok = false;
+    int64_t s0 = 0, e0 = 0;
+    if (have) { s0 = Q.sd.ceil_div(Q.S0 - init); e0 = Q.sd.floor_div(Q.E0 - init); }
+    const int Wr = (int)(e0 - s0);
+    int64_t kT0 = -e0; if (kT0 < 0) kT0 = 0;
+    int64_t kT1 = (int64_t)(nrows - 1) - s0; if (kT1 > q.T - 1) kT1 = q.T - 1;
+    const bool touch = have && kT0 <= kT1;
+    if (!touch) { kT0 = 0x3fffffff; kT1 = -1; }
+    const int Wr0 = __shfl_sync(FULL, Wr, 0);
+    bool okp = !have || Wr == Wr0;
+    if (Wr0 < 8 || (uint32_t)Wr0 + 1 > L.jcap) okp = false;
+    const unsigned tm = __ballot_sync(FULL, touch) & 0xfu;
+    if (tm != 0) { const unsigned lowbit = tm & (0u - tm); const unsigned filled = tm + lowbit; if ((filled & (filled - 1)) != 0) okp = false; }
+    const int64_t kT1p = __shfl_up_sync(FULL, kT1, 1), kT1pp = __shfl_up_sync(FULL, kT1, 2), kT0n = __shfl_down_sync(FULL, kT0, 1);
+    const bool prev_t = c > 0 && ((tm >> (c - 1)) & 1u), next_t = c + 1 < WP_MAXC && ((tm >> (c + 1)) & 1u);
+    if (touch && c >= 2 && ((tm >> (c - 2)) & 1u) && !(kT1pp < kT0)) okp = false;
+    int64_t ownLo = kT0, ownHi = kT1;
+    if (touch && prev_t && kT1p + 1 > ownLo) ownLo = kT1p + 1;
+    if (touch && next_t && kT0n - 1 < ownHi) ownHi = kT0n - 1;
+    const int hs = touch ? (int)(ownLo - kT0) : 0;
+    const int nblk = touch ? (int)((kT1 - kT0 + WP_R) / WP_R) : 0;
+    const int jzb = (hs + WP_R - 1) / WP_R;
+    const int tb = (touch && ownHi < kT1) ? (int)((ownHi + 1 - kT0) / WP_R) : nblk;
+    if (touch && jzb > tb) okp = false;
+    int blk0, items, joff, jtot;
+    { const int a0 = __shfl_sync(FULL, nblk, 0), a1 = __shfl_sync(FULL, nblk, 1), a2 = __shfl_sync(FULL, nblk, 2), a3 = __shfl_sync(FULL, nblk, 3);
+      blk0 = (c > 0 ? a0 : 0) + (c > 1 ? a1 : 0) + (c > 2 ? a2 : 0); items = a0 + a1 + a2 + a3; }
+    { const int z = jzb * WP_R;
+      const int a0 = __shfl_sync(FULL, z, 0), a1 = __shfl_sync(FULL, z, 1), a2 = __shfl_sync(FULL, z, 2), a3 = __shfl_sync(FULL, z, 3);
+      joff = (c > 0 ? a0 : 0) + (c > 1 ? a1 : 0) + (c > 2 ? a2 : 0); jtot = a0 + a1 + a2 + a3; }
+    if ((uint32_t)jtot > L.jcap) okp = false;
+    if (L.alias && items > 64) okp = false;
+    const int fr = touch ? (int)(s0 + kT0) : 0;
+    int rowpos = 0;
+    {
+      int base = 0;
+#pragma unroll
+      for (int cc = 0; cc < WP_MAXC; ++cc) {
+        int x;
+        if (cc == 0) { x = fr < 0 ? -fr : ((8 - (fr & 7)) & 7); }
+        else { x = base + ((-(base + fr)) & 7); }
+        if (c == cc) rowpos = x;
+        const int nb = __shfl_sync(FULL, x + nrows + Wr0, cc);
+        base = nb;
+      }
+    }
+    const int pend = __shfl_sync(FULL, rowpos + nrows, n > 0 ? n - 1 : 0) + Wr0 + 8;
+    if ((uint32_t)(pend + (pend >> 3) + 2) > L.vcap) okp = false;
+    if (!__all_sync(FULL, okp)) regular = false;
+    if (regular) {
+      if (c < WP_MAXC) {
+        WpChunk& d = CD[c];
+        d.kT0 = (int)kT0; d.kT1 = (int)kT1; d.ownLo = (int)ownLo; d.ownHi = (int)ownHi; d.blk0 = blk0; d.nblk = nblk;
+        d.vidx0 = wp_vidx(rowpos + fr); d.rowpos = rowpos; d.nrows = nrows; d.s0 = (int)s0; d.e0 = (int)e0; d.joff = joff; d.hs = hs; d.jzb = jzb; d.tb = tb;
+      }
+      { const int first_t = tm ? __ffs((int)tm) - 1 : 0;
+        M.p_psi = (-(int)__shfl_sync(FULL, (int)(touch ? kT0 : 0), first_t)) & 7;
+        M.p_oal = __all_sync(FULL, !touch || (((int)kT0 + M.p_psi) & 7) == 0); }
+      M.p_Wr = Wr0; M.p_items = items; M.p_nfull = Wr0 + 1; M.p_rcpn = 1.0 / (double)(Wr0 + 1);
+      __syncwarp();
+      {
+        int tot = 0;
+        M.gz[0] = M.gz[1] = M.gz[2] = -1;
+        for (int g = 0; g <= n; ++g) {
+          const int g0 = g == 0 ? 0 : CD[g - 1].rowpos + CD[g - 1].nrows;
+          const int g1 = g == n ? pend : CD[g].rowpos;
+#pragma unroll
+          for (int u = 0; u < 3; ++u) { const int i = u * 32 + lane - tot; if (i >= 0 && i < g1 - g0) M.gz[u] = wp_vidx(g0 + i); }
+          tot += g1 - g0;
+        }
+        M.gz_all = tot <= 96;
+      }
+      {
+        uint32_t cls = 0; uint64_t jx = 0; int nj = 0;
+#pragma unroll 1
+        for (int m = 0; m < 16 && lane + 32 * m < q.T; ++m) {
+          uint32_t js;
+          const uint32_t code = wp_class(CD, n, lane + 32 * m, js);
+          cls |= code << (2 * m);
+          if (code == WP_JUNC) { jx |= (uint64_t)js << (8 * nj); ++nj; }
+        }
+        M.p_cls = cls; M.p_jx = jx;
+      }
+      {
+        const int gb1 = __shfl_sync(FULL, have ? grp_base : 0x7fffffff, 1), gb2 = __shfl_sync(FULL, have ? grp_base : 0x7fffffff, 2),
+                  gb3 = __shfl_sync(FULL, have ? grp_base : 0x7fffffff, 3);
+#pragma unroll
+        for (int jj = 0; jj < 2; ++jj) {
+          const int slot = jj * 32 + lane;
+          const bool active = slot < ngroups;
+          const int ci = active ? (slot >= gb1 ? 1 : 0) + (slot >= gb2 ? 1 : 0) + (slot >= gb3 ? 1 : 0) : 0;
+          const int gbc = ci == 0 ? 0 : ci == 1 ? gb1 : ci == 2 ? gb2 : gb3;
+          const int g = active ? slot - gbc : 0;
+          const int pq = CD[ci].rowpos + 1 + g * 8;
+          M.dd_dst[jj] = wp_vidx(pq);
+          M.dd_inf[jj] = (active ? 1 : 0) | (ci << 1) | ((pq & 7) << 3) | (g << 8);
+        }
+#pragma unroll
+        for (int X = 0; X < 2; ++X) wp_item(CD, L, X * 32 + lane, items, M.p_psi, M.wi_pp[X], M.wi_op[X], M.wi_inf[X]);
+      }
+      M.m_ok = true;
+    }
+  }
+  return miss;
+}
+
+__device__ __forceinline__ void wp_zero_rows(double* V, const WpChunk* CD, int n, const WpPlan& M, int lane) {
+  if (M.gz_all) {
+#pragma unroll
+    for (int u = 0; u < 3; ++u) if (M.gz[u] >= 0) V[M.gz[u]] = 0.0;
+  } else {
+    const int pend = CD[n - 1].rowpos + CD[n - 1].nrows + M.p_Wr + 8;
+    for (int g = 0; g <= n; ++g) {
+      const int g0 = g == 0 ? 0 : CD[g - 1].rowpos + CD[g - 1].nrows;
+      const int g1 = g == n ? pend : CD[g].rowpos;
+      for (int pz = g0 + lane; pz < g1; pz += 32) V[wp_vidx(pz)] = 0.0;
+    }
+  }
+}
+
+template <int FN>
+__device__ __forceinline__ void wp_window_blocks(const double* V, uint8_t* wb, const WpChunk* CD, const WpSmem& L, const WpPlan& M, const WpQuery& Q,
+                                                 int lane) {
+  const int psi = M.p_psi;
+  const int Wr = M.p_Wr;
+  for (int it0 = 0; it0 < M.p_items; it0 += 64) {
+    int ipp[2], iop[2], iinf[2];
+#pragma unroll
+    for (int X = 0; X < 2; ++X) {
+      if (it0 == 0) { ipp[X] = M.wi_pp[X]; iop[X] = M.wi_op[X]; iinf[X] = M.wi_inf[X]; }
+      else wp_item(CD, L, it0 + X * 32 + lane, M.p_items, psi, ipp[X], iop[X], iinf[X]);
+    }
+    const double* pp[2]; double* op[2]; int jEnd[2], ot[2]; bool rawm[2];
+#pragma unroll
+    for (int X = 0; X < 2; ++X) {
+      pp[X] = V + ipp[X]; op[X] = reinterpret_cast<double*>(wb + iop[X]);
+      jEnd[X] = (iinf[X] & 15) - 1; rawm[X] = (iinf[X] >> 4) & 1; ot[X] = (iinf[X] >> 5) & 7;
+    }
+    double a[WP_R], bb[WP_R];
+    wp_block_pair(pp[0], pp[1], Wr, a, bb);
+    __syncwarp();
+#pragma unroll
+    for (int X = 0; X < 2; ++X) {
+      const double dv = rawm[X] ? 1.0 : Q.fdiv, rc = rawm[X] ? 1.0 : Q.frcp, sc = rawm[X] ? 1.0 : 1000.0;
+#pragma unroll
+      for (int j = 0; j < WP_R; ++j) {
+        const double raw = X ? bb[j] : a[j];
+        int nn = 1;
+        if (FN == FN_AVG || FN == FN_COUNT) {
+          const WpChunk& ch = CD[(iinf[X] >> 8) & 3];
+          int lo = ch.s0 + (iinf[X] >> 10) + j; const int hi0 = lo + Wr; if (lo < 0) lo = 0;
+          const int hi = hi0 > ch.nrows - 1 ? ch.nrows - 1 : hi0;
+          nn = hi - lo + 1;
+        }
+        const double fin = wp_finish<FN>(raw, nn, dv, rc, sc, M.p_nfull, M.p_rcpn, rawm[X]);
+        if (X) bb[j] = fin; else a[j] = fin;
+      }
+    }
+    if (M.p_oal) {
+#pragma unroll
+      for (int j = 0; j < WP_R; ++j) { if (j <= jEnd[0]) op[0][j] = a[j]; if (j <= jEnd[1]) op[1][j] = bb[j]; }
+    } else {
+#pragma unroll
+      for (int j = 0; j < WP_R; ++j) {
+        if (j <= jEnd[0]) op[0][j + ((ot[0] + j) >> 3)] = a[j];
+        if (j <= jEnd[1]) op[1][j + ((ot[1] + j) >> 3)] = bb[j];
+      }
+    }
+  }
+  __syncwarp();
+}
+
+template <int FN>
+__device__ __forceinline__ void wp_finish_store(double* __restrict__ out, int64_t s, const QueryParams& q, const double* O, const double* J,
+                                                const WpChunk* CD, int n, const WpPlan& M, const WpQuery& Q, int lane) {
+  const double NaNv = __longlong_as_double(0x7ff8000000000000LL);
+  const int psi = M.p_psi, Wr = M.p_Wr;
+  auto oidx = [&](int k) -> int { return k + ((k + psi) >> 3); };
+  double* gp = out + (size_t)s * q.T + lane;
+  const double* sp = O + oidx(lane);
+  auto fin = [&](double o, uint32_t code, uint32_t js, int k) -> double {
+    double v = o;
+    if (code == WP_JUNC) { const double jv = J[js & 127u]; v = (js & 128u) ? o + jv : jv; }
+    double r;
+    if (FN == FN_COUNT) r = v;
+    else {
+      int nn = 1;
+      if (FN == FN_AVG && (code == WP_RAWFIN || code == WP_JUNC)) {
+        const int ci = wp_chunk_of(CD, n, k);
+        nn = wp_rows_in(CD[ci], k, Wr);
+        if (code == WP_JUNC && (js & 128u)) nn += wp_rows_in(CD[ci - 1], k, Wr);
+      }
+      r = wp_finish<FN>(v, nn, Q.fdiv, Q.frcp, 1000.0, M.p_nfull, M.p_rcpn, false);
+    }
+    return code == WP_FINAL ? o : code == WP_GAP ? NaNv : r;
+  };
+  uint32_t cls = M.p_cls; uint64_t jx = M.p_jx;
+  auto fin_m = [&](double o, int k) -> double {
+    const uint32_t code = cls & 3u, js = (uint32_t)jx & 0xffu;
+    cls >>= 2;
+    if (code == WP_JUNC) jx >>= 8;
+    return fin(o, code, js, k);
+  };
+  int k = lane, iters = (q.T - lane + 31) >> 5;
+  int rest = iters > 16 ? iters - 16 : 0;
+  if (rest) iters = 16;
+  for (; iters >= 4; iters -= 4, gp += 128, sp += 144, k += 128) {
+    const double v0 = sp[0], v1 = sp[36], v2 = sp[72], v3 = sp[108];
+    const double r0 = fin_m(v0, k), r1 = fin_m(v1, k + 32), r2 = fin_m(v2, k + 64), r3 = fin_m(v3, k + 96);
+    wp_store_result(gp, r0); wp_store_result(gp + 32, r1); wp_store_result(gp + 64, r2); wp_store_result(gp + 96, r3);
+  }
+  for (; iters > 0; --iters, gp += 32, sp += 36, k += 32) wp_store_result(gp, fin_m(*sp, k));
+  for (; rest > 0; --rest, gp += 32, sp += 36, k += 32) {
+    uint32_t js;
+    const uint32_t code = wp_class(CD, n, k, js);
+    wp_store_result(gp, fin(*sp, code, js, k));
+  }
+}
+
+__device__ __forceinline__ void wp_series_desc(WpChunk* CD, int c, bool have, int grp_base, int ng, int vwire, uint32_t voff, int dropped, uint64_t first,
+                                               uint32_t grp_off, uint32_t tab_off) {
+  if (c < WP_MAXC) {
+    WpChunk& d = CD[c];
+    d.grp_base = have ? grp_base : 0x7fffffff; d.ng = ng; d.wire = vwire; d.val_off = voff; d.dropped = dropped;
+    d.first = first; d.grp_off = grp_off; d.tab_off = tab_off;
+  }
 }
 
 template <int FN, int NW>
@@ -322,18 +585,8 @@
   if (lane == 0) { mbar_init(bar, 1); if (two) mbar_init(bar + 1, 1); mbar_fence_init(); }
   __syncwarp();
 
-  int64_t winDur = q.inclusive ? q.window : q.window - 1; if (winDur < 0) winDur = 0;
-  const double fdiv = (double)(q.inclusive ? winDur : winDur + 1), frcp = 1.0 / fdiv;
-  const int64_t S0 = q.start - winDur, E0 = q.start;
-  const int64_t lastEnd = q.start + (int64_t)(q.T - 1) * q.step;
-  StepDiv sd; sd.init(q.step);
-  const double NaNv = __longlong_as_double(0x7ff8000000000000LL);
-
-  int64_t m_init = 0, m_end = 0; int m_nrows = -1, m_n = -1, m_wire = -1; bool m_ok = false;
-  int dd_dst[2] = {0, 0}, dd_inf[2] = {0, 0}, wi_pp[2] = {0, 0}, wi_op[2] = {0, 0}, wi_inf[2] = {0, 0};
-  int gz[3] = {-1, -1, -1}; bool gz_all = true;
-  int p_Wr = 0, p_items = 0, p_nfull = 0, p_psi = 0; double p_rcpn = 0.0; bool p_oal = false;
-  uint32_t p_cls = 0; uint64_t p_jx = 0;
+  WpQuery Q; Q.init(q);
+  WpPlan M;
   int64_t rows_scanned = 0, bytes_scanned = 0;
   uint32_t parity = 0;
 
@@ -369,117 +622,7 @@
     WPROF(1)
     bool regular = P.regular;
     const bool have = P.have; const int n = P.n, c = lane;
-    const int64_t init = P.init, end_time = P.end_time;
-    const int nrows = P.nrows, num_rows = P.num_rows, vbytes = P.vbytes, ng = P.ng, vwire = P.vwire, grp_base = P.grp_base, ngroups = P.ngroups;
-    const uint32_t voff = P.voff, w12 = P.w12; const bool any_raw = P.any_raw;
-    const bool samec = !(c < n) || (init == m_init && nrows == m_nrows && end_time == m_end && vwire == m_wire);
-    const bool same_all = __all_sync(FULL, samec);
-    const bool same = m_ok && n == m_n && same_all;
-    if (regular && !same) {
-      WPROF_COUNT(11)
-      m_init = init; m_end = end_time; m_nrows = nrows; m_n = n; m_wire = vwire; m_ok = false;
-      int64_t s0 = 0, e0 = 0;
-      if (have) { s0 = sd.ceil_div(S0 - init); e0 = sd.floor_div(E0 - init); }
-      const int Wr = (int)(e0 - s0);
-      int64_t kT0 = -e0; if (kT0 < 0) kT0 = 0;
-      int64_t kT1 = (int64_t)(nrows - 1) - s0; if (kT1 > q.T - 1) kT1 = q.T - 1;
-      const bool touch = have && kT0 <= kT1;
-      if (!touch) { kT0 = 0x3fffffff; kT1 = -1; }
-      const int Wr0 = __shfl_sync(FULL, Wr, 0);
-      bool okp = !have || Wr == Wr0;
-      if (Wr0 < 8 || (uint32_t)Wr0 + 1 > L.jcap) okp = false;
-      const unsigned tm = __ballot_sync(FULL, touch) & 0xfu;
-      if (tm != 0) { const unsigned lowbit = tm & (0u - tm); const unsigned filled = tm + lowbit; if ((filled & (filled - 1)) != 0) okp = false; }
-      const int64_t kT1p = __shfl_up_sync(FULL, kT1, 1), kT1pp = __shfl_up_sync(FULL, kT1, 2), kT0n = __shfl_down_sync(FULL, kT0, 1);
-      const bool prev_t = c > 0 && ((tm >> (c - 1)) & 1u), next_t = c + 1 < WP_MAXC && ((tm >> (c + 1)) & 1u);
-      if (touch && c >= 2 && ((tm >> (c - 2)) & 1u) && !(kT1pp < kT0)) okp = false;
-      int64_t ownLo = kT0, ownHi = kT1;
-      if (touch && prev_t && kT1p + 1 > ownLo) ownLo = kT1p + 1;
-      if (touch && next_t && kT0n - 1 < ownHi) ownHi = kT0n - 1;
-      const int hs = touch ? (int)(ownLo - kT0) : 0;
-      const int nblk = touch ? (int)((kT1 - kT0 + WP_R) / WP_R) : 0;
-      const int jzb = (hs + WP_R - 1) / WP_R;
-      const int tb = (touch && ownHi < kT1) ? (int)((ownHi + 1 - kT0) / WP_R) : nblk;
-      if (touch && jzb > tb) okp = false;
-      int blk0, items, joff, jtot;
-      { const int a0 = __shfl_sync(FULL, nblk, 0), a1 = __shfl_sync(FULL, nblk, 1), a2 = __shfl_sync(FULL, nblk, 2), a3 = __shfl_sync(FULL, nblk, 3);
-        blk0 = (c > 0 ? a0 : 0) + (c > 1 ? a1 : 0) + (c > 2 ? a2 : 0); items = a0 + a1 + a2 + a3; }
-      { const int z = jzb * WP_R;
-        const int a0 = __shfl_sync(FULL, z, 0), a1 = __shfl_sync(FULL, z, 1), a2 = __shfl_sync(FULL, z, 2), a3 = __shfl_sync(FULL, z, 3);
-        joff = (c > 0 ? a0 : 0) + (c > 1 ? a1 : 0) + (c > 2 ? a2 : 0); jtot = a0 + a1 + a2 + a3; }
-      if ((uint32_t)jtot > L.jcap) okp = false;
-      if (L.alias && items > 64) okp = false;
-      const int fr = touch ? (int)(s0 + kT0) : 0;
-      int rowpos = 0;
-      {
-        int base = 0;
-#pragma unroll
-        for (int cc = 0; cc < WP_MAXC; ++cc) {
-          int x;
-          if (cc == 0) { x = fr < 0 ? -fr : ((8 - (fr & 7)) & 7); }
-          else { x = base + ((-(base + fr)) & 7); }
-          if (c == cc) rowpos = x;
-          const int nb = __shfl_sync(FULL, x + nrows + Wr0, cc);
-          base = nb;
-        }
-      }
-      const int pend = __shfl_sync(FULL, rowpos + nrows, n > 0 ? n - 1 : 0) + Wr0 + 8;
-      if ((uint32_t)(pend + (pend >> 3) + 2) > L.vcap) okp = false;
-      if (!__all_sync(FULL, okp)) regular = false;
-      if (regular) {
-        if (c < WP_MAXC) {
-          WpChunk& d = CD[c];
-          d.kT0 = (int)kT0; d.kT1 = (int)kT1; d.ownLo = (int)ownLo; d.ownHi = (int)ownHi; d.blk0 = blk0; d.nblk = nblk;
-          d.vidx0 = wp_vidx(rowpos + fr); d.rowpos = rowpos; d.nrows = nrows; d.s0 = (int)s0; d.e0 = (int)e0; d.joff = joff; d.hs = hs; d.jzb = jzb; d.tb = tb;
-        }
-        { const int first_t = tm ? __ffs((int)tm) - 1 : 0;
-          p_psi = (-(int)__shfl_sync(FULL, (int)(touch ? kT0 : 0), first_t)) & 7;
-          p_oal = __all_sync(FULL, !touch || (((int)kT0 + p_psi) & 7) == 0); }
-        p_Wr = Wr0; p_items = items; p_nfull = Wr0 + 1; p_rcpn = 1.0 / (double)(Wr0 + 1);
-        __syncwarp();
-        {
-          int tot = 0;
-          gz[0] = gz[1] = gz[2] = -1;
-          for (int g = 0; g <= n; ++g) {
-            const int g0 = g == 0 ? 0 : CD[g - 1].rowpos + CD[g - 1].nrows;
-            const int g1 = g == n ? pend : CD[g].rowpos;
-#pragma unroll
-            for (int u = 0; u < 3; ++u) { const int i = u * 32 + lane - tot; if (i >= 0 && i < g1 - g0) gz[u] = wp_vidx(g0 + i); }
-            tot += g1 - g0;
-          }
-          gz_all = tot <= 96;
-        }
-        {
-          uint32_t cls = 0; uint64_t jx = 0; int nj = 0;
-#pragma unroll 1
-          for (int m = 0; m < 16 && lane + 32 * m < q.T; ++m) {
-            uint32_t js;
-            const uint32_t code = wp_class(CD, n, lane + 32 * m, js);
-            cls |= code << (2 * m);
-            if (code == WP_JUNC) { jx |= (uint64_t)js << (8 * nj); ++nj; }
-          }
-          p_cls = cls; p_jx = jx;
-        }
-        {
-          const int gb1 = __shfl_sync(FULL, have ? grp_base : 0x7fffffff, 1), gb2 = __shfl_sync(FULL, have ? grp_base : 0x7fffffff, 2),
-                    gb3 = __shfl_sync(FULL, have ? grp_base : 0x7fffffff, 3);
-#pragma unroll
-          for (int jj = 0; jj < 2; ++jj) {
-            const int slot = jj * 32 + lane;
-            const bool active = slot < ngroups;
-            const int ci = active ? (slot >= gb1 ? 1 : 0) + (slot >= gb2 ? 1 : 0) + (slot >= gb3 ? 1 : 0) : 0;
-            const int gbc = ci == 0 ? 0 : ci == 1 ? gb1 : ci == 2 ? gb2 : gb3;
-            const int g = active ? slot - gbc : 0;
-            const int pq = CD[ci].rowpos + 1 + g * 8;
-            dd_dst[jj] = wp_vidx(pq);
-            dd_inf[jj] = (active ? 1 : 0) | (ci << 1) | ((pq & 7) << 3) | (g << 8);
-          }
-#pragma unroll
-          for (int X = 0; X < 2; ++X) wp_item(CD, L, X * 32 + lane, items, p_psi, wi_pp[X], wi_op[X], wi_inf[X]);
-        }
-        m_ok = true;
-      }
-    }
+    if (wp_plan_series(M, regular, have, n, P.init, P.end_time, P.nrows, P.vwire, P.grp_base, P.ngroups, q, L, Q, CD, lane)) { WPROF_COUNT(11) }
     WPROF(2)
     if (!regular) {
       WPROF_COUNT(12)
@@ -489,15 +632,15 @@
       if (two) { cur_sz = nb_sz; nb_sz = nxt_sz; stage ^= 1u; R = wb + (stage ? L.rec2 : WP_OFF_REC); } else cur_sz = nxt_sz;
       continue;
     }
-    if (c < WP_MAXC) {
-      WpChunk& d = CD[c];
-      d.grp_base = have ? grp_base : 0x7fffffff; d.ng = ng; d.wire = vwire; d.val_off = voff; d.dropped = P.dropped;
-      if (have && vwire == WIRE_XOR) { const uint32_t po = w12 >> 16; d.first = ld64(R + voff + po); d.grp_off = voff + po + 8; d.tab_off = voff + XOR_OFF_GROUPTAB; }
-      else { d.first = have ? ld64(R + voff + 8) : 0ull; d.grp_off = 0; d.tab_off = 0; }
+    {
+      const uint32_t voff = P.voff, po = P.w12 >> 16;
+      const bool x = have && P.vwire == WIRE_XOR;
+      wp_series_desc(CD, c, have, P.grp_base, P.ng, P.vwire, voff, P.dropped, x ? ld64(R + voff + po) : have ? ld64(R + voff + 8) : 0ull,
+                     x ? voff + po + 8 : 0u, x ? voff + XOR_OFF_GROUPTAB : 0u);
     }
     int cnt_rows = 0, cnt_bytes = 0;
-    { const int64_t endp = __shfl_up_sync(FULL, end_time, 1);
-      if (have && !(c > 0 && !(endp < lastEnd))) { cnt_rows = num_rows; cnt_bytes = vbytes; } }
+    { const int64_t endp = __shfl_up_sync(FULL, P.end_time, 1);
+      if (have && !(c > 0 && !(endp < Q.lastEnd))) { cnt_rows = P.num_rows; cnt_bytes = P.vbytes; } }
 #pragma unroll
     for (int o = 1; o < WP_MAXC; o <<= 1) { cnt_rows += __shfl_xor_sync(FULL, cnt_rows, o); cnt_bytes += __shfl_xor_sync(FULL, cnt_bytes, o); }
     __syncwarp();
@@ -506,22 +649,12 @@
       __syncwarp();
       if (sn < n_series && nxt_sz <= L.rec_cap && lane == 0) issue(nxt_off, nxt_sz);
     };
-    const uint32_t okbits = wp_decode<false>(R, V, CD, xtab, dd_dst, dd_inf, n, any_raw, lane, nullptr, rec_done);
+    const uint32_t okbits = wp_decode<false>(R, V, CD, xtab, M.dd_dst, M.dd_inf, n, P.any_raw, lane, nullptr, rec_done);
     const bool vals_ok = __all_sync(FULL, (okbits >> 30) & 1u);
     __syncwarp();
     if (two) { cur_sz = nb_sz; nb_sz = nxt_sz; stage ^= 1u; R = wb + (stage ? L.rec2 : WP_OFF_REC); } else cur_sz = nxt_sz;
     WPROF(4)
-    if (gz_all) {
-#pragma unroll
-      for (int u = 0; u < 3; ++u) if (gz[u] >= 0) V[gz[u]] = 0.0;
-    } else {
-      const int pend = CD[n - 1].rowpos + CD[n - 1].nrows + p_Wr + 8;
-      for (int g = 0; g <= n; ++g) {
-        const int g0 = g == 0 ? 0 : CD[g - 1].rowpos + CD[g - 1].nrows;
-        const int g1 = g == n ? pend : CD[g].rowpos;
-        for (int pz = g0 + lane; pz < g1; pz += 32) V[wp_vidx(pz)] = 0.0;
-      }
-    }
+    wp_zero_rows(V, CD, n, M, lane);
     WPROF(5)
     if (!vals_ok) {
       WPROF_COUNT(13)
@@ -531,96 +664,9 @@
     }
     if (lane == 0) { rows_scanned += cnt_rows; bytes_scanned += cnt_bytes; }
     __syncwarp();
-    const int psi = p_psi;
-    auto oidx = [&](int k) -> int { return k + ((k + psi) >> 3); };
-    {
-      const int Wr = p_Wr;
-      for (int it0 = 0; it0 < p_items; it0 += 64) {
-        int ipp[2], iop[2], iinf[2];
-#pragma unroll
-        for (int X = 0; X < 2; ++X) {
-          if (it0 == 0) { ipp[X] = wi_pp[X]; iop[X] = wi_op[X]; iinf[X] = wi_inf[X]; }
-          else wp_item(CD, L, it0 + X * 32 + lane, p_items, psi, ipp[X], iop[X], iinf[X]);
-        }
-        const double* pp[2]; double* op[2]; int jEnd[2], ot[2]; bool rawm[2];
-#pragma unroll
-        for (int X = 0; X < 2; ++X) {
-          pp[X] = V + ipp[X]; op[X] = reinterpret_cast<double*>(wb + iop[X]);
-          jEnd[X] = (iinf[X] & 15) - 1; rawm[X] = (iinf[X] >> 4) & 1; ot[X] = (iinf[X] >> 5) & 7;
-        }
-        double a[WP_R], bb[WP_R];
-        wp_block_pair(pp[0], pp[1], Wr, a, bb);
-        __syncwarp();
-#pragma unroll
-        for (int X = 0; X < 2; ++X) {
-          const double dv = rawm[X] ? 1.0 : fdiv, rc = rawm[X] ? 1.0 : frcp, sc = rawm[X] ? 1.0 : 1000.0;
-#pragma unroll
-          for (int j = 0; j < WP_R; ++j) {
-            const double raw = X ? bb[j] : a[j];
-            int nn = 1;
-            if (FN == FN_AVG || FN == FN_COUNT) {
-              const WpChunk& ch = CD[(iinf[X] >> 8) & 3];
-              int lo = ch.s0 + (iinf[X] >> 10) + j; const int hi0 = lo + Wr; if (lo < 0) lo = 0;
-              const int hi = hi0 > ch.nrows - 1 ? ch.nrows - 1 : hi0;
-              nn = hi - lo + 1;
-            }
-            const double fin = wp_finish<FN>(raw, nn, dv, rc, sc, p_nfull, p_rcpn, rawm[X]);
-            if (X) bb[j] = fin; else a[j] = fin;
-          }
-        }
-        if (p_oal) {
-#pragma unroll
-          for (int j = 0; j < WP_R; ++j) { if (j <= jEnd[0]) op[0][j] = a[j]; if (j <= jEnd[1]) op[1][j] = bb[j]; }
-        } else {
-#pragma unroll
-          for (int j = 0; j < WP_R; ++j) {
-            if (j <= jEnd[0]) op[0][j + ((ot[0] + j) >> 3)] = a[j];
-            if (j <= jEnd[1]) op[1][j + ((ot[1] + j) >> 3)] = bb[j];
-          }
-        }
-      }
-      __syncwarp();
-      WPROF(6)
-      double* gp = out + (size_t)s * q.T + lane;
-      const double* sp = O + oidx(lane);
-      auto fin = [&](double o, uint32_t code, uint32_t js, int k) -> double {
-        double v = o;
-        if (code == WP_JUNC) { const double jv = J[js & 127u]; v = (js & 128u) ? o + jv : jv; }
-        double r;
-        if (FN == FN_COUNT) r = v;
-        else {
-          int nn = 1;
-          if (FN == FN_AVG && (code == WP_RAWFIN || code == WP_JUNC)) {
-            const int ci = wp_chunk_of(CD, n, k);
-            nn = wp_rows_in(CD[ci], k, Wr);
-            if (code == WP_JUNC && (js & 128u)) nn += wp_rows_in(CD[ci - 1], k, Wr);
-          }
-          r = wp_finish<FN>(v, nn, fdiv, frcp, 1000.0, p_nfull, p_rcpn, false);
-        }
-        return code == WP_FINAL ? o : code == WP_GAP ? NaNv : r;
-      };
-      uint32_t cls = p_cls; uint64_t jx = p_jx;
-      auto fin_m = [&](double o, int k) -> double {
-        const uint32_t code = cls & 3u, js = (uint32_t)jx & 0xffu;
-        cls >>= 2;
-        if (code == WP_JUNC) jx >>= 8;
-        return fin(o, code, js, k);
-      };
-      int k = lane, iters = (q.T - lane + 31) >> 5;
-      int rest = iters > 16 ? iters - 16 : 0;
-      if (rest) iters = 16;
-      for (; iters >= 4; iters -= 4, gp += 128, sp += 144, k += 128) {
-        const double v0 = sp[0], v1 = sp[36], v2 = sp[72], v3 = sp[108];
-        const double r0 = fin_m(v0, k), r1 = fin_m(v1, k + 32), r2 = fin_m(v2, k + 64), r3 = fin_m(v3, k + 96);
-        wp_store_result(gp, r0); wp_store_result(gp + 32, r1); wp_store_result(gp + 64, r2); wp_store_result(gp + 96, r3);
-      }
-      for (; iters > 0; --iters, gp += 32, sp += 36, k += 32) wp_store_result(gp, fin_m(*sp, k));
-      for (; rest > 0; --rest, gp += 32, sp += 36, k += 32) {
-        uint32_t js;
-        const uint32_t code = wp_class(CD, n, k, js);
-        wp_store_result(gp, fin(*sp, code, js, k));
-      }
-    }
+    wp_window_blocks<FN>(V, wb, CD, L, M, Q, lane);
+    WPROF(6)
+    wp_finish_store<FN>(out, s, q, O, J, CD, n, M, Q, lane);
     __syncwarp();
     WPROF(7)
   }
@@ -631,4 +677,230 @@
   }
 }
 
-}
+#if defined(FILO_WP_PROF) && !defined(FILO_CUSIM)
+#define WPPROD_DECL uint32_t wpq_t0 = (uint32_t)clock(), wpq_acc[4] = {0, 0, 0, 0};
+#define WPPROD(i) { const uint32_t wpq_t1 = (uint32_t)clock(); wpq_acc[i] += wpq_t1 - wpq_t0; wpq_t0 = wpq_t1; }
+#define WPPROD_COUNT { ++wpq_acc[3]; }
+#define WPPROD_FLUSH if (lane == 0) { for (int wpq_i = 0; wpq_i < 4; ++wpq_i) atomicAdd(&g_wp_prof[16 + wpq_i], (unsigned long long)wpq_acc[wpq_i]); atomicAdd(&g_wp_prof[20], 1ull); }
+#else
+#define WPPROD_DECL
+#define WPPROD(i)
+#define WPPROD_COUNT
+#define WPPROD_FLUSH
+#endif
+
+template <int FN, int NW>
+__global__ void __launch_bounds__(NW * 32, 1)
+scan_wp_batch_kernel(const uint8_t* __restrict__ arena, const int64_t* __restrict__ rec_off, int64_t n_series, QueryParams q,
+                     double* __restrict__ out, WpBatchSmem BL, int64_t* __restrict__ fallback_list, unsigned long long* __restrict__ fallback_count,
+                     unsigned long long* d_counters, int* d_err) {
+  extern __shared__ __align__(128) uint8_t smem[];
+  const unsigned FULL = 0xffffffffu;
+  const int lane = threadIdx.x & 31, warp = threadIdx.x >> 5;
+  const WpSmem& L = BL.W;
+  const int B = (int)BL.B, NB = (int)BL.nbuf, NC = (int)BL.consumers;
+  uint64_t* full = reinterpret_cast<uint64_t*>(smem + BL.bars);
+  uint64_t* parsed = full + NB;
+  uint64_t* empty = parsed + NB;
+  WpEntry* ENT = reinterpret_cast<WpEntry*>(smem + BL.ent);
+  if (threadIdx.x == 0) {
+    for (int b = 0; b < NB; ++b) { mbar_init(full + b, 1); mbar_init(parsed + b, 1); mbar_init(empty + b, B); }
+    mbar_fence_init();
+  }
+  __syncthreads();
+
+  if (warp == NC) {
+    const int64_t t1 = q.start - q.window, t2 = q.end;
+    const int64_t lastEnd = q.start + (int64_t)(q.T - 1) * q.step;
+    const int c = lane & 3, lb = lane & 28;
+    WPPROD_DECL
+    auto batch_start = [&](int i) -> int64_t { return ((int64_t)blockIdx.x + (int64_t)i * gridDim.x) * B; };
+    auto load_offs = [&](int i) -> int64_t {
+      const int64_t b0 = batch_start(i);
+      int64_t o = 0;
+      if (b0 < n_series && lane <= B && b0 + lane <= n_series) o = rec_off[b0 + lane];
+      return o;
+    };
+    auto issue = [&](int i, int64_t offs) {
+      const int64_t b0 = batch_start(i);
+      const int ns = (int)(n_series - b0 < B ? n_series - b0 : B);
+      const int b = i % NB;
+      const int64_t o0 = __shfl_sync(FULL, offs, 0), o1 = __shfl_sync(FULL, offs, ns);
+      const uint32_t bytes = (uint32_t)(o1 - o0);
+      if (lane == 0) {
+        if (bytes <= BL.buf_cap) { mbar_expect_tx(full + b, bytes); tma_load_1d(smem + BL.buf + (size_t)b * BL.buf_stride, arena + o0, bytes, full + b); }
+        else mbar_arrive(full + b);
+      }
+    };
+    int64_t offs = load_offs(0), offs_n = 0;
+    if (batch_start(0) < n_series) { issue(0, offs); offs_n = load_offs(1); }
+    WPPROD(1)
+    for (int i = 0; batch_start(i) < n_series; ++i) {
+      const int64_t b0 = batch_start(i);
+      const int ns = (int)(n_series - b0 < B ? n_series - b0 : B);
+      const int b = i % NB, u = i / NB;
+      const int64_t offs_c = offs;
+      if (batch_start(i + 1) < n_series) {
+        const int bn = (i + 1) % NB, un = (i + 1) / NB;
+        if (un > 0) mbar_wait_parked(empty + bn, (un - 1) & 1);
+        WPPROD(0)
+        issue(i + 1, offs_n);
+        offs = offs_n; offs_n = load_offs(i + 2);
+      }
+      const uint8_t* buf = smem + BL.buf + (size_t)b * BL.buf_stride;
+      const uint32_t bytes = (uint32_t)(__shfl_sync(FULL, offs_c, ns) - __shfl_sync(FULL, offs_c, 0));
+      const bool staged = bytes <= BL.buf_cap;
+      mbar_wait(full + b, u & 1);
+      WPPROD(1)
+      WpEntry* E = ENT + (size_t)b * B;
+      for (int g = 0; g < ns; g += 8) {
+        const int sl = g + (lane >> 2);
+        const bool present = sl < ns;
+        const uint32_t rofs = (uint32_t)(__shfl_sync(FULL, offs_c, present ? sl : 0) - __shfl_sync(FULL, offs_c, 0));
+        const uint8_t* R = buf + rofs;
+        bool regular = present && staged;
+        int nch = 0;
+        if (regular) {
+          const RecordHeader* h = reinterpret_cast<const RecordHeader*>(R);
+          nch = (int)h->n_chunks;
+          regular = nch <= 32 && (h->flags & REC_ALL_TS_CONST) != 0;
+        }
+        uint32_t mb = 0, mw = 0;
+        const ChunkEntry* Eall = reinterpret_cast<const ChunkEntry*>(R + sizeof(RecordHeader));
+        for (int r = 0; __any_sync(FULL, regular && 4 * r < nch); ++r) {
+          const int ci = 4 * r + c;
+          bool below = false, within = false;
+          if (regular && ci < nch) { below = Eall[ci].end_time < t1; within = !below && Eall[ci].start_time <= t2; }
+          const unsigned bb = __ballot_sync(FULL, below), bw = __ballot_sync(FULL, within);
+          mb |= ((bb >> lb) & 0xfu) << (4 * r); mw |= ((bw >> lb) & 0xfu) << (4 * r);
+        }
+        int cLo = __ffs((int)~mb) - 1; if (cLo < 0) cLo = 32;
+        const unsigned rest = cLo < 32 ? (mw >> cLo) : 0u;
+        int n = __ffs((int)~rest) - 1; if (n < 0) n = 32;
+        if (n > WP_MAXC) regular = false;
+        bool have = regular && c < n;
+        int64_t init = 0, end_time = 0; int nrows = 0, num_rows = 0, vbytes = 0, ng = 0, vwire = 0, dropped = 0, tlen = 0; uint32_t voff = 0, w12 = 0;
+        bool okc = true, irrc = false; int slope = 0; uint32_t toff = 0;
+        if (have)
+          wp_chunk_fields<true, false>(R, Eall[cLo + c], q, init, end_time, nrows, num_rows, vbytes, ng, vwire, dropped, tlen, voff, w12, okc, irrc, slope, toff);
+        const int64_t endp = __shfl_up_sync(FULL, end_time, 1);
+        if (have && c > 0 && !(endp < init)) okc = false;
+        if (((__ballot_sync(FULL, okc) >> lb) & 0xfu) != 0xfu) regular = false;
+        have = have && regular;
+        if (!have) { ng = 0; nrows = 0; }
+        const int a0 = __shfl_sync(FULL, ng, lb), a1 = __shfl_sync(FULL, ng, lb + 1), a2 = __shfl_sync(FULL, ng, lb + 2), a3 = __shfl_sync(FULL, ng, lb + 3);
+        const int grp_base = (c > 0 ? a0 : 0) + (c > 1 ? a1 : 0) + (c > 2 ? a2 : 0);
+        if (a0 + a1 + a2 + a3 > WP_MAXG) regular = false;
+        const bool any_raw = ((__ballot_sync(FULL, have && vwire == WIRE_RAW64) >> lb) & 0xfu) != 0;
+        have = have && regular;
+        uint64_t first = 0; uint32_t grp_off = 0;
+        if (have && vwire == WIRE_XOR) { const uint32_t po = w12 >> 16; first = ld64(R + voff + po); grp_off = voff + po + 8; }
+        else if (have) first = ld64(R + voff + 8);
+        int cnt_rows = 0, cnt_bytes = 0;
+        if (have && !(c > 0 && !(endp < lastEnd))) { cnt_rows = num_rows; cnt_bytes = vbytes; }
+        cnt_rows += __shfl_xor_sync(FULL, cnt_rows, 1); cnt_bytes += __shfl_xor_sync(FULL, cnt_bytes, 1);
+        cnt_rows += __shfl_xor_sync(FULL, cnt_rows, 2); cnt_bytes += __shfl_xor_sync(FULL, cnt_bytes, 2);
+        if (present) {
+          WpEntry& e = E[sl];
+          WpEntryChunk& ec = e.c[c];
+          ec.first = first; ec.init = init; ec.end_time = end_time; ec.grp_off = grp_off; ec.val_off = voff;
+          ec.nrows = nrows; ec.grp_base = grp_base; ec.ng = ng; ec.wire = (uint32_t)vwire | ((uint32_t)dropped << 16);
+          if (c == 0) {
+            e.rofs = rofs; e.n = n; e.flags = (regular ? 1 : 0) | (any_raw ? 2 : 0); e.ngroups = a0 + a1 + a2 + a3;
+            e.cnt_rows = cnt_rows; e.cnt_bytes = cnt_bytes;
+          }
+        }
+      }
+      __syncwarp();
+      if (lane == 0) mbar_arrive(parsed + b);
+      WPPROD(2)
+      WPPROD_COUNT
+    }
+    WPPROD_FLUSH
+    return;
+  }
+
+  uint8_t* wb = smem + (size_t)warp * L.per_warp;
+  WpChunk* CD = reinterpret_cast<WpChunk*>(wb + WP_OFF_DESC);
+  uint64_t* xtab = reinterpret_cast<uint64_t*>(wb + WP_OFF_J);
+  double* J = reinterpret_cast<double*>(wb + WP_OFF_J);
+  double* V = reinterpret_cast<double*>(wb + L.vals);
+  double* O = reinterpret_cast<double*>(wb + L.out);
+  const int c = lane;
+  WpQuery Q; Q.init(q);
+  WpPlan M;
+  int64_t rows_scanned = 0, bytes_scanned = 0;
+  int i = warp / B, slot = warp % B;
+  WPROF_DECL
+  for (;; slot += NC) {
+    while (slot >= B) { slot -= B; ++i; }
+    const int64_t s = ((int64_t)blockIdx.x + (int64_t)i * gridDim.x) * B + slot;
+    if (s >= n_series) break;
+    const int b = i % NB, u = i / NB;
+    WPROF_COUNT(10)
+    WPROF(9)
+    mbar_wait(parsed + b, u & 1);
+    mbar_wait(full + b, u & 1);
+    WPROF(0)
+    const WpEntry& e = ENT[(size_t)b * B + slot];
+    const uint8_t* R = smem + BL.buf + (size_t)b * BL.buf_stride + e.rofs;
+    const int n = e.n, flags = e.flags;
+    bool regular = flags & 1;
+    const bool have = regular && c < n;
+    int64_t init = 0, end_time = 0; int nrows = 0, grp_base = 0, ng = 0, wire = 0; uint32_t voff = 0, grp_off = 0; uint64_t first = 0;
+    if (c < WP_MAXC) {
+      const WpEntryChunk& ec = e.c[c];
+      init = ec.init; end_time = ec.end_time; nrows = ec.nrows; grp_base = ec.grp_base; ng = ec.ng; wire = (int)ec.wire;
+      voff = ec.val_off; grp_off = ec.grp_off; first = ec.first;
+    }
+    const int vwire = wire & 0xffff;
+    WPROF(1)
+    if (wp_plan_series(M, regular, have, n, init, end_time, nrows, vwire, grp_base, e.ngroups, q, L, Q, CD, lane)) { WPROF_COUNT(11) }
+    WPROF(2)
+    if (!regular) {
+      WPROF_COUNT(12)
+      __syncwarp();
+      if (lane == 0) {
+        const unsigned long long fs = atomicAdd(fallback_count, 1ull); fallback_list[fs] = s;
+        mbar_arrive(empty + b);
+      }
+      __syncwarp();
+      continue;
+    }
+    wp_series_desc(CD, c, have, grp_base, ng, vwire, voff, wire >> 16, first, grp_off, have && vwire == WIRE_XOR ? voff + XOR_OFF_GROUPTAB : 0u);
+    const int cnt_rows = e.cnt_rows, cnt_bytes = e.cnt_bytes;
+    const bool any_raw = (flags & 2) != 0;
+    __syncwarp();
+    WPROF(3)
+    auto rec_done = [&]() {
+      __syncwarp();
+      if (lane == 0) mbar_arrive(empty + b);
+    };
+    const uint32_t okbits = wp_decode<false>(R, V, CD, xtab, M.dd_dst, M.dd_inf, n, any_raw, lane, nullptr, rec_done);
+    const bool vals_ok = __all_sync(FULL, (okbits >> 30) & 1u);
+    __syncwarp();
+    WPROF(4)
+    wp_zero_rows(V, CD, n, M, lane);
+    WPROF(5)
+    if (!vals_ok) {
+      WPROF_COUNT(13)
+      if (lane == 0) { const unsigned long long fs = atomicAdd(fallback_count, 1ull); fallback_list[fs] = s; }
+      __syncwarp();
+      continue;
+    }
+    if (lane == 0) { rows_scanned += cnt_rows; bytes_scanned += cnt_bytes; }
+    __syncwarp();
+    wp_window_blocks<FN>(V, wb, CD, L, M, Q, lane);
+    WPROF(6)
+    wp_finish_store<FN>(out, s, q, O, J, CD, n, M, Q, lane);
+    __syncwarp();
+    WPROF(7)
+  }
+  WPROF(9)
+  WPROF_FLUSH
+  if (lane == 0) {
+    if (rows_scanned | bytes_scanned) { atomicAdd(&d_counters[0], (unsigned long long)rows_scanned); atomicAdd(&d_counters[1], (unsigned long long)bytes_scanned); }
+  }
+}
+
+}
diff --git a/filodb_b200/csrc/scan_wp_layout.h b/filodb_b200/csrc/scan_wp_layout.h
--- a/filodb_b200/csrc/scan_wp_layout.h
+++ b/filodb_b200/csrc/scan_wp_layout.h
@@ -57,6 +57,55 @@
   L.alias = alias ? 1u : 0u;
   return L;
 }
+
+constexpr int WP_BATCH_WARPS = 16;
+constexpr int WP_BATCH_SERIES = 15;
+constexpr int WP_BATCH_BUFS = 2;
+struct WpEntryChunk {
+  uint64_t first;
+  int64_t init, end_time;
+  uint32_t grp_off, val_off;
+  int32_t nrows, grp_base, ng;
+  uint32_t wire;
+};
+static_assert(sizeof(WpEntryChunk) == 48, "WpEntryChunk");
+struct WpEntry {
+  uint32_t rofs;
+  int32_t n;
+  int32_t flags;
+  int32_t ngroups, cnt_rows, cnt_bytes;
+  int32_t pad[2];
+  WpEntryChunk c[WP_MAXC];
+};
+static_assert(sizeof(WpEntry) == 224, "WpEntry");
+struct WpBatchSmem {
+  WpSmem W;
+  uint32_t B, nbuf, consumers;
+  uint32_t buf, buf_stride, buf_cap;
+  uint32_t ent;
+  uint32_t bars;
+  uint32_t total;
+};
+FILO_HD inline WpBatchSmem wp_batch_layout(uint32_t max_rec_bytes, uint32_t max_rows, uint32_t max_chunks, uint32_t T, uint32_t wrows, bool alias,
+                                           uint32_t B = WP_BATCH_SERIES, uint32_t nbuf = WP_BATCH_BUFS, uint32_t consumers = WP_BATCH_WARPS - 1) {
+  WpBatchSmem S;
+  WpSmem L = wp_layout(max_rec_bytes, max_rows, max_chunks, T, wrows, alias);
+  const uint32_t shift = L.vals - WP_OFF_REC;
+  L.vals -= shift; L.out -= shift; L.per_warp -= shift; L.rec = 0;
+  S.consumers = consumers;
+  L.warps = S.consumers;
+  S.W = L; S.B = B; S.nbuf = nbuf;
+  uint32_t o = L.per_warp * S.consumers;
+  S.buf = o;
+  S.buf_cap = B * align_up(max_rec_bytes, 16);
+  S.buf_stride = S.buf_cap + 16;
+  o += nbuf * S.buf_stride;
+  S.ent = o; o += nbuf * B * (uint32_t)sizeof(WpEntry);
+  S.bars = o; o += 3 * nbuf * 8;
+  S.total = align_up(o, 16);
+  return S;
+}
+
 FILO_HD inline uint32_t wp_max_items(uint32_t max_chunks, uint32_t T, uint32_t wrows) {
   if (max_chunks > (uint32_t)WP_MAXC) max_chunks = WP_MAXC;
   if (max_chunks == 0) max_chunks = 1;
diff --git a/scratch/wp_prof.py b/scratch/wp_prof.py
--- a/scratch/wp_prof.py
+++ b/scratch/wp_prof.py
@@ -14,7 +14,7 @@
 series = sys.argv[2] if len(sys.argv) > 2 else "5000000"
 L = capi.lib()
 L.filo_debug_wp_prof.argtypes = [C.c_void_p, C.c_int]
-out = np.zeros(16, np.uint64)
+out = np.zeros(32, np.uint64)
 sys.argv = ["bench.py", "--workload", workload, "--series", series, "--steps", "4", "--warmup", "2", "--no-e2e", "--no-cpu", "--no-extra", "--no-c5"]
 L.filo_debug_wp_prof(out.ctypes.data, 1)
 bench.main()
@@ -23,7 +23,7 @@
          "zero rows", "window blocks", "finish and store (earlier: fix-up, gaps)", None, "loop head, declined series"]
 ns = float(out[10])
 tot = float(out[:10].sum())
-print("scan_wp_sum_kernel: %d warps, %d series taken up, %d memo misses, %d declined by the plan, %d declined by the values"
+print("SUM kernel: %d consumer warps, %d series taken up, %d memo misses, %d declined by the plan, %d declined by the values"
       % (int(out[15]), int(ns), int(out[11]), int(out[12]), int(out[13])))
 print("  %-40s %10s %7s" % ("phase", "cyc/series", "share"))
 for i, n in enumerate(names):
@@ -33,3 +33,10 @@
         n = "result row (earlier builds)"
     print("  %-40s %10.1f %6.1f %%" % (n, float(out[i]) / ns, 100.0 * float(out[i]) / tot))
 print("  %-40s %10.1f" % ("total", tot / ns))
+if out[20]:
+    nb = float(out[19])
+    ptot = float(out[16:19].sum())
+    print("producer: %d warps, %d batches" % (int(out[20]), int(nb)))
+    for i, n in enumerate(["stalled on the empty barrier", "offsets, copy issue, copy wait", "header parse, entries"]):
+        print("  %-40s %10.1f %6.1f %%" % (n, float(out[16 + i]) / nb, 100.0 * float(out[16 + i]) / ptot))
+    print("  %-40s %10.1f" % ("total", ptot / nb))
```
